# zalo/TetSim

Measured on AMD Instinct MI355X. Metric: tet_solves_per_sec, higher is better.
Workload: dtype f32; 1 GPU; Kuhn-6 cube lattice 55x55x55 cells (998250 tets, 175616 particles), polar-decomposition Jacobi, 20 substeps/frame, dt=1/1200 s; solver=polar_jacobi, arithmetic=fast, formulation=reference (rest shape carried from substep to substep, 148 B/tet), tets=998250, particles=175616, parallelism=single GPU

## Files before the change

include/tetsim.h:

```cpp
#ifndef TETSIM_H
#define TETSIM_H

#include <stdint.h>

#ifdef __cplusplus
extern "C" {
#endif

#define TETSIM_ABI_VERSION 5

typedef struct tetsim_body *tetsim_handle;

enum {
    TETSIM_OK = 0,
    TETSIM_EINVAL = 1,
    TETSIM_ENODEVICE = 2,
    TETSIM_EHIP = 3,
    TETSIM_ENOMEM = 4,
    TETSIM_ECOMM = 5,
    TETSIM_ESTATE = 6
};

enum {
    TETSIM_SOLVER_POLAR_JACOBI = 0,
// ... 102 lines not shown
int tetsim_write_state(tetsim_handle h, const float *pos, const float *vel);
int tetsim_state_size(tetsim_handle h, uint64_t *bytes_out);
int tetsim_save_state(tetsim_handle h, void *blob, uint64_t bytes);
int tetsim_load_state(tetsim_handle h, const void *blob, uint64_t bytes);

int tetsim_get_owned_ids(tetsim_handle h, int32_t *out);
int tetsim_get_local_tets(tetsim_handle h, int32_t *out);
int tetsim_get_tet_order(tetsim_handle h, int32_t *out);
int tetsim_get_level_offsets(tetsim_handle h, int32_t *out);
int tetsim_read_inv_mass(tetsim_handle h, float *out);


int tetsim_set_visual_mesh(tetsim_handle h, const float *vis_verts, uint32_t nvis, const float *rest_normals);
int tetsim_get_visual_ids(tetsim_handle h, int32_t *out);
int tetsim_read_visual_mesh(tetsim_handle h, float *positions_out, float *normals_out);
int tetsim_halo_refresh_final(tetsim_handle h);
int tetsim_group_refresh_final(tetsim_handle *handles, uint32_t count);
int tetsim_set_visual_triangles(tetsim_handle h, const int32_t *tri_ids, uint32_t ntri);
int tetsim_read_visual_vertex_normals(tetsim_handle h, float *normals_out);
int tetsim_visual_vertex_normals_from(tetsim_handle h, const float *all_positions, float *normals_out);
int tetsim_group_read_visual_vertex_normals(tetsim_handle *handles, uint32_t count, float *positions_out, float *normals_out);


int tetsim_set_grab(tetsim_handle h, int32_t id, const float xyz[3]);
int tetsim_start_grab(tetsim_handle h, const float xyz[3], int32_t *id_out);
int tetsim_nearest_particle(tetsim_handle h, const float xyz[3], int32_t *global_id, double *dist2);


typedef struct TetSimRay    { double origin[3], direction[3], near, far; } TetSimRay;
typedef struct TetSimRayHit { int32_t hit, body, triangle, reserved; double distance, point[3]; } TetSimRayHit;
int tetsim_raycast_visual(tetsim_handle h, const TetSimRay *rays, uint32_t count, TetSimRayHit *hits);
int tetsim_start_grab_ray(tetsim_handle h, const TetSimRay *ray, TetSimRayHit *hit_out, int32_t *id_out);
int tetsim_read_visual_bounding_sphere(tetsim_handle h, double centre[3], double *radius);


enum { TETSIM_COLLIDER_SPHERE = 0, TETSIM_COLLIDER_CAPSULE = 1, TETSIM_COLLIDER_BOX = 2, TETSIM_COLLIDER_PLANE = 3 };
#define TETSIM_MAX_COLLIDERS 8
typedef struct TetSimCollider {
    int32_t kind;
    int32_t reserved;
    double a[3];
    double b[3];
    double axes[9];
    double radius;
    double friction;
    double velocity[3];
} TetSimCollider;
int tetsim_set_colliders(tetsim_handle h, const TetSimCollider *colliders, uint32_t count);


enum { TETSIM_FIELD_POSITIONS = 0, TETSIM_FIELD_VELOCITIES = 1, TETSIM_FIELD_PREV_POSITIONS = 2,
       TETSIM_FIELD_QUATS = 3, TETSIM_FIELD_VISUAL_POSITIONS = 4, TETSIM_FIELD_VISUAL_NORMALS = 5,
       TETSIM_FIELD_VISUAL_VERTEX_NORMALS = 6 };
#define TETSIM_MAX_EXPORT_FIELDS 8
typedef struct TetSimDeviceField {
    int32_t field, reserved;
    void *dst;
    uint64_t row_stride;
} TetSimDeviceField;
int tetsim_export_device(tetsim_handle h, const TetSimDeviceField *fields, uint32_t count, void *consumer_stream);
int tetsim_import_device(tetsim_handle h, const void *pos, uint64_t pos_stride,
                         const void *vel, uint64_t vel_stride, void *producer_stream);


typedef struct tetsim_snapshot_s *tetsim_snapshot;
int tetsim_snapshot_create(tetsim_handle h, tetsim_snapshot *out);
int tetsim_snapshot_capture(tetsim_handle h, tetsim_snapshot s, const void *body_mask, void *caller_stream);
int tetsim_snapshot_restore(tetsim_handle h, tetsim_snapshot s, const void *body_mask, void *caller_stream);
void tetsim_snapshot_destroy(tetsim_snapshot s);


#define TETSIM_OBS_WIDTH 20
enum { TETSIM_OBS_MASS = 0, TETSIM_OBS_COM = 1 , TETSIM_OBS_VCOM = 4 , TETSIM_OBS_VOLUME = 7,
       TETSIM_OBS_REST_VOLUME = 8, TETSIM_OBS_MIN_VOLUME_RATIO = 9, TETSIM_OBS_INVERTED_TETS = 10,
       TETSIM_OBS_AABB_MIN = 11 , TETSIM_OBS_AABB_MAX = 14 , TETSIM_OBS_MAX_SPEED2 = 17,
       TETSIM_OBS_NONFINITE = 18, TETSIM_OBS_RESERVED = 19  };
int tetsim_observe_bodies_device(tetsim_handle h, void *dst, uint64_t row_stride, void *caller_stream);
int tetsim_read_body_observations(tetsim_handle h, double *out);


#define TETSIM_RAY_INVALID (-1)
int tetsim_raycast_visual_device(tetsim_handle h,
        const void *rays,     uint64_t ray_stride,
        const void *ray_body,
        uint32_t count,
        void *hits,           uint64_t hit_stride,
        void *caller_stream);
int tetsim_visual_bounding_spheres_device(tetsim_handle h, void *dst, uint64_t row_stride, void *caller_stream);


#define TETSIM_STRAIN_WIDTH 16
#define TETSIM_STRAIN_BODY_WIDTH 8
#define TETSIM_STRAIN_SWEEPS 4
enum { TETSIM_STRAIN_F = 0 , TETSIM_STRAIN_J = 9, TETSIM_STRAIN_DEV = 10,
       TETSIM_STRAIN_STRETCH = 11 , TETSIM_STRAIN_GREEN = 14, TETSIM_STRAIN_RESERVED = 15  };
int tetsim_tet_strain_device(tetsim_handle h, void *dst, uint64_t row_stride, void *caller_stream);
int tetsim_read_tet_strain(tetsim_handle h, float *out);
int tetsim_body_strain_device(tetsim_handle h, void *dst, uint64_t row_stride, void *caller_stream);
int tetsim_visual_strain_device(tetsim_handle h, int32_t channel, void *dst, uint64_t row_stride, void *caller_stream);
int tetsim_prep_strain_table(const float *verts, uint32_t nv, const int32_t *tets, uint32_t nt, double density, void *records_out);


int tetsim_profile(tetsim_handle h, uint32_t n, double dt, const TetSimParams *params, TetSimProfile *out);
int tetsim_time_kernels(tetsim_handle h, uint32_t reps, double dt, const TetSimParams *params, TetSimProfile *out);
int tetsim_time_step_n(tetsim_handle h, uint32_t n, double dt, const TetSimParams *params, double *ms_out);
int tetsim_measure_copy_bandwidth(int32_t device, uint64_t bytes, uint32_t reps, double *gbps_out);
int tetsim_measure_stream_bandwidth(int32_t device, uint64_t bytes, uint32_t reps, int32_t kind, double *gbps_out);


int tetsim_comm_unique_id(void *id128);
int tetsim_comm_init(tetsim_handle h, const void *id128, int32_t rank, int32_t nranks);
typedef struct TetSimCommInfo {
    int32_t rccl_ranks, rccl_rank;
    uint32_t neighbours;
    uint64_t send_bytes_per_substep, recv_bytes_per_substep, max_message_bytes;
    int32_t loopback;
    int32_t p2p;
} TetSimCommInfo;
int tetsim_comm_info(tetsim_handle h, TetSimCommInfo *out);
int tetsim_comm_selftest(tetsim_handle h);
int tetsim_comm_probe(tetsim_handle h, uint64_t bytes, uint32_t reps, int32_t use_graph, uint32_t per_graph,
                      double *host_us, double *total_us);
int tetsim_halo_probe(tetsim_handle h, uint32_t reps, double *min_us, double *median_us, double *max_us);
#define TETSIM_P2P_BLOB_BYTES 512
int tetsim_halo_p2p_export(tetsim_handle h, void *blob);
int tetsim_halo_p2p_connect(tetsim_handle h, const void *blobs, uint32_t count);
int tetsim_halo_p2p_probe(tetsim_handle h, uint32_t reps, double *min_us, double *median_us, double *max_us);
int tetsim_group_step_n(tetsim_handle *handles, uint32_t count, uint32_t n, double dt, const TetSimParams *params);
int tetsim_halo_exchange_local(tetsim_handle *handles, uint32_t count);
int tetsim_get_halo_plan(tetsim_handle h, int32_t *neigh ,
                         int32_t *send_counts, int32_t *recv_counts,
                         int32_t *send_ids, int32_t *recv_ids);
int tetsim_halo_export(tetsim_handle h, uint32_t n, float *out_xyzw);
int tetsim_halo_import(tetsim_handle h, uint32_t n, const float *in_xyzw);


int tetsim_prep_levels(const int32_t *tets, uint32_t nt, uint32_t nv, int32_t *level, uint32_t *num_levels);
int tetsim_prep_colours(const int32_t *tets, uint32_t nt, uint32_t nv, int32_t *colour, uint32_t *num_colours);
int tetsim_prep_clusters(const int32_t *tets, uint32_t nt, uint32_t nv, int32_t *order, int32_t *launch, int32_t *lane,
                         int32_t *step, uint32_t *num_launches, uint32_t *num_clusters);
int tetsim_prep_tiles(const float *verts, uint32_t nv, const int32_t *tets, uint32_t nt, const uint32_t *body_first_tet,
                      const uint32_t *body_first_vert, uint32_t bodies, int32_t *tile_tets, uint32_t *tile_off,
                      uint8_t *corner_slot, uint32_t *num_tiles);
int tetsim_prep_slot_table(const int32_t *tets, uint32_t nt, uint32_t nv, int32_t ref_quirk,
                           int32_t *slots , uint32_t *dropped);
int tetsim_prep_call_tiles(const float *verts, uint32_t nv, const int32_t *tets, uint32_t nt, uint32_t sizes[4],
                           uint32_t *blk_vert_off, int32_t *blk_verts, uint32_t *vp_ell);
int tetsim_prep_call_schedule(const int32_t *blk_verts, const uint32_t *blk_vert_off, uint32_t nb, const uint32_t *vp_ell,
                              uint32_t vp_cols, uint32_t nv_pad, uint32_t nv_owned, uint32_t lag, uint32_t *entry,
                              uint32_t capacity, uint32_t *period, uint32_t *tail, int32_t *fell_back);
int tetsim_prep_check_call_schedule(const int32_t *blk_verts, const uint32_t *blk_vert_off, uint32_t nb, const uint32_t *vp_ell,
                                    uint32_t vp_cols, uint32_t nv_pad, uint32_t nv_owned, const uint32_t *entry, uint32_t period,
                                    uint32_t tail);
int tetsim_prep_ref_grab_texels(int32_t grab_id, uint32_t num_elems, uint32_t num_particles, int32_t out[2]);
int tetsim_prep_boundary_surface(const float *verts ,
                                 const int32_t *tets, uint32_t nt, uint32_t nv,
                                 float *vis_verts , int32_t *tri_ids ,
                                 uint32_t *nrows, uint32_t *ntri);
int tetsim_prep_rest(const float *verts, uint32_t nv, const int32_t *tets, uint32_t nt, double density,
                     float *inv_mass, float *inv_rest_pose, float *inv_rest_volume);

int tetsim_prep_partition(const float *verts , uint32_t nv, const int32_t *tets, uint32_t nt,
                          int32_t part_count, int32_t *vert_owner_out);
typedef struct TetSimPartQuality {
    uint32_t owned_particles;
    uint32_t ghost_particles;
    uint32_t boundary_particles;
    uint32_t local_elems;
    uint32_t owned_elems;
    uint32_t num_neighbours;
} TetSimPartQuality;
int tetsim_prep_partition_quality(const int32_t *tets, uint32_t nt, uint32_t nv, int32_t part_count,
                                  const int32_t *vert_owner, TetSimPartQuality *out);

typedef struct tetsim_plan_s *tetsim_plan;
typedef struct TetSimPlanSizes {
    uint32_t owned_particles, boundary_particles, local_particles, local_elems, owned_elems, num_neighbours;
} TetSimPlanSizes;
int tetsim_plan_create(const int32_t *tets, uint32_t nt, uint32_t nv, int32_t part_count, int32_t part_index,
                       const int32_t *vert_owner, tetsim_plan *out);
int tetsim_plan_create_deep(const int32_t *tets, uint32_t nt, uint32_t nv, int32_t part_count, int32_t part_index,
                            const int32_t *vert_owner, int32_t depth, tetsim_plan *out);
int tetsim_plan_layers(tetsim_plan p, uint32_t *first_layer_ghosts, uint8_t *tet_layer);
int tetsim_plan_neighbour_layer2(tetsim_plan p, uint32_t i, uint32_t *send_count, uint32_t *recv_start, uint32_t *recv_count);
int tetsim_plan_neighbour_layer2_ids(tetsim_plan p, uint32_t i, int32_t *send_local, int32_t *send_global, int32_t *recv_global);
void tetsim_plan_destroy(tetsim_plan p);
int tetsim_plan_sizes(tetsim_plan p, TetSimPlanSizes *out);
int tetsim_plan_arrays(tetsim_plan p, int32_t *local_to_global_vert, int32_t *local_to_global_tet, int32_t *local_tets);
int tetsim_plan_neighbour(tetsim_plan p, uint32_t i, int32_t *rank, uint32_t *send_count, uint32_t *recv_start,
                          uint32_t *recv_count, int32_t *send_is_contiguous);
int tetsim_plan_neighbour_ids(tetsim_plan p, uint32_t i, int32_t *send_local, int32_t *send_global, int32_t *recv_global);

int tetsim_abi_version(void);
typedef struct TetSimLibraryInfo {
    int32_t abi;
    int32_t ablation;
    uint32_t debug_env;
    char source_sha[20];
    char kernel_sha[20];
} TetSimLibraryInfo;
int tetsim_library_info(TetSimLibraryInfo *out);

typedef struct TetSimMeshArrays {
    uint32_t num_particles;
    uint32_t num_elems;
    uint32_t num_edges;
    uint32_t num_vis_verts;
    uint32_t num_vis_tris;
    uint32_t part_count;
    const float *verts;
    const int32_t *tets;
    const int32_t *edge_ids;
    const float *vis_verts;
    const int32_t *vis_tri_ids;
    const int32_t *tet_colour;
    const int32_t *vert_owner;
} TetSimMeshArrays;
typedef struct tetsim_mesh_file *tetsim_mesh;

int tetsim_mesh_write(const char *path, const TetSimMeshArrays *a);
int tetsim_mesh_open(const char *path, tetsim_mesh *out);
int tetsim_mesh_arrays(tetsim_mesh m, TetSimMeshArrays *out);
int tetsim_mesh_close(tetsim_mesh m);
int tetsim_create_from_file(const char *path, const TetSimOptions *opts, tetsim_handle *out);

#ifdef __cplusplus
}
#endif
#endif
```

tetsim_amd/_capi.py:

```python
import ctypes as C
import os

_HERE = os.path.dirname(os.path.abspath(__file__))
LIB_PATH = os.environ.get("TETSIM_HIP_LIB") or os.path.join(_HERE, "libtetsim_hip.so")

OK, EINVAL, ENODEVICE, EHIP, ENOMEM, ECOMM, ESTATE = range(7)
RAY_INVALID = -1
SOLVER_POLAR_JACOBI, SOLVER_NEOHOOKEAN_GS = 0, 1
PRECISE, FAST = 0, 1
ORDER_ORIGINAL, ORDER_COLOURED, ORDER_CLUSTERED = 0, 1, 2
FLAG_REF_SLOT_TABLE, FLAG_REF_FIXED_BOUNDS, FLAG_GATHER_FORMULATION, FLAG_CONSTANT_REST_SHAPE, FLAG_REF_GRAB_TEXEL, FLAG_DEEP_GHOSTS = 1, 2, 4, 8, 16, 32
FLAG_REF_ROTATION_EXIT = 64
FLAG_LEAN_STATE = 128
K_TET, K_VERTEX, K_HALO, K_COUNT = 0, 1, 2, 3
COLLIDER_SPHERE, COLLIDER_CAPSULE, COLLIDER_BOX, COLLIDER_PLANE = 0, 1, 2, 3
MAX_COLLIDERS = 8
FIELD_POSITIONS, FIELD_VELOCITIES, FIELD_PREV_POSITIONS, FIELD_QUATS, FIELD_VISUAL_POSITIONS, FIELD_VISUAL_NORMALS, FIELD_VISUAL_VERTEX_NORMALS = range(7)
MAX_EXPORT_FIELDS = 8
OBS_WIDTH = 20
(OBS_MASS, OBS_COM, OBS_VCOM, OBS_VOLUME, OBS_REST_VOLUME, OBS_MIN_VOLUME_RATIO, OBS_INVERTED_TETS, OBS_AABB_MIN, OBS_AABB_MAX, OBS_MAX_SPEED2,
 OBS_NONFINITE, OBS_RESERVED) = 0, 1, 4, 7, 8, 9, 10, 11, 14, 17, 18, 19
STRAIN_WIDTH, STRAIN_BODY_WIDTH, STRAIN_SWEEPS = 16, 8, 4
STRAIN_F, STRAIN_J, STRAIN_DEV, STRAIN_STRETCH, STRAIN_GREEN, STRAIN_RESERVED = 0, 9, 10, 11, 14, 15


class TetSimParams(C.Structure):
    _fields_ = [("gravity", C.c_double), ("friction", C.c_double), ("devCompliance", C.c_double),
                ("volCompliance", C.c_double), ("worldBounds", C.c_double * 6)]


class TetSimOptions(C.Structure):
    _fields_ = [("solver", C.c_int32), ("precision", C.c_int32), ("order", C.c_int32), ("flags", C.c_uint32),
                ("device", C.c_int32), ("density", C.c_double), ("part_count", C.c_int32),
                ("part_index", C.c_int32), ("vert_owner", C.POINTER(C.c_int32)), ("tet_colour", C.POINTER(C.c_int32))]


class TetSimMeshArrays(C.Structure):
    _fields_ = [("num_particles", C.c_uint32), ("num_elems", C.c_uint32), ("num_edges", C.c_uint32),
                ("num_vis_verts", C.c_uint32), ("num_vis_tris", C.c_uint32), ("part_count", C.c_uint32),
                ("verts", C.POINTER(C.c_float)), ("tets", C.POINTER(C.c_int32)), ("edge_ids", C.POINTER(C.c_int32)),
                ("vis_verts", C.POINTER(C.c_float)), ("vis_tri_ids", C.POINTER(C.c_int32)),
                ("tet_colour", C.POINTER(C.c_int32)), ("vert_owner", C.POINTER(C.c_int32))]


class TetSimInfo(C.Structure):
    _fields_ = [("num_particles", C.c_uint32), ("num_elems", C.c_uint32), ("owned_particles", C.c_uint32),
                ("local_particles", C.c_uint32), ("local_elems", C.c_uint32), ("owned_elems", C.c_uint32),
                ("num_levels", C.c_uint32), ("max_valence", C.c_uint32), ("dropped_slots", C.c_uint32),
                ("num_neighbours", C.c_uint32), ("device_bytes", C.c_uint64), ("solver", C.c_int32),
                ("precision", C.c_int32), ("order", C.c_int32), ("device", C.c_int32), ("flags", C.c_uint32),
                ("num_vis_verts", C.c_uint32), ("num_bodies", C.c_uint32), ("fused_particle_pass", C.c_uint32), ("total_vis_verts", C.c_uint32)]


class TetSimProfile(C.Structure):
    _fields_ = [("total_ms", C.c_double), ("kernel_ms", C.c_double * K_COUNT), ("launches", C.c_uint32 * K_COUNT),
                ("substeps", C.c_uint32), ("tets_per_tet_launch", C.c_uint32)]


class TetSimLibraryInfo(C.Structure):
    _fields_ = [("abi", C.c_int32), ("ablation", C.c_int32), ("debug_env", C.c_uint32), ("source_sha", C.c_char * 20),
                ("kernel_sha", C.c_char * 20)]


DEBUG_ENV_NAMES = ["TETSIM_DEBUG_LOOPBACK_HALO", "TETSIM_DEBUG_LOOPBACK_COPY", "TETSIM_DEBUG_ONE_STREAM", "TETSIM_DEBUG_GROUP_SYNC",
                   "TETSIM_DEBUG_HOSTPROF", "TETSIM_DEBUG_TRACE", "TETSIM_HALO_SYNC", "TETSIM_HALO_GRAPH", "TETSIM_DEBUG_LOOPBACK_DELAY_US", "TETSIM_NH_QUADS", "TETSIM_FUSED_PARTICLE_PASS",
                   "TETSIM_FRAME_KERNEL", "TETSIM_FRAME_LOCAL", "TETSIM_NH_FOLD", "TETSIM_HALO_ALIGNED_TILES", "TETSIM_HALO_FOLD_WAIT", "TETSIM_QUAD", "TETSIM_QUAD_POLL_DELAY", "TETSIM_NH_FRAME",
                   "TETSIM_NH_ONE_LAUNCH", "TETSIM_PJ_ONE_LAUNCH", "TETSIM_PJ_CALL_LAG"]


LAB_ENV_NAMES = ["TETSIM_DEBUG_TRACE", "TETSIM_NH_QUADS", "TETSIM_FRAME_LOCAL", "TETSIM_NH_FOLD", "TETSIM_HALO_ALIGNED_TILES", "TETSIM_QUAD_POLL_DELAY", "TETSIM_NH_FRAME"]


class TetSimCommInfo(C.Structure):
    _fields_ = [("rccl_ranks", C.c_int32), ("rccl_rank", C.c_int32), ("neighbours", C.c_uint32), ("send_bytes_per_substep", C.c_uint64),
                ("recv_bytes_per_substep", C.c_uint64), ("max_message_bytes", C.c_uint64), ("loopback", C.c_int32), ("p2p", C.c_int32)]


class TetSimPlanSizes(C.Structure):
    _fields_ = [("owned_particles", C.c_uint32), ("boundary_particles", C.c_uint32), ("local_particles", C.c_uint32),
                ("local_elems", C.c_uint32), ("owned_elems", C.c_uint32), ("num_neighbours", C.c_uint32)]


class TetSimPartQuality(C.Structure):
    _fields_ = [("owned_particles", C.c_uint32), ("ghost_particles", C.c_uint32), ("boundary_particles", C.c_uint32),
                ("local_elems", C.c_uint32), ("owned_elems", C.c_uint32), ("num_neighbours", C.c_uint32)]


class TetSimError(RuntimeError):
    def __init__(self, code, msg):
        super().__init__("tetsim error %d: %s" % (code, msg))
        self.code = code


class TetSimCollider(C.Structure):
    _fields_ = [("kind", C.c_int32), ("reserved", C.c_int32), ("a", C.c_double * 3), ("b", C.c_double * 3), ("axes", C.c_double * 9),
                ("radius", C.c_double), ("friction", C.c_double), ("velocity", C.c_double * 3)]


class TetSimRay(C.Structure):
    _fields_ = [("origin", C.c_double * 3), ("direction", C.c_double * 3), ("near", C.c_double), ("far", C.c_double)]


class TetSimRayHit(C.Structure):
    _fields_ = [("hit", C.c_int32), ("body", C.c_int32), ("triangle", C.c_int32), ("reserved", C.c_int32), ("distance", C.c_double),
                ("point", C.c_double * 3)]


class TetSimDeviceField(C.Structure):
    _fields_ = [("field", C.c_int32), ("reserved", C.c_int32), ("dst", C.c_void_p), ("row_stride", C.c_uint64)]


SYMBOLS = [
    "tetsim_abi_version", "tetsim_default_options", "tetsim_default_params", "tetsim_create", "tetsim_create_batch", "tetsim_get_batch_layout", "tetsim_destroy",
    "tetsim_last_error", "tetsim_get_info", "tetsim_step", "tetsim_step_n", "tetsim_sync",
    "tetsim_library_info", "tetsim_read_quats_pinned", "tetsim_state_size", "tetsim_save_state", "tetsim_load_state",
    "tetsim_read_positions", "tetsim_read_positions_pinned", "tetsim_read_prev_positions", "tetsim_read_velocities", "tetsim_read_quats",
    "tetsim_read_vol_error", "tetsim_write_state", "tetsim_get_owned_ids", "tetsim_get_local_tets",
    "tetsim_get_tet_order", "tetsim_get_level_offsets", "tetsim_read_inv_mass", "tetsim_set_visual_mesh", "tetsim_get_visual_ids", "tetsim_halo_refresh_final", "tetsim_group_refresh_final", "tetsim_halo_probe", "tetsim_halo_p2p_probe",
    "tetsim_read_visual_mesh", "tetsim_set_visual_triangles", "tetsim_read_visual_vertex_normals", "tetsim_visual_vertex_normals_from", "tetsim_group_read_visual_vertex_normals", "tetsim_set_grab", "tetsim_set_colliders",
    "tetsim_start_grab", "tetsim_nearest_particle", "tetsim_profile", "tetsim_time_kernels", "tetsim_time_step_n", "tetsim_measure_copy_bandwidth", "tetsim_measure_stream_bandwidth",
    "tetsim_comm_unique_id", "tetsim_comm_init", "tetsim_comm_info", "tetsim_comm_selftest", "tetsim_comm_probe", "tetsim_group_step_n", "tetsim_halo_exchange_local", "tetsim_get_halo_plan",
    "tetsim_halo_p2p_export", "tetsim_halo_p2p_connect",
    "tetsim_halo_export", "tetsim_halo_import", "tetsim_prep_levels", "tetsim_prep_colours", "tetsim_prep_clusters",
    "tetsim_prep_tiles", "tetsim_prep_slot_table", "tetsim_prep_call_tiles", "tetsim_prep_call_schedule", "tetsim_prep_check_call_schedule", "tetsim_prep_ref_grab_texels", "tetsim_prep_rest", "tetsim_prep_partition", "tetsim_prep_partition_quality", "tetsim_plan_create", "tetsim_plan_destroy", "tetsim_plan_sizes",
    "tetsim_plan_arrays", "tetsim_plan_neighbour", "tetsim_plan_neighbour_ids",
    "tetsim_plan_create_deep", "tetsim_plan_layers", "tetsim_plan_neighbour_layer2", "tetsim_plan_neighbour_layer2_ids",
    "tetsim_raycast_visual", "tetsim_start_grab_ray", "tetsim_read_visual_bounding_sphere", "tetsim_prep_boundary_surface",
    "tetsim_export_device", "tetsim_import_device",
    "tetsim_snapshot_create", "tetsim_snapshot_capture", "tetsim_snapshot_restore", "tetsim_snapshot_destroy",
    "tetsim_observe_bodies_device", "tetsim_read_body_observations",
    "tetsim_raycast_visual_device", "tetsim_visual_bounding_spheres_device",
    "tetsim_tet_strain_device", "tetsim_read_tet_strain", "tetsim_body_strain_device", "tetsim_visual_strain_device", "tetsim_prep_strain_table",
    "tetsim_mesh_write", "tetsim_mesh_open", "tetsim_mesh_arrays", "tetsim_mesh_close", "tetsim_create_from_file",
]

OPTIONAL_SYMBOLS = ("tetsim_set_colliders", "tetsim_raycast_visual", "tetsim_start_grab_ray", "tetsim_read_visual_bounding_sphere", "tetsim_prep_boundary_surface",
                    "tetsim_export_device", "tetsim_import_device",
                    "tetsim_snapshot_create", "tetsim_snapshot_capture", "tetsim_snapshot_restore", "tetsim_snapshot_destroy",
                    "tetsim_observe_bodies_device", "tetsim_read_body_observations",
                    "tetsim_raycast_visual_device", "tetsim_visual_bounding_spheres_device",
                    "tetsim_tet_strain_device", "tetsim_read_tet_strain", "tetsim_body_strain_device", "tetsim_visual_strain_device", "tetsim_prep_strain_table")

_lib = None


def lib():
    global _lib
    if _lib is not None:
        return _lib
    if not os.path.exists(LIB_PATH):
        raise ImportError("libtetsim_hip.so is not built: run `python -m tetsim_amd.build` "
                          "(the HIP extension is mandatory; there is no CPU fallback)")
    L = C.CDLL(LIB_PATH)
    H, fp, ip, dp = C.c_void_p, C.POINTER(C.c_float), C.POINTER(C.c_int32), C.POINTER(C.c_double)
    u32, i32, dbl = C.c_uint32, C.c_int32, C.c_double
    PP = C.POINTER(TetSimParams)
    L.tetsim_abi_version.restype = C.c_int
    L.tetsim_default_options.argtypes = [C.POINTER(TetSimOptions)]
    L.tetsim_default_options.restype = None
    L.tetsim_default_params.argtypes = [PP]
    L.tetsim_default_params.restype = None
    L.tetsim_create.argtypes = [fp, u32, ip, u32, C.POINTER(TetSimOptions), C.POINTER(H)]
    L.tetsim_create_batch.argtypes = [C.POINTER(fp), C.POINTER(u32), C.POINTER(ip), C.POINTER(u32), u32, C.POINTER(TetSimOptions), C.POINTER(H)]
    L.tetsim_get_batch_layout.argtypes = [H, C.POINTER(u32), C.POINTER(u32)]
    L.tetsim_destroy.argtypes = [H]
    L.tetsim_destroy.restype = None
    L.tetsim_comm_probe.argtypes = [H, C.c_uint64, u32, i32, u32, dp, dp]
    L.tetsim_nearest_particle.argtypes = [H, fp, ip, dp]
    L.tetsim_mesh_write.argtypes = [C.c_char_p, C.POINTER(TetSimMeshArrays)]
    L.tetsim_mesh_open.argtypes = [C.c_char_p, C.POINTER(H)]
    L.tetsim_mesh_arrays.argtypes = [H, C.POINTER(TetSimMeshArrays)]
    L.tetsim_mesh_close.argtypes = [H]
    L.tetsim_create_from_file.argtypes = [C.c_char_p, C.POINTER(TetSimOptions), C.POINTER(H)]
    L.tetsim_last_error.argtypes = [H]
    L.tetsim_last_error.restype = C.c_char_p
    L.tetsim_get_info.argtypes = [H, C.POINTER(TetSimInfo)]
    L.tetsim_step.argtypes = [H, dbl, PP]
    L.tetsim_step_n.argtypes = [H, u32, dbl, PP]
    L.tetsim_sync.argtypes = [H]
    for n in ("positions", "prev_positions", "velocities", "quats", "inv_mass"):
        getattr(L, "tetsim_read_" + n).argtypes = [H, fp]
    L.tetsim_read_positions_pinned.argtypes = [H, C.POINTER(fp)]
    L.tetsim_read_quats_pinned.argtypes = [H, C.POINTER(fp)]
    L.tetsim_library_info.argtypes = [C.POINTER(TetSimLibraryInfo)]
    L.tetsim_state_size.argtypes = [H, C.POINTER(C.c_uint64)]
    L.tetsim_save_state.argtypes = [H, C.c_void_p, C.c_uint64]
    L.tetsim_load_state.argtypes = [H, C.c_void_p, C.c_uint64]
    L.tetsim_read_vol_error.argtypes = [H, dp]
    L.tetsim_write_state.argtypes = [H, fp, fp]
    for n in ("owned_ids", "local_tets", "tet_order", "level_offsets"):
        getattr(L, "tetsim_get_" + n).argtypes = [H, ip]
    L.tetsim_set_visual_mesh.argtypes = [H, fp, u32, fp]
    L.tetsim_read_visual_mesh.argtypes = [H, fp, fp]
    L.tetsim_get_visual_ids.argtypes = [H, C.POINTER(C.c_int32)]
    L.tetsim_halo_refresh_final.argtypes = [H]
    L.tetsim_halo_probe.argtypes = [H, u32, C.POINTER(C.c_double), C.POINTER(C.c_double), C.POINTER(C.c_double)]
    L.tetsim_halo_p2p_probe.argtypes = [H, u32, C.POINTER(C.c_double), C.POINTER(C.c_double), C.POINTER(C.c_double)]
    L.tetsim_group_refresh_final.argtypes = [C.POINTER(H), u32]
    L.tetsim_set_visual_triangles.argtypes = [H, ip, u32]
    L.tetsim_read_visual_vertex_normals.argtypes = [H, fp]
    L.tetsim_visual_vertex_normals_from.argtypes = [H, fp, fp]
    L.tetsim_group_read_visual_vertex_normals.argtypes = [C.POINTER(H), u32, fp, fp]
    L.tetsim_set_grab.argtypes = [H, i32, fp]
    if hasattr(L, "tetsim_set_colliders"):
        L.tetsim_set_colliders.argtypes = [H, C.POINTER(TetSimCollider), u32]
    L.tetsim_start_grab.argtypes = [H, fp, ip]
    if hasattr(L, "tetsim_raycast_visual"):
        L.tetsim_raycast_visual.argtypes = [H, C.c_void_p, u32, C.c_void_p]
        L.tetsim_start_grab_ray.argtypes = [H, C.POINTER(TetSimRay), C.POINTER(TetSimRayHit), ip]
        L.tetsim_read_visual_bounding_sphere.argtypes = [H, dp, dp]
        L.tetsim_prep_boundary_surface.argtypes = [fp, ip, u32, u32, fp, ip, C.POINTER(u32), C.POINTER(u32)]
    if hasattr(L, "tetsim_export_device"):
        L.tetsim_export_device.argtypes = [H, C.POINTER(TetSimDeviceField), u32, C.c_void_p]
        L.tetsim_import_device.argtypes = [H, C.c_void_p, C.c_uint64, C.c_void_p, C.c_uint64, C.c_void_p]
    if hasattr(L, "tetsim_snapshot_create"):
        L.tetsim_snapshot_create.argtypes = [H, C.POINTER(H)]
        L.tetsim_snapshot_capture.argtypes = [H, H, C.c_void_p, C.c_void_p]
        L.tetsim_snapshot_restore.argtypes = [H, H, C.c_void_p, C.c_void_p]
        L.tetsim_snapshot_destroy.argtypes = [H]
        L.tetsim_snapshot_destroy.restype = None
    if hasattr(L, "tetsim_observe_bodies_device"):
        L.tetsim_observe_bodies_device.argtypes = [H, C.c_void_p, C.c_uint64, C.c_void_p]
        L.tetsim_read_body_observations.argtypes = [H, dp]
    if hasattr(L, "tetsim_raycast_visual_device"):
        L.tetsim_raycast_visual_device.argtypes = [H, C.c_void_p, C.c_uint64, C.c_void_p, u32, C.c_void_p, C.c_uint64, C.c_void_p]
        L.tetsim_visual_bounding_spheres_device.argtypes = [H, C.c_void_p, C.c_uint64, C.c_void_p]
    if hasattr(L, "tetsim_tet_strain_device"):
        L.tetsim_tet_strain_device.argtypes = [H, C.c_void_p, C.c_uint64, C.c_void_p]
        L.tetsim_read_tet_strain.argtypes = [H, fp]
        L.tetsim_body_strain_device.argtypes = [H, C.c_void_p, C.c_uint64, C.c_void_p]
        L.tetsim_visual_strain_device.argtypes = [H, i32, C.c_void_p, C.c_uint64, C.c_void_p]
        L.tetsim_prep_strain_table.argtypes = [fp, u32, ip, u32, dbl, C.c_void_p]
    L.tetsim_profile.argtypes = [H, u32, dbl, PP, C.POINTER(TetSimProfile)]
    L.tetsim_time_kernels.argtypes = [H, u32, dbl, PP, C.POINTER(TetSimProfile)]
    L.tetsim_time_step_n.argtypes = [H, u32, dbl, PP, dp]
    L.tetsim_measure_copy_bandwidth.argtypes = [i32, C.c_uint64, u32, dp]
    L.tetsim_measure_stream_bandwidth.argtypes = [i32, C.c_uint64, u32, i32, dp]
    L.tetsim_comm_unique_id.argtypes = [C.c_void_p]
    L.tetsim_comm_init.argtypes = [H, C.c_void_p, i32, i32]
    L.tetsim_comm_selftest.argtypes = [H]
    L.tetsim_comm_info.argtypes = [H, C.POINTER(TetSimCommInfo)]
    L.tetsim_group_step_n.argtypes = [C.POINTER(H), u32, u32, dbl, PP]
    L.tetsim_halo_exchange_local.argtypes = [C.POINTER(H), u32]
    L.tetsim_halo_p2p_export.argtypes = [H, C.c_void_p]
    L.tetsim_halo_p2p_connect.argtypes = [H, C.c_void_p, u32]
    L.tetsim_get_halo_plan.argtypes = [H, ip, ip, ip, ip, ip]
    L.tetsim_halo_export.argtypes = [H, u32, fp]
    L.tetsim_halo_import.argtypes = [H, u32, fp]
    L.tetsim_prep_levels.argtypes = [ip, u32, u32, ip, C.POINTER(u32)]
    L.tetsim_prep_colours.argtypes = [ip, u32, u32, ip, C.POINTER(u32)]
    L.tetsim_prep_clusters.argtypes = [ip, u32, u32, ip, ip, ip, ip, C.POINTER(u32), C.POINTER(u32)]
    L.tetsim_prep_tiles.argtypes = [fp, u32, ip, u32, C.POINTER(u32), C.POINTER(u32), u32, ip, C.POINTER(u32), C.POINTER(C.c_uint8), C.POINTER(u32)]
    L.tetsim_prep_slot_table.argtypes = [ip, u32, u32, i32, ip, C.POINTER(u32)]
    up = C.POINTER(u32)
    L.tetsim_prep_call_tiles.argtypes = [fp, u32, ip, u32, up, up, ip, up]
    L.tetsim_prep_call_schedule.argtypes = [ip, up, u32, up, u32, u32, u32, u32, up, u32, up, up, ip]
    L.tetsim_prep_check_call_schedule.argtypes = [ip, up, u32, up, u32, u32, u32, up, u32, u32]
    L.tetsim_prep_ref_grab_texels.argtypes = [i32, u32, u32, ip]
    L.tetsim_prep_rest.argtypes = [fp, u32, ip, u32, dbl, fp, fp, fp]
    L.tetsim_prep_partition.argtypes = [fp, u32, ip, u32, i32, ip]
    L.tetsim_prep_partition_quality.argtypes = [ip, u32, u32, i32, ip, C.POINTER(TetSimPartQuality)]
    L.tetsim_plan_create.argtypes = [ip, u32, u32, i32, i32, ip, C.POINTER(H)]
    L.tetsim_plan_destroy.argtypes = [H]
    L.tetsim_plan_destroy.restype = None
    L.tetsim_plan_sizes.argtypes = [H, C.POINTER(TetSimPlanSizes)]
    L.tetsim_plan_arrays.argtypes = [H, ip, ip, ip]
    L.tetsim_plan_neighbour.argtypes = [H, u32, ip, C.POINTER(u32), C.POINTER(u32), C.POINTER(u32), ip]
    L.tetsim_plan_neighbour_ids.argtypes = [H, u32, ip, ip, ip]
    L.tetsim_plan_create_deep.argtypes = [ip, u32, u32, i32, i32, ip, i32, C.POINTER(H)]
    L.tetsim_plan_layers.argtypes = [H, C.POINTER(u32), C.POINTER(C.c_uint8)]
    L.tetsim_plan_neighbour_layer2.argtypes = [H, u32, C.POINTER(u32), C.POINTER(u32), C.POINTER(u32)]
    L.tetsim_plan_neighbour_layer2_ids.argtypes = [H, u32, ip, ip, ip]
    for s in SYMBOLS:
        if s in OPTIONAL_SYMBOLS and not hasattr(L, s):
            continue
        f = getattr(L, s)
        if s not in ("tetsim_default_options", "tetsim_default_params", "tetsim_destroy", "tetsim_last_error",
                     "tetsim_plan_destroy", "tetsim_snapshot_destroy"):
            f.restype = C.c_int
    _lib = L
    return L


def library_info():
    li = TetSimLibraryInfo()
    check(lib().tetsim_library_info(C.byref(li)))
    return {"abi": li.abi, "ablation": bool(li.ablation), "source_sha": li.source_sha.decode(), "kernel_sha": li.kernel_sha.decode(),
            "debug_env": [n for i, n in enumerate(DEBUG_ENV_NAMES) if li.debug_env >> i & 1], "path": LIB_PATH}


def check(rc, handle=None):
    if rc != OK:
        msg = lib().tetsim_last_error(handle)
        raise TetSimError(rc, msg.decode("utf-8", "replace") if msg else "")
```

tetsim_amd/csrc/body.h:

```cpp
#pragma once
#include <dlfcn.h>
#include <hip/hip_runtime.h>
#include <rccl/rccl.h>

#include <algorithm>
#include <atomic>
#include <chrono>
#include <cmath>
#include <cstdio>
#include <cstdlib>
#include <cstring>
#include <map>
#include <string>
#include <vector>

#include "../../include/tetsim.h"
#include "dev_common.h"
#include "dev_store.h"
#include "query_device.h"
#include "host_prep.h"
#include "mesh_file.h"

namespace tetsim {

// ... 4 lines not shown
    ncclResult_t (*GetUniqueId)(ncclUniqueId*) = nullptr;
    ncclResult_t (*CommInitRank)(ncclComm_t*, int, ncclUniqueId, int) = nullptr;
    ncclResult_t (*CommDestroy)(ncclComm_t) = nullptr;
    ncclResult_t (*CommCount)(const ncclComm_t, int*) = nullptr;
    ncclResult_t (*CommUserRank)(const ncclComm_t, int*) = nullptr;
    ncclResult_t (*Send)(const void*, size_t, ncclDataType_t, int, ncclComm_t, hipStream_t) = nullptr;
    ncclResult_t (*Recv)(void*, size_t, ncclDataType_t, int, ncclComm_t, hipStream_t) = nullptr;
    ncclResult_t (*GroupStart)() = nullptr;
    ncclResult_t (*GroupEnd)() = nullptr;
    const char* (*GetErrorString)(ncclResult_t) = nullptr;
    std::string err;
    bool loaded = false, process_wide = false;
    bool load() {
        if (loaded) return true;
        if (const char* over = getenv("TETSIM_RCCL_LIB")) {
            lib = dlopen(over, RTLD_NOW | RTLD_LOCAL);
            if (!lib) { err = std::string("cannot load TETSIM_RCCL_LIB=") + over + ": " + dlerror(); return false; }
        }
        for (const char* name : {"librccl.so.1", "librccl.so"}) {
            if (lib) break;
            lib = dlopen(name, RTLD_NOW | RTLD_NOLOAD);
        }
        if (!lib && dlsym(RTLD_DEFAULT, "ncclCommInitRank") && dlsym(RTLD_DEFAULT, "ncclSend")) process_wide = true;
        for (const char* name : {"librccl.so.1", "librccl.so", "/opt/rocm/lib/librccl.so.1"}) {
            if (lib || process_wide) break;
            lib = dlopen(name, RTLD_NOW | RTLD_LOCAL | RTLD_DEEPBIND);
        }
        if (!lib && !process_wide) { err = std::string("cannot load librccl: ") + dlerror(); return false; }
        auto sym = [&](const char* n) { void* p = dlsym(process_wide ? RTLD_DEFAULT : lib, n); if (!p) err = std::string("librccl lacks ") + n; return p; };
        GetUniqueId = reinterpret_cast<decltype(GetUniqueId)>(sym("ncclGetUniqueId"));
        CommInitRank = reinterpret_cast<decltype(CommInitRank)>(sym("ncclCommInitRank"));
        CommDestroy = reinterpret_cast<decltype(CommDestroy)>(sym("ncclCommDestroy"));
        CommCount = reinterpret_cast<decltype(CommCount)>(sym("ncclCommCount"));
        CommUserRank = reinterpret_cast<decltype(CommUserRank)>(sym("ncclCommUserRank"));
        Send = reinterpret_cast<decltype(Send)>(sym("ncclSend"));
        Recv = reinterpret_cast<decltype(Recv)>(sym("ncclRecv"));
        GroupStart = reinterpret_cast<decltype(GroupStart)>(sym("ncclGroupStart"));
        GroupEnd = reinterpret_cast<decltype(GroupEnd)>(sym("ncclGroupEnd"));
        GetErrorString = reinterpret_cast<decltype(GetErrorString)>(sym("ncclGetErrorString"));
        loaded = GetUniqueId && CommInitRank && CommDestroy && CommCount && CommUserRank && Send && Recv && GroupStart && GroupEnd && GetErrorString;
        return loaded;
    }
};
inline const char* lab_env(const char* name) {
#ifdef TETSIM_ABLATION
    return getenv(name);
#else
    (void)name;
    return nullptr;
#endif
}
extern Rccl g_rccl;
extern std::atomic<uint64_t> g_stream_generation;

struct PeerLink {
    float4* ghost[2] = {nullptr, nullptr};
    uint32_t* arrived[2] = {nullptr, nullptr};
    void* ipc[3] = {nullptr, nullptr, nullptr};
    float4* g1_even[2] = {nullptr, nullptr};
    float4* g1_final[2] = {nullptr, nullptr};
    float4* g2_even[2] = {nullptr, nullptr};
    float4* g2_odd[2] = {nullptr, nullptr};
    uint32_t* arrived2[2][2] = {{nullptr, nullptr}, {nullptr, nullptr}};
};
struct NeighDev {
    int rank = -1;
    uint32_t send_count = 0, recv_start = 0, recv_count = 0;
    bool contiguous = false;
    uint32_t send_first = 0;
    int32_t* send_idx = nullptr;
    float4* send_buf = nullptr;
    std::vector<int32_t> send_global, recv_global, send_local;
};

struct ObsDev {
    const void* tets = nullptr;
    const double* v0 = nullptr;
    const void *chunks = nullptr, *bodies = nullptr;
    double* partial = nullptr;
    double* rows = nullptr;
    uint32_t n_chunks = 0;
    bool ready = false;
};

struct StrainRec {
    int32_t id[4];
    float b[9];
    uint32_t degenerate;
    double v0_abs;
};
static_assert(sizeof(StrainRec) == 64 && alignof(StrainRec) == 8, "four dwordx4 loads per record");
struct StrainDev {
    const void* table = nullptr;
    const void *chunks = nullptr, *bodies = nullptr;
    const uint32_t* vis_tet = nullptr;
    double* partial = nullptr;
    float* rows = nullptr;
    uint32_t n_chunks = 0;
    bool ready = false;
};

}

using namespace tetsim;

struct tetsim_snapshot_s;

struct tetsim_body {
    std::string err;
    TetSimOptions opt{};
    TetSimInfo info{};
    hipStream_t stream = nullptr, comm_stream = nullptr;
    hipEvent_t ev_fork = nullptr, ev_bnd_tet = nullptr;
    uint32_t interior_tets = 0;
    bool queues_probed = false, queues_independent = false;
    uint64_t probe_generation = 0;
    std::map<uint32_t, std::pair<hipGraphExec_t, hipGraphExec_t>> flag_graphs;
    uint32_t* d_sync = nullptr;
    bool flag_sync = false;
    bool halo_graph_broken = false;
    bool halo_warm = false;
    bool loopback = false;
    bool vel_dead = false;
    bool needs_halo_refresh = false;
    bool fork_needed = true;
    hipEvent_t ev_a = nullptr, ev_b = nullptr, ev_halo = nullptr;
    hipEvent_t ev_boundary2[2] = {nullptr, nullptr}, ev_packed2[2] = {nullptr, nullptr}, ev_sent2[2] = {nullptr, nullptr};
    uint32_t halo_parity = 0;
    DevParams* d_params = nullptr;
    DevParams* d_params_halo = nullptr;
    std::vector<int32_t> tet_colour;
    int32_t grab_global = -1;
    int32_t grab_ref[2] = {-1, -1};
    float grab_pos[3] = {0, 0, 0};
    uint32_t n_colliders = 0;
    DevColliderF col[kMaxColliders] = {};
    DevColliderD d_col[kMaxColliders] = {};
    std::map<uint32_t, hipGraphExec_t> graphs;
    std::vector<void*> allocs;
    std::vector<float> h_verts;
    std::vector<int32_t> h_tets;
    std::vector<uint32_t> batch_first_vert, batch_first_tet;
    bool fast = false;

    PJDev pj;
    PJBlk blk;
    bool blocked = false;
    bool halo_use_flags = true;
    bool halo_use_graph = true;
    bool fused = false;
    bool pj_one_launch = false;
    uint32_t* d_substep_err = nullptr;
    PJCallSched call_sched;
    float4 *rest0_a = nullptr, *rest0_b = nullptr, *rest0_c = nullptr;
    bool quat_stale = false;
    bool frame = false;
    uint32_t frame_epoch = 1;
    uint32_t fold_wave_limit = 0, fold_tile_limit = 0;
    bool quad = false;
    uint32_t* d_frame_err = nullptr;
    int32_t* d_block_tile = nullptr;
    uint32_t frame_blocks = 0;
    DevParams params_on_device;
    bool params_known = false;
    bool frame_local = false;
    bool frame_turn_counted = false;
    bool epoch_block_fresh = false;
    bool frame_exclusive = false;
    float4* partial_b = nullptr;
    size_t partial_slots = 0;
    float4* pos_final_b = nullptr;
    bool fold_halo = false;
    bool fold_possible = false;
    bool fold_wait = false;
    bool v_pending = false;
    uint32_t fuse_step = 0;
    bool fin_in_b = false;
    std::vector<int32_t> tet_perm;
    std::vector<uint32_t> api2dev, dev2api;
    Partition part;
    bool partitioned = false;
    std::vector<int32_t> g2l_owned;
    std::vector<NeighDev> neigh;
    bool pred_any_dt = true;
    float dt_pred = 0.0f;
    ncclComm_t comm = nullptr;
    int comm_rank = -1, comm_size = 0;
    bool deep = false;
    uint32_t n_ghost1 = 0, nb_first = 0;
    std::vector<int32_t> g2l_ghost1;
    bool p2p = false;
    uint32_t timeout_ms = 0;
    float4* ghost_alt = nullptr;
    uint32_t* d_arrived = nullptr;
    uint32_t* d_peer_slots = nullptr;
    uint32_t p2p_cols = 0, p2p_stride = 0;
    uint32_t* d_peer_slots2 = nullptr;
    uint32_t p2p_cols2 = 0;
    float4* own_g1_even[2] = {nullptr, nullptr};
    float4* own_g1_final[2] = {nullptr, nullptr};
    float4* own_g2_even[2] = {nullptr, nullptr};
    float4* own_g2_odd[2] = {nullptr, nullptr};
    std::vector<PeerLink> links;
    uint32_t p2p_probe_base = 0;
    uint64_t p2p_round = 0;
    bool p2p_raise_pending = false;
    bool halo_pending = false;
    bool final_ghosts_fresh = false;
    std::vector<tetsim_body*> group;

    SkinDev skin;
    std::vector<uint32_t> vis_tet;
    std::vector<int32_t> vis_global;
    bool vis_attached = false;
    uint32_t vis_total = 0;
    float4* d_vis_full = nullptr;
    float* pinned_pos = nullptr;
    float* d_packed = nullptr;
    size_t packed_cap = 0;
    float* pinned_quat = nullptr;
    uint32_t* d_api2dev = nullptr;
    hipEvent_t ev_io[2][2] = {{nullptr, nullptr}, {nullptr, nullptr}};
    uint32_t io_parity = 0;
    std::vector<tetsim_snapshot_s*> snapshots;
    uint32_t *d_snap_first_vert = nullptr, *d_snap_first_elem = nullptr, *d_snap_tet_body = nullptr;
    ObsDev obs;
    StrainDev strain;
    double* d_best = nullptr; uint32_t* d_best_id = nullptr;
    uint32_t* d_sphere = nullptr;
    RayIn* d_rays = nullptr; RayPrep* d_ray_prep = nullptr; RayOut* d_ray_hits = nullptr; RayCand* d_ray_cand = nullptr;
    size_t ray_cap = 0, ray_prep_cap = 0, ray_hits_cap = 0, ray_cand_cap = 0;
    std::vector<int32_t> vis_row_body, tri_body;
    QueryBodiesDev qbodies;
    bool qrows_ready = false, qtris_ready = false;
    bool tri_spans_bodies = false;
    RayCand* d_cast_cand = nullptr;

    NHDev nh;
    std::vector<NHClusterLaunch> cluster_launch;
    int32_t* d_slot_vid = nullptr;
    bool nh_fold = false;
    uint8_t* d_first_mask = nullptr;
    uint32_t* d_nh_untouched = nullptr;
    uint32_t nh_untouched = 0;
    bool nh_one_launch = false;
    bool nh_call = false;
    NHSweep nh_sweep1;
    uint32_t nh_sub_index = 0;
    uint32_t nh_epoch_arg = 0;
    std::vector<uint32_t> level_off;
    bool nh_frame = false;
    NHFrameLaunch nh_frame_launch;
    std::vector<uint32_t> nh_seg;
    std::vector<int32_t> order;
    std::vector<float> h_inv_mass;
};

namespace tetsim {

inline bool is_batch(const tetsim_body* h) { return !h->batch_first_vert.empty(); }
inline void body_ranges(const tetsim_body* h, std::vector<uint32_t>* first_vert, std::vector<uint32_t>* first_tet) {
    *first_vert = h->batch_first_vert; *first_tet = h->batch_first_tet;
    if (!is_batch(h)) { *first_vert = {0u, h->info.num_particles}; *first_tet = {0u, h->info.num_elems}; }
}
inline uint32_t body_of_tet(const tetsim_body* h, uint32_t t) {
    const std::vector<uint32_t>& first = h->batch_first_tet;
    return first.empty() ? 0u : static_cast<uint32_t>(std::upper_bound(first.begin(), first.end(), t) - first.begin()) - 1u;
}

inline double rest_volume(const float* v, const int32_t* t) {
    const float *a = v + 3 * t[0], *b = v + 3 * t[1], *c = v + 3 * t[2], *d = v + 3 * t[3];
    const double e1x = static_cast<double>(b[0]) - a[0], e1y = static_cast<double>(b[1]) - a[1], e1z = static_cast<double>(b[2]) - a[2];
    const double e2x = static_cast<double>(c[0]) - a[0], e2y = static_cast<double>(c[1]) - a[1], e2z = static_cast<double>(c[2]) - a[2];
    const double e3x = static_cast<double>(d[0]) - a[0], e3y = static_cast<double>(d[1]) - a[1], e3z = static_cast<double>(d[2]) - a[2];
    const double cx = e2y * e3z - e2z * e3y, cy = e2z * e3x - e2x * e3z, cz = e2x * e3y - e2y * e3x;
    return ((e1x * cx + e1y * cy) + e1z * cz) / 6.0;
}

void build_strain_table(const float* verts, uint32_t nv, const int32_t* tets, uint32_t nt, double density, StrainRec* out);

#define HIPCHK(h, call)                                                                                 \
    do {                                                                                                \
        hipError_t e_ = (call);                                                                         \
        if (e_ != hipSuccess) {                                                                         \
            (h)->err = std::string(#call) + ": " + hipGetErrorString(e_);                               \
            return TETSIM_EHIP;                                                                         \
        }                                                                                               \
    } while (0)

int fail(tetsim_body* h, int code, const std::string& msg);
const char* create_error();
void group_begin(tetsim_body* const* hs, uint32_t count);
int group_result(tetsim_body* const* hs, uint32_t count, int rc);

template <class Tp>
inline int dev_alloc(tetsim_body* h, Tp** p, size_t count) {
    *p = nullptr;
    const size_t bytes = std::max<size_t>(count, 1) * sizeof(Tp);
    void* raw = nullptr;
    hipError_t e = hipMalloc(&raw, bytes);
    if (e != hipSuccess) { h->err = std::string("hipMalloc(") + std::to_string(bytes) + "): " + hipGetErrorString(e); return TETSIM_ENOMEM; }
    h->allocs.push_back(raw);
    h->info.device_bytes += bytes;
    *p = static_cast<Tp*>(raw);
    return 0;
}
// ... 112 lines not shown
```

tetsim_amd/csrc/build_info.cpp:

```cpp
#include <cstdlib>
#include <cstring>

#include "../../include/tetsim.h"

#ifndef TETSIM_SOURCE_SHA
#define TETSIM_SOURCE_SHA "unstamped"
#endif
#ifndef TETSIM_KERNEL_SHA
#define TETSIM_KERNEL_SHA "unstamped"
#endif

extern "C" int tetsim_library_info(TetSimLibraryInfo* out) {
    if (!out) return TETSIM_EINVAL;
    std::memset(out, 0, sizeof(*out));
    out->abi = TETSIM_ABI_VERSION;
#ifdef TETSIM_ABLATION
    out->ablation = 1;
#endif
    static const struct { const char* name; bool lab; } kEnv[] = {
        {"TETSIM_DEBUG_LOOPBACK_HALO", false}, {"TETSIM_DEBUG_LOOPBACK_COPY", false}, {"TETSIM_DEBUG_ONE_STREAM", false}, {"TETSIM_DEBUG_GROUP_SYNC", false},
        {"TETSIM_DEBUG_HOSTPROF", false}, {"TETSIM_DEBUG_TRACE", true}, {"TETSIM_HALO_SYNC", false}, {"TETSIM_HALO_GRAPH", false}, {"TETSIM_DEBUG_LOOPBACK_DELAY_US", false},
        {"TETSIM_NH_QUADS", true}, {"TETSIM_FUSED_PARTICLE_PASS", false}, {"TETSIM_FRAME_KERNEL", false}, {"TETSIM_FRAME_LOCAL", true}, {"TETSIM_NH_FOLD", true},
        {"TETSIM_HALO_ALIGNED_TILES", true}, {"TETSIM_HALO_FOLD_WAIT", false}, {"TETSIM_QUAD", false}, {"TETSIM_QUAD_POLL_DELAY", true}, {"TETSIM_NH_FRAME", true},
        {"TETSIM_NH_ONE_LAUNCH", false}, {"TETSIM_PJ_ONE_LAUNCH", false}, {"TETSIM_PJ_CALL_LAG", false}};
    for (unsigned i = 0; i < sizeof(kEnv) / sizeof(kEnv[0]); i++) {
#ifndef TETSIM_ABLATION
        if (kEnv[i].lab) continue;
#endif
        if (std::getenv(kEnv[i].name)) out->debug_env |= 1u << i;
    }
    std::strncpy(out->source_sha, TETSIM_SOURCE_SHA, sizeof(out->source_sha) - 1);
    std::strncpy(out->kernel_sha, TETSIM_KERNEL_SHA, sizeof(out->kernel_sha) - 1);
    return TETSIM_OK;
}
```

tetsim_amd/csrc/host_prep.cpp:

```cpp
#include "host_prep.h"

#include <algorithm>
#include <cmath>
#include <numeric>

namespace tetsim {

namespace {
inline float fround(double x) { return static_cast<float>(x); }

inline void edge_matrix(const float* verts, const int32_t* t, float m[9]) {
    for (int k = 0; k < 3; k++)
        for (int c = 0; c < 3; c++)
            m[3 * k + c] = fround(static_cast<double>(verts[3 * t[k + 1] + c]) - static_cast<double>(verts[3 * t[0] + c]));
}
inline double det3(const float* A) {
    double a11 = A[0], a12 = A[3], a13 = A[6];
    double a21 = A[1], a22 = A[4], a23 = A[7];
    double a31 = A[2], a32 = A[5], a33 = A[8];
    return a11 * a22 * a33 + a12 * a23 * a31 + a13 * a21 * a32 - a13 * a22 * a31 - a12 * a21 * a33 - a11 * a23 * a32;
}
}

void prep_rest(const float* verts, uint32_t nv, const int32_t* tets, uint32_t nt, double density,
// ... 341 lines not shown
    std::vector<uint8_t> live(4ull * nt, 0);
    for (int32_t enc : inc.slot) live[enc] = 1;

    std::vector<int32_t> slot_of(nv, -1);
    std::vector<int32_t> touched;
    struct Run { uint32_t begin, end; bool ghost; uint8_t cls; };
    auto cls_of = [&](uint32_t sorted_pos) -> uint8_t { return tet_class ? tet_class[B.tet_perm[sorted_pos]] : 0; };
    std::vector<Run> runs;
    {
        uint32_t i = 0;
        while (i < nt) {
            const uint32_t t0 = i;
            touched.clear();
            bool ghost = false;
            while (i < nt && i - t0 < kMaxTets && body_of_pos[i] == body_of_pos[t0] && cls_of(i) == cls_of(t0)) {
                const int32_t* t = &tets[4 * B.tet_perm[i]];
                uint32_t fresh = 0;
                for (int k = 0; k < 4; k++) {
                    bool seen = slot_of[t[k]] >= 0;
                    for (int j = 0; j < k && !seen; j++) seen = t[j] == t[k];
                    if (!seen) fresh++;
                }
                if (touched.size() + fresh > kMaxVerts) break;
                for (int k = 0; k < 4; k++)
                    if (slot_of[t[k]] < 0) {
                        slot_of[t[k]] = 0; touched.push_back(t[k]);
                        ghost |= static_cast<uint32_t>(t[k]) >= nv_owned || static_cast<uint32_t>(t[k]) < nv_boundary;
                    }
                i++;
            }
            for (int32_t v : touched) slot_of[v] = -1;
            runs.push_back({t0, i, ghost, cls_of(t0)});
        }
    }
    std::stable_sort(runs.begin(), runs.end(), [](const Run& a, const Run& b) { return a.cls != b.cls ? a.cls < b.cls : a.ghost < b.ghost; });
    {
        std::vector<int32_t> perm2(nt);
        uint32_t o = 0;
        for (Run& r : runs) {
            std::copy(B.tet_perm.begin() + r.begin, B.tet_perm.begin() + r.end, perm2.begin() + o);
            const uint32_t len = r.end - r.begin;
            r.begin = o; r.end = o + len;
            o += len;
        }
        B.tet_perm.swap(perm2);
    }

    B.tet_lidx.resize(4ull * nt);
    B.lc_ent.resize(4ull * nt);
    B.blk_tet_off.push_back(0);
    B.blk_vert_off.push_back(0);
    std::vector<std::vector<uint32_t>> vert_partials(nv_sum);
    std::vector<std::vector<uint32_t>> vert_staged(nv_sum);
    for (const Run& r : runs) {
        const uint32_t t0 = r.begin, i = r.end;
        if (!r.ghost && r.cls == 0) B.num_interior_blocks++;
        if (r.cls <= 1) B.num_first_blocks++;
        touched.clear();
        for (uint32_t j = t0; j < i; j++)
            for (int k = 0; k < 4; k++) {
                const int32_t v = tets[4 * B.tet_perm[j] + k];
                if (slot_of[v] < 0) { slot_of[v] = 0; touched.push_back(v); }
            }
        std::sort(touched.begin(), touched.end());
        for (size_t u = 0; u < touched.size(); u++) slot_of[touched[u]] = static_cast<int32_t>(u);
        for (uint32_t j = t0; j < i; j++)
            for (int k = 0; k < 4; k++) B.tet_lidx[4ull * j + k] = static_cast<uint8_t>(slot_of[tets[4 * B.tet_perm[j] + k]]);
        const uint32_t ntb = i - t0, nu = static_cast<uint32_t>(touched.size());
        const uint32_t v0 = B.blk_vert_off.back();
        std::vector<uint32_t> cnt(nu + 1, 0);
        for (uint32_t j = 0; j < ntb; j++)
            for (int k = 0; k < 4; k++)
                if (live[4ull * B.tet_perm[t0 + j] + k]) cnt[B.tet_lidx[4ull * (t0 + j) + k] + 1]++;
        for (uint32_t u = 0; u < nu; u++) cnt[u + 1] += cnt[u];
        for (uint32_t u = 0; u < nu; u++) B.lc_range.push_back(cnt[u] | (cnt[u + 1] << 16));
        std::vector<uint32_t> fillp(cnt.begin(), cnt.end() - 1);
        for (uint32_t j = 0; j < ntb; j++)
            for (int k = 0; k < 4; k++)
                if (live[4ull * B.tet_perm[t0 + j] + k]) {
                    const uint32_t u = B.tet_lidx[4ull * (t0 + j) + k];
                    B.lc_ent[4ull * t0 + fillp[u]++] = static_cast<uint16_t>(kMaxTets * k + j);
                }
        for (uint32_t u = 0; u < nu; u++) {
            const int32_t v = touched[u];
            B.blk_verts.push_back(v);
            if (static_cast<uint32_t>(v) < nv_sum && cnt[u + 1] > cnt[u]) vert_partials[v].push_back(v0 + u);
            else if (static_cast<uint32_t>(v) < nv_sum) vert_staged[v].push_back(v0 + u);
            slot_of[v] = -1;
        }
        B.blk_tet_off.push_back(i);
        B.blk_vert_off.push_back(v0 + nu);
        B.max_tile_verts = std::max(B.max_tile_verts, nu);
    }
    B.num_blocks = static_cast<uint32_t>(B.blk_tet_off.size() - 1);
    B.vp_off.assign(nv_sum + 1, 0);
    for (uint32_t v = 0; v < nv_sum; v++) {
        B.vp_off[v + 1] = B.vp_off[v] + static_cast<uint32_t>(vert_partials[v].size());
        B.max_partials = std::max<uint32_t>(B.max_partials, static_cast<uint32_t>(vert_partials[v].size()));
    }
    B.vp_idx.reserve(B.vp_off[nv_sum]);
    for (uint32_t v = 0; v < nv_sum; v++) B.vp_idx.insert(B.vp_idx.end(), vert_partials[v].begin(), vert_partials[v].end());
    B.nv_pad = (nv_sum + 63u) & ~63u;
    B.vp_cols = 0;
    for (uint32_t v = 0; v < nv_sum; v++) B.vp_cols = std::max<uint32_t>(B.vp_cols, static_cast<uint32_t>(vert_partials[v].size() + vert_staged[v].size()));
    B.vp_ell.assign(static_cast<size_t>(std::max(B.vp_cols, 1u)) * B.nv_pad, 0xffffffffu);
    for (uint32_t v = 0; v < nv_sum; v++) {
        const size_t live = vert_partials[v].size();
        for (size_t j = 0; j < live; j++) B.vp_ell[j * B.nv_pad + v] = vert_partials[v][j];
        for (size_t j = 0; j < vert_staged[v].size(); j++) B.vp_ell[(live + j) * B.nv_pad + v] = vert_staged[v][j];
    }
    const uint32_t ns = static_cast<uint32_t>(B.blk_verts.size());
    B.ns_pad = (ns + 63u) & ~63u;
    B.slot_src.assign(static_cast<size_t>(std::max(B.max_partials, 1u)) * B.ns_pad, 0xffffffffu);
    B.blk_maxsrc.assign(B.num_blocks, 0);
    for (uint32_t v = 0; v < nv_sum; v++)
        if (vert_partials[v].empty()) B.every_owned_particle_has_a_partial = false;
    for (uint32_t b = 0; b < B.num_blocks; b++)
        for (uint32_t g = B.blk_vert_off[b]; g < B.blk_vert_off[b + 1]; g++) {
            const uint32_t v = static_cast<uint32_t>(B.blk_verts[g]);
            if (v >= nv_sum) continue;
            const std::vector<uint32_t>& list = vert_partials[v];
            for (size_t j = 0; j < list.size(); j++) B.slot_src[j * B.ns_pad + g] = list[j];
            B.blk_maxsrc[b] = std::max<uint32_t>(B.blk_maxsrc[b], static_cast<uint32_t>(list.size()));
            if (!list.empty() && list[0] == g) B.lc_range[g] |= 1u << 15;
        }
}

namespace {
struct SchedDeps {
    uint32_t per_xcd = 0, tet_blocks = 0, npb = 0, plain_period = 0;
    std::vector<std::vector<uint32_t>> tiles_of_pb, pbs_of_tile;
};
SchedDeps sched_deps(const int32_t* blk_verts, const uint32_t* blk_vert_off, uint32_t nb, const uint32_t* vp_ell, uint32_t vp_cols, uint32_t nv_pad,
                     uint32_t nv_owned, uint32_t tile) {
    SchedDeps D;
    D.per_xcd = (nb + 7u) / 8u; D.tet_blocks = D.per_xcd * 8u; D.npb = (nv_owned + tile - 1u) / tile;
    D.plain_period = pjb_call_blocks_per_sub(nb, nv_owned, tile);
    D.tiles_of_pb.resize(D.npb); D.pbs_of_tile.resize(nb);
    for (uint32_t v = 0; v < nv_owned; v++)
        for (uint32_t j = 0; j < vp_cols; j++) {
            const uint32_t idx = vp_ell[static_cast<size_t>(j) * nv_pad + v];
            if (idx == 0xffffffffu) continue;
            const uint32_t b = static_cast<uint32_t>(std::upper_bound(blk_vert_off, blk_vert_off + nb + 1, idx) - blk_vert_off) - 1u;
            if (b < nb) D.tiles_of_pb[v / tile].push_back(b);
        }
    for (uint32_t b = 0; b < nb; b++)
        for (uint32_t g = blk_vert_off[b]; g < blk_vert_off[b + 1]; g++)
            if (static_cast<uint32_t>(blk_verts[g]) < nv_owned) D.pbs_of_tile[b].push_back(static_cast<uint32_t>(blk_verts[g]) / tile);
    auto uniq = [](std::vector<uint32_t>& v) { std::sort(v.begin(), v.end()); v.erase(std::unique(v.begin(), v.end()), v.end()); };
    for (auto& v : D.tiles_of_pb) uniq(v);
    for (auto& v : D.pbs_of_tile) uniq(v);
    return D;
}
inline uint32_t sched_tile_of(uint32_t r, uint32_t per_xcd) { return (r & 7u) * per_xcd + (r >> 3); }
void sched_plain(const SchedDeps& D, uint32_t nb, CallSchedule* out) {
    out->period = D.plain_period;
    out->tail = 0; out->lag = 0;
    out->entry.assign(out->period, sched_entry(kSchedEmpty, 0));
    for (uint32_t r = 0; r < D.tet_blocks; r++)
        if (sched_tile_of(r, D.per_xcd) < nb) out->entry[r] = sched_entry(kSchedTile, r);
    for (uint32_t k = 0; k < D.npb; k++) out->entry[D.tet_blocks + k] = sched_entry(kSchedParticles, k);
}
struct SchedPass { std::vector<uint32_t> entry, ready, left; uint32_t head_end = 0; bool stuck = false; };
SchedPass sched_pass(const SchedDeps& D, uint32_t nb, uint32_t lag, const std::vector<uint32_t>& head_at) {
    constexpr uint32_t none = 0xffffffffu;
    SchedPass R;
    R.ready.assign(D.npb, none);
    std::vector<uint32_t> need(D.npb), head, queue;
    std::vector<uint8_t> head_placed(D.npb, 0);
    for (uint32_t k = 0; k < D.npb; k++) {
        need[k] = static_cast<uint32_t>(D.tiles_of_pb[k].size());
        if (head_at[k] != none) head.push_back(k);
        if (need[k] == 0) { R.ready[k] = 0; if (head_at[k] == none) queue.push_back(k); }
    }
    std::stable_sort(head.begin(), head.end(), [&](uint32_t a, uint32_t b) { return head_at[a] < head_at[b]; });
    std::vector<std::vector<uint32_t>> pbs_by_tile(nb);
    for (uint32_t k = 0; k < D.npb; k++) for (uint32_t b : D.tiles_of_pb[k]) pbs_by_tile[b].push_back(k);
    size_t hi = 0, qi = 0;
    uint32_t col_next[8] = {}, tiles_left = D.tet_blocks;
    const uint64_t limit = 4ull * (D.tet_blocks + D.npb) + 64ull * (static_cast<uint64_t>(lag) + 1ull) + 64ull;
    for (uint32_t p = 0;; p++) {
        if (tiles_left == 0 && hi == head.size() && (p & 7u) == 0u) break;
        if (p >= limit) { R.stuck = true; break; }
        const uint32_t x = p & 7u;
        if (hi < head.size() && head_at[head[hi]] <= p) {
            const uint32_t k = head[hi++];
            R.entry.push_back(sched_entry(kSchedParticles, k, true));
            head_placed[k] = 1; R.head_end = p + 1u;
            continue;
        }
        if (qi < queue.size() && R.ready[queue[qi]] <= p) { R.entry.push_back(sched_entry(kSchedParticles, queue[qi++])); continue; }
        if (col_next[x] < D.per_xcd) {
            const uint32_t r = 8u * col_next[x] + x, b = sched_tile_of(r, D.per_xcd);
            bool held = false;
            if (b < nb) for (uint32_t k : D.pbs_of_tile[b]) held = held || (head_at[k] != none && !head_placed[k]);
            if (!held) {
                col_next[x]++; tiles_left--;
                R.entry.push_back(b < nb ? sched_entry(kSchedTile, r) : sched_entry(kSchedEmpty, 0));
                if (b < nb) for (uint32_t k : pbs_by_tile[b])
                    if (--need[k] == 0) { R.ready[k] = p + 8u * lag; if (head_at[k] == none) queue.push_back(k); }
                continue;
            }
        }
        R.entry.push_back(sched_entry(kSchedEmpty, 0));
    }
    R.left.assign(queue.begin() + static_cast<std::ptrdiff_t>(qi), queue.end());
    return R;
}
}

std::string check_call_schedule(const int32_t* blk_verts, const uint32_t* blk_vert_off, uint32_t nb, const uint32_t* vp_ell, uint32_t vp_cols,
                                uint32_t nv_pad, uint32_t nv_owned, const uint32_t* entry, uint32_t period, uint32_t tail, uint32_t tile) {
    constexpr uint32_t none = 0xffffffffu;
    const SchedDeps D = sched_deps(blk_verts, blk_vert_off, nb, vp_ell, vp_cols, nv_pad, nv_owned, tile);
    if (period == 0 || period % 8u != 0u) return "the period is not a positive multiple of 8";
    if (period < D.plain_period) return "the period is shorter than a substep's blocks";
    std::vector<uint64_t> at_tile(nb, none), at_pb(D.npb, none);
    uint32_t col_seen[8] = {}, wrapped_end = 0;
    for (uint32_t p = 0; p < period; p++) {
        const uint32_t kind = entry[p] >> 30, index = entry[p] & kSchedIndexMask;
        const bool wrapped = (entry[p] & kSchedWrapped) != 0u;
        if (kind == kSchedEmpty) continue;
        if (kind == kSchedTile) {
            const uint32_t b = sched_tile_of(index, D.per_xcd);
            if (index >= D.tet_blocks || b >= nb) return "entry " + std::to_string(p) + " names a tile that does not exist";
            if ((index & 7u) != (p & 7u)) return "tile block " + std::to_string(index) + " is not on its XCD";
            if (wrapped) return "tile block " + std::to_string(index) + " is wrapped";
            if ((index >> 3) < col_seen[p & 7u]) return "tile block " + std::to_string(index) + " is out of its XCD's order";
            col_seen[p & 7u] = (index >> 3) + 1u;
            if (at_tile[b] != none) return "tile " + std::to_string(b) + " appears twice";
            at_tile[b] = p;
        } else if (kind == kSchedParticles) {
            if (index >= D.npb) return "entry " + std::to_string(p) + " names a particle block that does not exist";
            if (at_pb[index] != none) return "particle block " + std::to_string(index) + " appears twice";
            at_pb[index] = static_cast<uint64_t>(p) + (wrapped ? period : 0u);
            if (wrapped) wrapped_end = p + 1u;
        } else return "entry " + std::to_string(p) + " has no kind";
    }
    for (uint32_t b = 0; b < nb; b++) if (at_tile[b] == none) return "tile " + std::to_string(b) + " is missing";
    for (uint32_t k = 0; k < D.npb; k++) if (at_pb[k] == none) return "particle block " + std::to_string(k) + " is missing";
    if (tail < wrapped_end || tail > period) return "the tail does not cover the wrapped entries";
    for (uint32_t k = 0; k < D.npb; k++)
        for (uint32_t b : D.tiles_of_pb[k])
            if (!(at_tile[b] < at_pb[k])) return "particle block " + std::to_string(k) + " does not follow tile " + std::to_string(b) + " of its lists";
    for (uint32_t b = 0; b < nb; b++)
        for (uint32_t k : D.pbs_of_tile[b])
            if (!(at_pb[k] < at_tile[b] + period)) return "tile " + std::to_string(b) + " of the next substep does not follow particle block " + std::to_string(k);
    return "";
}

void build_call_schedule(const int32_t* blk_verts, const uint32_t* blk_vert_off, uint32_t nb, const uint32_t* vp_ell, uint32_t vp_cols,
                         uint32_t nv_pad, uint32_t nv_owned, uint32_t lag, CallSchedule* out, uint32_t tile) {
    constexpr uint32_t none = 0xffffffffu;
    const SchedDeps D = sched_deps(blk_verts, blk_vert_off, nb, vp_ell, vp_cols, nv_pad, nv_owned, tile);
    *out = CallSchedule();
    auto plain = [&](const std::string& why) {
        sched_plain(D, nb, out);
        out->fell_back = !why.empty(); out->why = why;
    };
    if (lag == 0 || nb == 0) return plain("");
    if (static_cast<uint64_t>(lag) * 8u >= D.plain_period) return plain("lag " + std::to_string(lag) + ": a whole substep or more");
    std::vector<uint32_t> head_at(D.npb, none);
    SchedPass R;
    bool settled = false;
    for (int pass = 0; pass < 64 && !settled; pass++) {
        R = sched_pass(D, nb, lag, head_at);
        if (R.stuck) return plain("lag " + std::to_string(lag) + ": the layout does not close");
        const uint32_t period = static_cast<uint32_t>(R.entry.size());
        settled = R.left.empty();
        for (uint32_t k : R.left) head_at[k] = 0;
        for (uint32_t k = 0; k < D.npb; k++)
            if (head_at[k] != none && !settled) head_at[k] = R.ready[k] != none && R.ready[k] > period ? R.ready[k] - period : 0u;
    }
    if (!settled) return plain("lag " + std::to_string(lag) + ": the wrapped blocks do not settle");
    out->entry = R.entry;
    out->period = static_cast<uint32_t>(R.entry.size());
    out->tail = R.head_end;
    out->lag = lag;
    const std::string bad = check_call_schedule(blk_verts, blk_vert_off, nb, vp_ell, vp_cols, nv_pad, nv_owned, out->entry.data(), out->period, out->tail, tile);
    if (!bad.empty()) return plain("lag " + std::to_string(lag) + ": " + bad);
}

std::string validate_mesh(const float* verts, uint32_t nv, const int32_t* tets, uint32_t nt, bool forbid_repeats) {
    if ((nv && !verts) || (nt && !tets)) return "null mesh pointer";
    if (nv == 0) return "mesh has no vertices";
    if (nv > 0x3fffffffu || nt > 0x1fffffffu) return "mesh too large for 32-bit slot encoding";
    for (uint32_t e = 0; e < nt; e++) {
        const int32_t* t = &tets[4 * e];
        for (int k = 0; k < 4; k++)
            if (t[k] < 0 || static_cast<uint32_t>(t[k]) >= nv)
                return "tet " + std::to_string(e) + " references vertex " + std::to_string(t[k]) + " outside [0," + std::to_string(nv) + ")";
        if (forbid_repeats && (t[0] == t[1] || t[0] == t[2] || t[0] == t[3] || t[1] == t[2] || t[1] == t[3] || t[2] == t[3]))
            return "tet " + std::to_string(e) + " repeats a vertex (unsupported by the parallel Gauss-Seidel schedule)";
    }
    return "";
}

std::string build_partition(const int32_t* tets, uint32_t nt, uint32_t nv, int part_count, int part_index,
                            const int32_t* vert_owner, Partition* out, int depth) {
    Partition& P = *out;
    P = Partition();
    P.nv_global = nv;
    P.nt_global = nt;
    P.part_count = part_count;
    P.part_index = part_index;
    P.depth = depth;
    if (part_count < 1 || part_index < 0 || part_index >= part_count) return "bad part_index/part_count";
    if (depth != 1 && depth != 2) return "ghost depth must be 1 or 2";

    std::vector<int32_t> owner(nv);
    if (vert_owner) {
        for (uint32_t v = 0; v < nv; v++) {
            if (vert_owner[v] < 0 || vert_owner[v] >= part_count) return "vert_owner out of range";
            owner[v] = vert_owner[v];
        }
    } else {
        const std::string perr = prep_partition(nullptr, nv, tets, nt, part_count, owner.data());
        if (!perr.empty()) return perr;
    }
    const int me = part_index;

    std::vector<std::vector<int32_t>> near1(nv), near2(depth == 2 ? nv : 0);
    auto add = [](std::vector<int32_t>& s, int32_t r) { if (std::find(s.begin(), s.end(), r) == s.end()) s.push_back(r); };
    for (uint32_t e = 0; e < nt; e++) {
        const int32_t* t = &tets[4 * e];
        const int32_t o[4] = {owner[t[0]], owner[t[1]], owner[t[2]], owner[t[3]]};
        if (o[0] == o[1] && o[1] == o[2] && o[2] == o[3]) continue;
        for (int a = 0; a < 4; a++)
            for (int b = 0; b < 4; b++)
                if (o[b] != o[a]) add(near1[t[a]], o[b]);
    }
    if (depth == 2)
        for (uint32_t e = 0; e < nt; e++) {
            const int32_t* t = &tets[4 * e];
            for (int a = 0; a < 4; a++)
                for (int32_t r : near1[t[a]])
                    for (int b = 0; b < 4; b++) {
                        const int32_t v = t[b];
                        if (owner[v] != r && std::find(near1[v].begin(), near1[v].end(), r) == near1[v].end()) add(near2[v], r);
                    }
        }
    auto reads = [&](const std::vector<std::vector<int32_t>>& near, uint32_t v, int32_t r) {
        return !near.empty() && std::find(near[v].begin(), near[v].end(), r) != near[v].end();
    };

    for (uint32_t e = 0; e < nt; e++) {
        const int32_t* t = &tets[4 * e];
        bool mine = false, first_layer = false;
        int lowest = part_count;
        for (int k = 0; k < 4; k++) {
            if (owner[t[k]] == me) mine = true;
            else if (reads(near1, static_cast<uint32_t>(t[k]), me)) first_layer = true;
            lowest = std::min(lowest, owner[t[k]]);
        }
        if (!mine && !(depth == 2 && first_layer)) continue;
        P.local_to_global_tet.push_back(static_cast<int32_t>(e));
        P.tet_layer.push_back(mine ? 0 : 1);
        if (mine && lowest == me) P.owned_tets++;
    }

    std::vector<int32_t> g2l(nv, -1);
    auto is_boundary = [&](uint32_t v) { return !near1[v].empty() || (depth == 2 && !near2[v].empty()); };
    for (uint32_t v = 0; v < nv; v++)
        if (owner[v] == me && is_boundary(v)) { g2l[v] = static_cast<int32_t>(P.local_to_global_vert.size()); P.local_to_global_vert.push_back(v); }
    P.n_boundary = static_cast<uint32_t>(P.local_to_global_vert.size());
    for (uint32_t v = 0; v < nv; v++)
        if (owner[v] == me && !is_boundary(v)) { g2l[v] = static_cast<int32_t>(P.local_to_global_vert.size()); P.local_to_global_vert.push_back(v); }
    P.n_owned = static_cast<uint32_t>(P.local_to_global_vert.size());
    std::vector<int32_t> ghosts1, ghosts2;
    for (uint32_t v = 0; v < nv; v++) {
        if (owner[v] == me) continue;
        if (reads(near1, v, me)) ghosts1.push_back(static_cast<int32_t>(v));
        else if (reads(near2, v, me)) ghosts2.push_back(static_cast<int32_t>(v));
    }
    auto by_owner = [&](int32_t a, int32_t b) { return owner[a] < owner[b]; };
    std::stable_sort(ghosts1.begin(), ghosts1.end(), by_owner);
    std::stable_sort(ghosts2.begin(), ghosts2.end(), by_owner);
    for (int32_t v : ghosts1) { g2l[v] = static_cast<int32_t>(P.local_to_global_vert.size()); P.local_to_global_vert.push_back(v); }
    P.n_ghost1 = static_cast<uint32_t>(ghosts1.size());
    for (int32_t v : ghosts2) { g2l[v] = static_cast<int32_t>(P.local_to_global_vert.size()); P.local_to_global_vert.push_back(v); }

    P.local_tets.resize(4 * P.local_to_global_tet.size());
    for (size_t i = 0; i < P.local_to_global_tet.size(); i++)
        for (int k = 0; k < 4; k++) {
            const int32_t l = g2l[tets[4 * P.local_to_global_tet[i] + k]];
            if (l < 0) return "internal error in the partition plan: a local tet has a corner outside the ghost layers";
            P.local_tets[4 * i + k] = l;
        }

    size_t g1 = 0, g2 = 0;
    for (int r = 0; r < part_count; r++) {
        if (r == me) continue;
        Partition::Neighbour nb;
        nb.rank = r;
        nb.recv_start = P.n_owned + static_cast<uint32_t>(g1);
        while (g1 < ghosts1.size() && owner[ghosts1[g1]] == r) { nb.recv_global.push_back(ghosts1[g1]); g1++; }
        nb.recv_count = static_cast<uint32_t>(nb.recv_global.size());
        nb.recv2_start = P.n_owned + P.n_ghost1 + static_cast<uint32_t>(g2);
        while (g2 < ghosts2.size() && owner[ghosts2[g2]] == r) { nb.recv2_global.push_back(ghosts2[g2]); g2++; }
        nb.recv2_count = static_cast<uint32_t>(nb.recv2_global.size());
        for (uint32_t v = 0; v < nv; v++) {
            if (owner[v] != me) continue;
            if (reads(near1, v, r)) { nb.send_global.push_back(static_cast<int32_t>(v)); nb.send_local.push_back(g2l[v]); }
            else if (reads(near2, v, r)) { nb.send2_global.push_back(static_cast<int32_t>(v)); nb.send2_local.push_back(g2l[v]); }
        }
        nb.send_contiguous = !nb.send_local.empty();
        for (size_t i = 1; i < nb.send_local.size(); i++)
            if (nb.send_local[i] != nb.send_local[i - 1] + 1) { nb.send_contiguous = false; break; }
        if (nb.recv_count || nb.recv2_count || !nb.send_local.empty() || !nb.send2_local.empty()) P.neigh.push_back(std::move(nb));
    }
    return "";
}

}
```

tetsim_amd/csrc/host_prep.h:

```cpp
#pragma once
#include <cstdint>
#include <string>
#include <vector>

namespace tetsim {

constexpr int kRefSlots = 36;

void prep_rest(const float* verts, uint32_t nv, const int32_t* tets, uint32_t nt, double density,
               float* inv_mass, float* inv_rest_pose, float* inv_rest_volume);

float pj_inv_rest_volume(const float* verts, const int32_t* tet);

uint32_t prep_levels(const int32_t* tets, uint32_t nt, uint32_t nv, int32_t* level);
uint32_t prep_colours(const int32_t* tets, uint32_t nt, uint32_t nv, int32_t* colour);
constexpr uint32_t kClusterTets = 8, kClusterVerts = 8;
struct ClusterPlan {
    std::vector<int32_t> pre;
    std::vector<uint32_t> exec_pos;
    std::vector<uint32_t> corner_slots;
    std::vector<uint32_t> launch_off;
    std::vector<uint32_t> step_off;
    std::vector<uint32_t> step_first, step_count;
    std::vector<uint32_t> vid_off;
    std::vector<int32_t> slot_vid;
    uint32_t num_clusters = 0;
};
ClusterPlan prep_clusters(const int32_t* tets, uint32_t nt, uint32_t nv);
uint32_t prep_slot_table(const int32_t* tets, uint32_t nt, uint32_t nv, bool ref_quirk, int32_t* slots);

struct Incidence {
    std::vector<uint32_t> offset;
    std::vector<int32_t> slot;
    uint32_t max_valence = 0;
    uint32_t dropped = 0;
};
Incidence build_incidence(const int32_t* tets, uint32_t nt, uint32_t nv, bool ref_quirk, bool ref_cap);

struct Partition {
    uint32_t nv_global = 0, nt_global = 0;
    int part_count = 1, part_index = 0;
    std::vector<int32_t> local_to_global_vert;
    uint32_t n_owned = 0, n_boundary = 0;
    std::vector<int32_t> local_to_global_tet;
    std::vector<int32_t> local_tets;
    uint32_t owned_tets = 0;
    struct Neighbour {
        int rank;
        std::vector<int32_t> send_local;
        std::vector<int32_t> send_global;
        uint32_t recv_start = 0, recv_count = 0;
        std::vector<int32_t> recv_global;
        bool send_contiguous = false;
        std::vector<int32_t> send2_local, send2_global;
        uint32_t recv2_start = 0, recv2_count = 0;
        std::vector<int32_t> recv2_global;
    };
    std::vector<Neighbour> neigh;
    int depth = 1;
    uint32_t n_ghost1 = 0;
    std::vector<uint8_t> tet_layer;
};
std::string prep_partition(const float* verts, uint32_t nv, const int32_t* tets, uint32_t nt, int parts, int32_t* out_owner);
struct PartQuality {
    uint32_t owned_particles = 0, ghost_particles = 0, boundary_particles = 0;
    uint32_t local_elems = 0, owned_elems = 0;
    uint32_t num_neighbours = 0;
};
std::string partition_quality(const int32_t* tets, uint32_t nt, uint32_t nv, int parts, const int32_t* owner, PartQuality* out);
std::string build_partition(const int32_t* tets, uint32_t nt, uint32_t nv, int part_count, int part_index,
                            const int32_t* vert_owner, Partition* out, int depth = 1);

std::vector<uint32_t> morton_vertex_order(const float* xyz, uint32_t n, uint32_t first, uint32_t count);

#ifndef TETSIM_TILE
#define TETSIM_TILE 256
#endif
constexpr uint32_t kBlockTile = TETSIM_TILE;
constexpr uint32_t kQuadTile = 64;
constexpr int32_t kQuadPollDelay = 0;
constexpr uint32_t kQuadMaxPartials = 12;
struct BlockPlan {
    uint32_t num_blocks = 0;
    uint32_t tile = kBlockTile;
    std::vector<int32_t> tet_perm;
    std::vector<uint32_t> blk_tet_off;
    std::vector<uint32_t> blk_vert_off;
    std::vector<int32_t> blk_verts;
    std::vector<uint8_t> tet_lidx;
    std::vector<uint32_t> lc_range;
    std::vector<uint16_t> lc_ent;
    std::vector<uint32_t> vp_off;
    std::vector<uint32_t> vp_idx;
    std::vector<uint32_t> vp_ell;
    uint32_t vp_cols = 0;
    std::vector<uint32_t> slot_src;
    std::vector<uint32_t> blk_maxsrc;
    uint32_t ns_pad = 0;
    bool every_owned_particle_has_a_partial = true;
    uint32_t nv_pad = 0;
    uint32_t max_tile_verts = 0, max_partials = 0;
    uint32_t num_interior_blocks = 0;
    uint32_t num_first_blocks = 0;
};
void build_blocks(const float* verts, const int32_t* tets, uint32_t nt, uint32_t nv, uint32_t nv_sum,
                  const Incidence& inc, BlockPlan* out, const uint32_t* body_first_tet = nullptr,
                  const uint32_t* body_first_vert = nullptr, uint32_t bodies = 1, uint32_t nv_boundary = 0,
                  const uint8_t* tet_class = nullptr, uint32_t nv_owned = 0xffffffffu, uint32_t tile = kBlockTile);

constexpr uint32_t kSchedTile = 0u, kSchedParticles = 1u, kSchedEmpty = 2u, kSchedWrapped = 1u << 29, kSchedIndexMask = (1u << 29) - 1u;
constexpr uint32_t sched_entry(uint32_t kind, uint32_t index, bool wrapped = false) { return kind << 30 | (wrapped ? kSchedWrapped : 0u) | index; }
constexpr uint32_t pjb_call_blocks_per_sub(uint32_t nb, uint32_t nv_owned, uint32_t threads) {
    return (((nb + 7u) & ~7u) + (nv_owned + threads - 1u) / threads + 7u) & ~7u;
}
constexpr uint32_t kPJCallLagDefault = 0;
struct CallSchedule {
    std::vector<uint32_t> entry;
    uint32_t period = 0, tail = 0;
    uint32_t lag = 0;
    bool fell_back = false;
    std::string why;
};
void build_call_schedule(const int32_t* blk_verts, const uint32_t* blk_vert_off, uint32_t nb, const uint32_t* vp_ell, uint32_t vp_cols,
                         uint32_t nv_pad, uint32_t nv_owned, uint32_t lag, CallSchedule* out, uint32_t tile = kBlockTile);
std::string check_call_schedule(const int32_t* blk_verts, const uint32_t* blk_vert_off, uint32_t nb, const uint32_t* vp_ell, uint32_t vp_cols,
                                uint32_t nv_pad, uint32_t nv_owned, const uint32_t* entry, uint32_t period, uint32_t tail, uint32_t tile = kBlockTile);

std::string validate_mesh(const float* verts, uint32_t nv, const int32_t* tets, uint32_t nt, bool forbid_repeats);

}
```

tetsim_amd/csrc/pj_blocked.hip:

```cpp
#define TETSIM_FAST 1
#include <cstdio>
#include <algorithm>
#include <cstdlib>
#include <type_traits>
#include <vector>

#include "collide.h"
#include "dev_common.h"
#include "dev_store.h"
#include "host_prep.h"
#include "pj_lab.h"

namespace tetsim {
namespace {

#include "pj_math.inc"
#include "pj_blocked_lab.inc"


__device__ __forceinline__ uint32_t xcd_tile(uint32_t b, uint32_t tiles_per_xcd) { return (b & 7u) * tiles_per_xcd + (b >> 3); }

struct VertexOut { f3 p, vel, pred; };
__device__ __forceinline__ VertexOut pjb_vertex_update(f3 acc, float wsum, f3 prev, const DevParams& P, uint32_t v) {
    const float rw = __builtin_amdgcn_rcpf(wsum);
    f3 p = F3(acc.x * rw, acc.y * rw, acc.z * rw);
    const bool grabbed = static_cast<int32_t>(v) == P.grab_local || static_cast<int32_t>(v) == P.grab_local2;
    if (grabbed) p = F3(P.grab[0], P.grab[1], P.grab[2]);
    p.x = fminf(fmaxf(p.x, P.lo[0]), P.hi[0]);
    p.y = fminf(fmaxf(p.y, P.lo[1]), P.hi[1]);
    p.z = fminf(fmaxf(p.z, P.lo[2]), P.hi[2]);
    if (p.y < 0.0f) {
        p.y = 0.0f;
        const float Fx = prev.x - p.x, Fz = prev.z - p.z;
        const float fr = fminf(1.0f, P.dt * P.friction);
        p.x = fmaf(Fx, fr, p.x);
        p.z = fmaf(Fz, fr, p.z);
    }
    if (P.n_colliders != 0u && !grabbed) collide_f32<true>(p.x, p.y, p.z, prev.x, prev.y, prev.z, P);
    const float dt = P.dt;
    const float rdt = __builtin_amdgcn_rcpf(dt);
    VertexOut o;
    o.p = p;
    const float gx = dt * 0.0f, gy = dt * P.gravity, gz = dt * 0.0f;
    o.vel = F3(fmaf(rdt, p.x - prev.x, gx), fmaf(rdt, p.y - prev.y, gy), fmaf(rdt, p.z - prev.z, gz));
    o.pred = F3(fmaf(dt, o.vel.x, p.x), fmaf(dt, o.vel.y, p.y), fmaf(dt, o.vel.z, p.z));
    return o;
}

constexpr uint32_t kTile = kBlockTile;

__device__ __forceinline__ f3 lean_fourth_corner(const f3 r[4]) {
    return F3(-((r[0].x + r[1].x) + r[2].x), -((r[0].y + r[1].y) + r[2].y), -((r[0].z + r[1].z) + r[2].z));
}
struct PJHaloWait { const PJPeerSync* w; const uint32_t* vflag; uint32_t* error; uint32_t timeout_ms; const float4* ghosts; };
constexpr int kModeCarried = 0, kModeConstantRest = 1, kModeLeanState = 2;
inline int blk_mode(const PJBlk& d) { return pjb_mode(d); }
struct PJPoll { uint32_t block, want; uint32_t* error; uint32_t timeout_ms; };
template <int kMode, bool kFused, bool kAlt = false, bool kHaloWait = false, bool kPoll = false>
__device__ __forceinline__ void pjb_tet_body(const PJBlk& d, uint32_t tile_first, uint32_t tile_count, uint32_t tiles_per_xcd TETSIM_DBG_PARAM,
                                             [[maybe_unused]] const PJHaloWait* hw = nullptr, const uint32_t stamp = 0u, [[maybe_unused]] const PJPoll* poll = nullptr) {
    __shared__ float4 s_pos[kTile];
    __shared__ float s_gx[4 * kTile];
    __shared__ float s_gy[4 * kTile];
    __shared__ float s_gz[4 * kTile];
    __shared__ uint2 s_ent[kTile];

    constexpr bool kLean = kMode == kModeConstantRest;
    uint32_t block_index = blockIdx.x;
    if constexpr (kPoll) block_index = poll->block;
    const uint32_t rel = xcd_tile(block_index, tiles_per_xcd);
    if (rel >= tile_count) return;
    const uint32_t b = tile_first + rel;
    const uint32_t tid = threadIdx.x;
    TETSIM_LAB_TILE_BEGIN();
    TETSIM_POLL_TILE(0);
    const uint32_t t0 = d.blk_tet_off[b], ntb = d.blk_tet_off[b + 1] - t0;
    const uint32_t v0 = d.blk_vert_off[b], nu = d.blk_vert_off[b + 1] - v0;

    const bool has_slot = tid < nu, has_tet = tid < ntb;
    const uint32_t slot = v0 + (has_slot ? tid : 0u), e = t0 + (has_tet ? tid : 0u);
    const uint32_t vid = static_cast<uint32_t>(d.blk_verts[slot]);
    const uint32_t range = has_slot ? d.lc_range[slot] : 0u;
    uint32_t src[8];
    uint32_t src8 = 0xffffffffu;
    [[maybe_unused]] uint32_t maxsrc = 0;
    if constexpr (kFused) {
        maxsrc = d.blk_maxsrc[b];
        const uint32_t* col = d.slot_src + slot;
#pragma unroll
        for (uint32_t j = 0; j < 8u; j++) src[j] = (j < maxsrc) ? col[static_cast<size_t>(j) * d.ns_pad] : 0xffffffffu;
        if (maxsrc > 8u) src8 = col[8ull * d.ns_pad];
    }
    const uchar4 li = d.tet_lidx[e];
    auto rec4 = [](const float4* a, uint32_t i) { if constexpr (kPoll) return load_coherent(a, i); else return a[i]; };
    float4 ra = make_float4(0.0f, 0.0f, 0.0f, 0.0f), rb = ra, rc = ra, q_old = make_float4(0.0f, 0.0f, 0.0f, 1.0f);
    auto load_record = [&]() {
        ra = rec4(d.rest_a, e); rb = rec4(d.rest_b, e);
        if constexpr (kMode == kModeLeanState) { if constexpr (kPoll) rc.x = load_coherent1(d.rest_c1, e); else rc.x = d.rest_c1[e]; }
        else { rc = rec4(d.rest_c, e); q_old = rec4(d.quat, e); }
    };
    bool record_late = false;
    if constexpr (kPoll) record_late = poll->want != 0u;
    if (!record_late) load_record();
    const float V = d.vol[e];
    const uint2 ent_row = d.lc_ent[e];
    float4 pos_stage;
    if constexpr (kFused) {
        f3 g[8];
#pragma unroll
        for (uint32_t j = 0; j < 8u; j++) {
            const float4 t = d.partial_prev[src[j] == 0xffffffffu ? 0u : src[j]];
            g[j] = src[j] == 0xffffffffu ? F3(0.0f, 0.0f, 0.0f) : xyz(t);
        }
        const float4 t8 = d.partial_prev[src8 == 0xffffffffu ? 0u : src8];
        const float4 prev4 = d.fin_in[vid];
        const float wsum = d.wsum[vid];
        f3 acc = F3(0.0f, 0.0f, 0.0f);
#pragma unroll
        for (uint32_t j = 0; j < 8u; j++) { acc.x += g[j].x; acc.y += g[j].y; acc.z += g[j].z; }
        if (src8 != 0xffffffffu) { acc.x += t8.x; acc.y += t8.y; acc.z += t8.z; }
        if (maxsrc > 9u) {
            const uint32_t* col = d.slot_src + slot;
            for (uint32_t j = 9u; j < maxsrc; j++) {
                const uint32_t sj = col[static_cast<size_t>(j) * d.ns_pad];
                const float4 tj = d.partial_prev[sj == 0xffffffffu ? 0u : sj];
                if (sj != 0xffffffffu) { acc.x += tj.x; acc.y += tj.y; acc.z += tj.z; }
            }
        }
        const VertexOut o = pjb_vertex_update(acc, wsum, xyz(prev4), *d.params, vid);
        pos_stage = make_float4(o.pred.x, o.pred.y, o.pred.z, 0.0f);
        if (has_slot && ((range >> 15) & 1u)) {
            store_wt(d.fin_out, vid, make_float4(o.p.x, o.p.y, o.p.z, 0.0f));
            if (d.vel) store_wt(d.vel, vid, make_float4(o.vel.x, o.vel.y, o.vel.z, 0.0f));
        }
    } else if constexpr (kHaloWait) {
        if (tid < 64u) {
            const PJPeerSync& w = *hw->w;
            const uint32_t* word = tid == 0u ? hw->vflag : (tid <= w.n_wait ? w.wait[tid - 1u] : nullptr);
            bool pending = word != nullptr;
            const long long t0 = wall_clock64(), limit = 100000ll * hw->timeout_ms;
            while (true) {
                if (pending) pending = __hip_atomic_load(word, __ATOMIC_RELAXED, __HIP_MEMORY_SCOPE_SYSTEM) == 0u;
                if (__builtin_amdgcn_ballot_w64(pending) == 0ull) break;
                __builtin_amdgcn_s_sleep(16);
                if (limit && wall_clock64() - t0 > limit) { if (tid == 0) __hip_atomic_store(hw->error, 1u, __ATOMIC_RELAXED, __HIP_MEMORY_SCOPE_SYSTEM); break; }
            }
            if (w.delay_us && w.n_wait) { const long long d0 = wall_clock64(); while (wall_clock64() - d0 < 100ll * w.delay_us) __builtin_amdgcn_s_sleep(8); }
        }
        __syncthreads();
        const bool ghost = vid >= d.nv_owned;
        const float4 own = load_coherent(d.pos_pred, ghost ? 0u : vid), gh = load_coherent(hw->ghosts, ghost ? vid - d.nv_owned : 0u);
        pos_stage = ghost ? gh : own;
    } else if constexpr (kAlt) {
        const uint32_t g = vid - d.nv_owned;
        const float4* src = vid >= d.nv_owned ? (g < d.n_ghost1 ? d.ghost_alt + g : d.ghost2 + (g - d.n_ghost1)) : d.pos_pred + vid;
        pos_stage = *src;
    } else if constexpr (kPoll) {
        TETSIM_POLL_BEGIN();
        TETSIM_POLL_TILE(1);
        pos_stage = load_coherent(d.pos_pred, vid);
        if (poll->want != 0u) {
            bool pend = has_slot && __float_as_uint(pos_stage.w) != poll->want;
            if (__builtin_amdgcn_ballot_w64(pend) != 0ull) {
                const long long t0 = wall_clock64(), limit = 100000ll * poll->timeout_ms;
                do {
                    __builtin_amdgcn_s_sleep(TETSIM_POLL_SLEEP);
                    TETSIM_POLL_LOOK();
                    asm volatile("" ::: "memory");
                    if (pend) { pos_stage = load_coherent(d.pos_pred, vid); pend = __float_as_uint(pos_stage.w) != poll->want; }
                    if (limit && pend && wall_clock64() - t0 > limit) { __hip_atomic_store(poll->error, 1u, __ATOMIC_RELAXED, __HIP_MEMORY_SCOPE_SYSTEM); pend = false; }
                } while (__builtin_amdgcn_ballot_w64(pend) != 0ull);
            }
            TETSIM_POLL_TILE(2);
            __syncthreads();
            TETSIM_POLL_TILE(3);
            load_record();
        }
        TETSIM_POLL_TILE_SAVE();
    } else {
        pos_stage = d.pos_pred[vid];
    }
    if (has_slot) s_pos[tid] = pos_stage;
    if (has_tet) s_ent[tid] = ent_row;
    TETSIM_STAMP(1);
    __builtin_amdgcn_s_waitcnt(0x0F70);
    __syncthreads();
    TETSIM_STAMP(2);

    if (has_tet) {
        f3 cur[4], rest[4], goal[4];
        cur[0] = xyz(s_pos[li.x]); cur[1] = xyz(s_pos[li.y]); cur[2] = xyz(s_pos[li.z]); cur[3] = xyz(s_pos[li.w]);
        rest[0] = F3(ra.x, ra.y, ra.z); rest[1] = F3(ra.w, rb.x, rb.y);
        rest[2] = F3(rb.z, rb.w, rc.x); rest[3] = F3(rc.y, rc.z, rc.w);
        if constexpr (kMode == kModeLeanState) rest[3] = lean_fourth_corner(rest);
        float4 q_new;
        f3 cc;
        TETSIM_LAB_SOLVE_TET(cur, rest, q_old, q_new, goal, cc);
        TETSIM_STAMP(3);
        const f3 vcc = cc * V;
#pragma unroll
        for (int k = 0; k < 4; k++) {
            s_gx[k * kTile + tid] = fmaf(goal[k].x, V, vcc.x);
            s_gy[k * kTile + tid] = fmaf(goal[k].y, V, vcc.y);
            s_gz[k * kTile + tid] = fmaf(goal[k].z, V, vcc.z);
        }
        if constexpr (kMode != kModeLeanState) store_wt(d.quat, e, q_new);
        if (!kLean && TETSIM_DBG_STORE_REST) {
            store_wt(d.rest_a, e, make_float4(goal[0].x, goal[0].y, goal[0].z, goal[1].x));
            store_wt(d.rest_b, e, make_float4(goal[1].y, goal[1].z, goal[2].x, goal[2].y));
            if constexpr (kMode == kModeLeanState) store_wt1(d.rest_c1, e, goal[2].z);
            else store_wt(d.rest_c, e, make_float4(goal[2].z, goal[3].x, goal[3].y, goal[3].z));
        }
    }
    TETSIM_STAMP(4);
    if constexpr (kPoll) __builtin_amdgcn_s_waitcnt(0x0F70);
    __syncthreads();
    TETSIM_STAMP(5);

    if (tid < nu) {
        const uint32_t first = range & 0x7ffu, last = range >> 16;
        const uint16_t* ent = reinterpret_cast<const uint16_t*>(s_ent);
        auto plane = [](const float* base, uint32_t byte_off) { return *reinterpret_cast<const float*>(reinterpret_cast<const char*>(base) + byte_off); };
        float4 acc = make_float4(0.0f, 0.0f, 0.0f, 0.0f);
// ... 596 lines not shown
```

tetsim_amd/csrc/tetsim_api.hip:

```cpp
#include <mutex>

#include "body.h"

using namespace tetsim;

namespace tetsim {

namespace {
thread_local std::string g_create_error;
}
HostProf g_hostprof;

int fail(tetsim_body* h, int code, const std::string& msg) {
    if (h) h->err = msg; else g_create_error = msg;
    return code;
}
const char* create_error() { return g_create_error.c_str(); }
int group_result(tetsim_body* const* hs, uint32_t count, int rc) {
    if (rc == TETSIM_OK || !hs) return rc;
    for (uint32_t i = 0; i < count; i++)
        if (hs[i] && !hs[i]->err.empty()) { g_create_error = "partition " + std::to_string(i) + ": " + hs[i]->err; return rc; }
    if (g_create_error.empty()) g_create_error = "bad argument";
    return rc;
}
// ... 414 lines not shown
    if (o.part_count < 1) o.part_count = 1;
    std::string merr = validate_mesh(verts, nv, tets, nt, o.solver == TETSIM_SOLVER_NEOHOOKEAN_GS);
    if (!merr.empty()) return fail(nullptr, TETSIM_EINVAL, merr);

    int ndev = 0;
    hipError_t e = hipGetDeviceCount(&ndev);
    if (e != hipSuccess || ndev <= 0)
        return fail(nullptr, TETSIM_ENODEVICE, std::string("no HIP device available (") + (e != hipSuccess ? hipGetErrorString(e) : "device count 0") +
                                                   "); libtetsim_hip has no CPU fallback");
    if (o.device < 0 || o.device >= ndev) return fail(nullptr, TETSIM_ENODEVICE, "device ordinal out of range");
    if ((o.flags & TETSIM_FLAG_CONSTANT_REST_SHAPE) && o.solver != TETSIM_SOLVER_POLAR_JACOBI)
        return fail(nullptr, TETSIM_EINVAL, "TETSIM_FLAG_CONSTANT_REST_SHAPE applies to TETSIM_SOLVER_POLAR_JACOBI only");
    if ((o.flags & TETSIM_FLAG_LEAN_STATE) && o.solver != TETSIM_SOLVER_POLAR_JACOBI)
        return fail(nullptr, TETSIM_EINVAL, "TETSIM_FLAG_LEAN_STATE applies to TETSIM_SOLVER_POLAR_JACOBI only");
    if ((o.flags & TETSIM_FLAG_LEAN_STATE) && (o.flags & (TETSIM_FLAG_CONSTANT_REST_SHAPE | TETSIM_FLAG_DEEP_GHOSTS)))
        return fail(nullptr, TETSIM_EINVAL, "TETSIM_FLAG_LEAN_STATE excludes TETSIM_FLAG_CONSTANT_REST_SHAPE and TETSIM_FLAG_DEEP_GHOSTS");

    tetsim_body* h = new tetsim_body();
    h->opt = o;
    h->opt.vert_owner = nullptr;
    if (o.tet_colour && nt) h->tet_colour.assign(o.tet_colour, o.tet_colour + nt);
    h->opt.tet_colour = nullptr;
    h->fast = o.precision == TETSIM_FAST;
    h->timeout_ms = halo_timeout_ms(nullptr);
    h->info.num_particles = nv;
    h->info.num_elems = nt;
    h->info.solver = o.solver; h->info.precision = o.precision; h->info.order = o.order; h->info.device = o.device; h->info.flags = o.flags;
    h->h_verts.assign(verts, verts + 3ull * nv);
    h->h_tets.assign(tets, tets + 4ull * nt);
    h->batch_first_vert = batch_first_vert;
    h->batch_first_tet = batch_first_tet;
    h->info.num_bodies = batch_first_vert.empty() ? 1u : static_cast<uint32_t>(batch_first_vert.size() - 1);

    auto bail = [&](int rc) { g_create_error = h->err; tetsim_destroy(h); return rc; };
    auto hipok = [&](hipError_t er, const char* what) { if (er != hipSuccess) { h->err = std::string(what) + ": " + hipGetErrorString(er); return false; } return true; };
    if (!hipok(hipSetDevice(o.device), "hipSetDevice")) return bail(TETSIM_EHIP);
    if (!hipok(hipStreamCreateWithFlags(&h->stream, hipStreamNonBlocking), "hipStreamCreate")) return bail(TETSIM_EHIP);
    g_stream_generation++;
    if (!hipok(hipEventCreate(&h->ev_a), "hipEventCreate") || !hipok(hipEventCreate(&h->ev_b), "hipEventCreate")) return bail(TETSIM_EHIP);
    for (int i = 0; i < 2; i++)
        if (!hipok(hipEventCreateWithFlags(&h->ev_boundary2[i], hipEventDisableTiming), "hipEventCreate") ||
            !hipok(hipEventCreateWithFlags(&h->ev_packed2[i], hipEventDisableTiming), "hipEventCreate") ||
            !hipok(hipEventCreateWithFlags(&h->ev_sent2[i], hipEventDisableTiming), "hipEventCreate")) return bail(TETSIM_EHIP);
    if (!hipok(hipEventCreateWithFlags(&h->ev_halo, hipEventDisableTiming), "hipEventCreate")) return bail(TETSIM_EHIP);
    { int rc = dev_alloc(h, &h->d_params, 1); if (rc) return bail(rc); }

    TetSimOptions with_owner = o;
    h->opt.vert_owner = with_owner.vert_owner;
    int rc = o.solver == TETSIM_SOLVER_POLAR_JACOBI ? create_polar(h, verts, nv, tets, nt) : create_neohookean(h, verts, nv, tets, nt);
    h->opt.vert_owner = nullptr;
    if (rc) return bail(rc);
    if (!hipok(hipDeviceSynchronize(), "hipDeviceSynchronize")) return bail(TETSIM_EHIP);
    *out = h;
    return TETSIM_OK;
}
}

int tetsim_create(const float* verts, uint32_t nv, const int32_t* tets, uint32_t nt, const TetSimOptions* opts, tetsim_handle* out) {
    return create_common(verts, nv, tets, nt, opts, out, {}, {});
}

int tetsim_create_batch(const float* const* verts, const uint32_t* nv, const int32_t* const* tets, const uint32_t* nt, uint32_t count,
                        const TetSimOptions* opts, tetsim_handle* out) {
    if (!out) return fail(nullptr, TETSIM_EINVAL, "out handle pointer is null");
    *out = nullptr;
    if (!verts || !nv || !tets || !nt || count == 0) return fail(nullptr, TETSIM_EINVAL, "tetsim_create_batch: null argument or empty batch");
    if (opts && opts->part_count > 1) return fail(nullptr, TETSIM_EINVAL, "a batch cannot be partitioned (partition the bodies over handles instead)");
    if (opts && opts->tet_colour) return fail(nullptr, TETSIM_EINVAL, "tet_colour is not supported for batches");
    std::vector<uint32_t> fv(count + 1, 0), ft(count + 1, 0);
    for (uint32_t b = 0; b < count; b++) {
        const std::string merr = validate_mesh(verts[b], nv[b], tets[b], nt[b], opts && opts->solver == TETSIM_SOLVER_NEOHOOKEAN_GS);
        if (!merr.empty()) return fail(nullptr, TETSIM_EINVAL, "body " + std::to_string(b) + ": " + merr);
        const uint64_t v = static_cast<uint64_t>(fv[b]) + nv[b], t = static_cast<uint64_t>(ft[b]) + nt[b];
        if (v > 0x3fffffffull || t > 0x1fffffffull) return fail(nullptr, TETSIM_EINVAL, "batch too large for one handle");
        fv[b + 1] = static_cast<uint32_t>(v); ft[b + 1] = static_cast<uint32_t>(t);
    }
    std::vector<float> av(3ull * fv[count]);
    std::vector<int32_t> at(4ull * ft[count]);
    for (uint32_t b = 0; b < count; b++) {
        std::copy(verts[b], verts[b] + 3ull * nv[b], av.begin() + 3ull * fv[b]);
        for (uint64_t i = 0; i < 4ull * nt[b]; i++) at[4ull * ft[b] + i] = tets[b][i] + static_cast<int32_t>(fv[b]);
    }
    return create_common(av.data(), fv[count], at.data(), ft[count], opts, out, fv, ft);
}

int tetsim_get_batch_layout(tetsim_handle h, uint32_t* first_particle, uint32_t* first_elem) {
    if (!h || !first_particle || !first_elem) return fail(h, TETSIM_EINVAL, "null argument");
    std::vector<uint32_t> fv, ft;
    body_ranges(h, &fv, &ft);
    std::copy(fv.begin(), fv.end(), first_particle);
    std::copy(ft.begin(), ft.end(), first_elem);
    return 0;
}

void tetsim_destroy(tetsim_handle h) {
    if (!h) return;
    (void)hipSetDevice(h->opt.device);
    if (h->stream) (void)hipStreamSynchronize(h->stream);
    if (h->comm_stream) (void)hipStreamSynchronize(h->comm_stream);
    for (tetsim_body* g : h->group) {
        if (!g || g == h) continue;
        (void)hipSetDevice(g->opt.device);
        if (g->stream) (void)hipStreamSynchronize(g->stream);
        if (g->comm_stream) (void)hipStreamSynchronize(g->comm_stream);
        for (tetsim_body*& x : g->group) if (x == h) x = nullptr;
    }
    (void)hipSetDevice(h->opt.device);
    if (h->blk.trace && lab_env("TETSIM_DEBUG_TRACE")) {
        std::vector<unsigned long long> tr(8ull * h->blk.nb);
        if (hipMemcpy(tr.data(), h->blk.trace, tr.size() * sizeof(tr[0]), hipMemcpyDeviceToHost) == hipSuccess)
            if (FILE* f = fopen(lab_env("TETSIM_DEBUG_TRACE"), "wb")) { fwrite(tr.data(), sizeof(tr[0]), tr.size(), f); fclose(f); }
    }
    if (h->blk.trace && lab_env("TETSIM_DEBUG_POLL_TRACE")) {
        std::vector<unsigned long long> tr(8ull * (2ull * h->blk.nb + (h->blk.nv_owned + kBlockTile - 1u) / kBlockTile));
        if (hipMemcpy(tr.data(), h->blk.trace, tr.size() * sizeof(tr[0]), hipMemcpyDeviceToHost) == hipSuccess)
            if (FILE* f = fopen(lab_env("TETSIM_DEBUG_POLL_TRACE"), "wb")) { fwrite(tr.data(), sizeof(tr[0]), tr.size(), f); fclose(f); }
    }
#ifdef TETSIM_ABLATION
    if (h->blk.iter_hist && lab_env("TETSIM_DEBUG_ITER_HIST")) {
        std::vector<unsigned long long> hs(278);
        if (hipMemcpy(hs.data(), h->blk.iter_hist, hs.size() * sizeof(hs[0]), hipMemcpyDeviceToHost) == hipSuccess)
            if (FILE* f = fopen(lab_env("TETSIM_DEBUG_ITER_HIST"), "a")) {
                fprintf(f, "%u %u", h->info.num_elems, h->info.num_particles);
                for (unsigned long long x : hs) fprintf(f, " %llu", x);
                fprintf(f, "\n");
                fclose(f);
            }
    }
#endif
    frame_turn_leave(h);
    for (auto& kv : h->graphs) (void)hipGraphExecDestroy(kv.second);
    h->graphs.clear();
    drop_flag_graphs(h);
    for (PeerLink& l : h->links) for (void* m : l.ipc) if (m) (void)hipIpcCloseMemHandle(m);
    if (h->comm && g_rccl.CommDestroy) g_rccl.CommDestroy(h->comm);
    release_snapshots(h);
    for (void* p : h->allocs) (void)hipFree(p);
    if (h->pinned_pos) (void)hipHostFree(h->pinned_pos);
    if (h->pinned_quat) (void)hipHostFree(h->pinned_quat);
    for (hipEvent_t ev : {h->ev_a, h->ev_b, h->ev_halo, h->ev_boundary2[0], h->ev_boundary2[1], h->ev_packed2[0], h->ev_packed2[1],
                          h->ev_sent2[0], h->ev_sent2[1]}) if (ev) (void)hipEventDestroy(ev);
    for (hipEvent_t ev : {h->ev_fork, h->ev_bnd_tet, h->ev_io[0][0], h->ev_io[0][1], h->ev_io[1][0], h->ev_io[1][1]}) if (ev) (void)hipEventDestroy(ev);
    if (h->comm_stream) (void)hipStreamDestroy(h->comm_stream);
    if (h->stream) (void)hipStreamDestroy(h->stream);
    delete h;
}

int tetsim_get_info(tetsim_handle h, TetSimInfo* info) {
    if (!h || !info) return fail(h, TETSIM_EINVAL, "null argument");
    *info = h->info;
    return 0;
}

int tetsim_step(tetsim_handle h, double dt, const TetSimParams* params) {
    if (!h) return TETSIM_EINVAL;
    if (!h->group.empty()) return fail(h, TETSIM_ESTATE, "this body belongs to an in-process group: step it with tetsim_group_step_n");
    HIPCHK(h, hipSetDevice(h->opt.device));
    if (h->frame) {
        if (int rc = params_for_launch(h, dt, params)) return rc;
        return launch_in_turn(h, [&]() -> int { return launch_frame_kernel(h, 1u, 0u); });
    }
    if (h->nh_frame) {
        if (int rc = params_for_launch(h, dt, params)) return rc;
        return launch_nh_frame_kernel(h, 1u);
    }
    int rc = push_params(h, dt, params, true);
    if (rc) return rc;
    if ((rc = ensure_prediction(h, dt))) return rc;
    if (h->nh_one_launch) {
        if (!h->epoch_block_fresh && (rc = next_epoch_block(h))) return rc;
        h->epoch_block_fresh = false;
        h->nh_epoch_arg = h->frame_epoch;
    }
    if (h->nh_one_launch) rc = launch_in_turn(h, [&]() -> int { return enqueue_substep(h); });
    else rc = enqueue_substep(h);
    h->nh_epoch_arg = 0u;
    if (!rc) rc = flush_v(h);
    return rc;
}

int tetsim_step_n(tetsim_handle h, uint32_t n, double dt, const TetSimParams* params) {
    if (!h) return TETSIM_EINVAL;
    if (!h->group.empty()) return fail(h, TETSIM_ESTATE, "this body belongs to an in-process group: step it with tetsim_group_step_n");
    if (n == 0) return 0;
    while (h->frame && n > 32768u) {
        if (int rc = tetsim_step_n(h, 32768u, dt, params)) return rc;
        n -= 32768u;
    }
    if (h->pj_one_launch) {
        const uint32_t most = pjb_call_chunk(h->call_sched.period, h->call_sched.tail, kBlockTile, 8192u);
        while (n > most) {
            if (int rc = tetsim_step_n(h, most, dt, params)) return rc;
            n -= most;
        }
    }
    if (h->nh_one_launch) {
        const uint32_t stamps = 65000u / h->nh_sweep1.ncolours;
        const uint32_t most = h->nh_call ? call_chunk(nh_call_blocks_per_sub(h->nh_sweep1.blocks), 256u, stamps) : stamps;
        while (n > most) {
            if (int rc = tetsim_step_n(h, most, dt, params)) return rc;
            n -= most;
        }
    }
    HIPCHK(h, hipSetDevice(h->opt.device));
    if (h->nh_call && h->nh_one_launch && !has_transport(h)) {
        if (int rc = params_for_launch(h, dt, params)) return rc;
        return launch_in_turn(h, [&]() -> int {
            nh_launch_predict_value_fast(h->stream, h->nh, h->params_on_device, h->d_params);
            nh_launch_call_fast(h->stream, h->nh, h->nh_sweep1, n);
            nh_launch_post_fast(h->stream, h->nh);
            return launched_with_params(h);
        });
    }
    if (h->nh_frame) {
        if (int rc = params_for_launch(h, dt, params)) return rc;
        return launch_nh_frame_kernel(h, n);
    }
    if ((h->frame || h->pj_one_launch) && !has_transport(h)) {
        if (int rc = params_for_launch(h, dt, params)) return rc;
        return launch_in_turn(h, [&]() -> int {
            if (h->frame) return launch_frame_kernel(h, n, 0u);
            pjb_launch_call(h->stream, h->blk, h->call_sched, n, h->d_substep_err, halo_timeout_ms(h), h->params_on_device, h->d_params);
            return launched_with_params(h);
        });
    }
    int rc = push_params(h, dt, params);
    if (rc) return rc;
    if ((rc = ensure_prediction(h, dt))) return rc;
    if (has_transport(h)) {
        const bool use_graph = h->halo_use_graph;
        const bool own_rank = h->group.empty() && (h->comm || h->p2p);
        if (own_rank && use_graph && h->halo_warm && !h->halo_graph_broken && uses_flag_sync(h)) {
            if ((rc = probe_queue_independence(h))) return rc;
            if (h->queues_independent) {
                rc = step_n_flag_graphs(h, n);
                if (!rc) return 0;
                fprintf(stderr, "[tetsim] halo graph capture failed (%s); falling back to eager halo stepping\n", h->err.c_str());
                h->halo_graph_broken = true;
                (void)hipGetLastError();
                rc = 0;
            }
        }
        if (!own_rank || !h->comm || !use_graph || !h->halo_warm || h->halo_graph_broken || uses_flag_sync(h)) {
            for (uint32_t i = 0; i < n && !rc; i++) rc = enqueue_substep(h, i == 0, i + 1 == n);
            if (!rc) rc = flush_v(h);
            h->halo_warm = true;
            return rc;
        }
        if (h->halo_pending) {
            HIPCHK(h, hipStreamWaitEvent(h->stream, h->ev_sent2[h->halo_parity ^ 1u], 0));
            h->halo_pending = false;
        }
    }
    if (!has_transport(h) && !h->nh_one_launch && h->info.num_elems >= kDirectLaunchTets &&
        (h->opt.solver == TETSIM_SOLVER_POLAR_JACOBI || h->info.num_levels <= 32u)) {
        for (uint32_t i = 0; i < n && !rc; i++) rc = enqueue_substep(h, i == 0, i + 1 == n);
        return rc;
    }
    auto it = h->graphs.find(n);
    if (it == h->graphs.end()) {
        hipGraphExec_t exec = nullptr;
        if ((rc = build_graph(h, n, &exec))) {
            if (!has_transport(h)) return rc;
            fprintf(stderr, "[tetsim] halo graph capture failed (%s); falling back to eager halo stepping\n", h->err.c_str());
            h->halo_graph_broken = true;
            (void)hipGetLastError();
            rc = 0;
            for (uint32_t i = 0; i < n && !rc; i++) rc = enqueue_substep(h, i == 0, i + 1 == n);
            if (!rc) rc = flush_v(h);
            return rc;
        }
        it = h->graphs.emplace(n, exec).first;
    }
    if (h->nh_one_launch)
        return launch_in_turn(h, [&]() -> int { HIPCHK(h, hipGraphLaunch(it->second, h->stream)); return 0; });
    HIPCHK(h, hipGraphLaunch(it->second, h->stream));
    return 0;
}

int tetsim_sync(tetsim_handle h) {
    if (!h) return TETSIM_EINVAL;
    if (int rc = drain(h)) return rc;
    if (h->d_frame_err) {
        uint32_t err = 0;
        HIPCHK(h, hipMemcpy(&err, h->d_frame_err, sizeof err, hipMemcpyDeviceToHost));
        if (err) {
            HIPCHK(h, hipMemset(h->d_frame_err, 0, sizeof err));
            h->frame = false;
            frame_turn_leave(h);
            for (auto& kv : h->graphs) (void)hipGraphExecDestroy(kv.second);
            h->graphs.clear();
            return fail(h, TETSIM_EHIP, "persistent frame kernel: a tile waited in vain for a neighbour tile's partial sums (workgroups not co-resident?); "
                                        "the state since then is invalid; this body falls back to one kernel per substep");
        }
    }
    if (h->pj_one_launch) {
        uint32_t err = 0;
        HIPCHK(h, hipMemcpy(&err, h->d_substep_err, sizeof err, hipMemcpyDeviceToHost));
        if (err) {
            HIPCHK(h, hipMemset(h->d_substep_err, 0, sizeof err));
            h->pj_one_launch = false;
            for (auto& kv : h->graphs) (void)hipGraphExecDestroy(kv.second);
            h->graphs.clear();
            return fail(h, TETSIM_EHIP, "one-launch substep: a particle wave waited in vain for a tile's partial sums (workgroups not dispatched in grid order?); "
                                        "the state since then is invalid; this body falls back to two kernels per substep");
        }
// ... 32 lines not shown
```

tetsim_amd/csrc/tetsim_create.hip:

```cpp
#include "body.h"

namespace tetsim {

int create_polar(tetsim_body* h, const float* verts, uint32_t nv, const int32_t* tets, uint32_t nt) {
    const TetSimOptions& o = h->opt;
    const bool ref_table = (o.flags & TETSIM_FLAG_REF_SLOT_TABLE) != 0;
    std::vector<int32_t> ltets;
    std::vector<int32_t> l2g_v, l2g_t;
    uint32_t nvl = nv, nvo = nv, nvb = 0, ntl = nt;
    h->partitioned = o.part_count > 1;
    h->deep = h->partitioned && (o.flags & TETSIM_FLAG_DEEP_GHOSTS);
    {
        const char* sy = getenv("TETSIM_HALO_SYNC");
        const char* gr = getenv("TETSIM_HALO_GRAPH");
        h->halo_use_flags = !(sy && sy[0] == 'e');
        h->halo_use_graph = !(gr && gr[0] == '0');
    }
    if ((o.flags & TETSIM_FLAG_DEEP_GHOSTS) && !(h->partitioned && h->fast && !(o.flags & TETSIM_FLAG_GATHER_FORMULATION)))
        return fail(h, TETSIM_EINVAL, "TETSIM_FLAG_DEEP_GHOSTS needs a partitioned POLAR_JACOBI body in the blocked FAST formulation");
    uint32_t nvg1 = 0;
    if (h->partitioned) {
        std::string e = build_partition(tets, nt, nv, o.part_count, o.part_index, o.vert_owner, &h->part, h->deep ? 2 : 1);
        if (!e.empty()) return fail(h, TETSIM_EINVAL, e);
        if (h->deep) {
// ... 92 lines not shown
    HIPCHK(h, hipMemset(d.vel, 0, std::max<size_t>(nvl, 1) * sizeof(float4)));

    auto rest_weight = [&](uint32_t local_tet) {
        const uint32_t ge = h->partitioned ? static_cast<uint32_t>(l2g_t[local_tet]) : local_tet;
        return 1.0f / pj_inv_rest_volume(verts, &tets[4 * ge]);
    };

    h->blocked = h->fast && !(o.flags & TETSIM_FLAG_GATHER_FORMULATION);
    if ((o.flags & TETSIM_FLAG_CONSTANT_REST_SHAPE) && !h->blocked)
        return fail(h, TETSIM_EINVAL, "TETSIM_FLAG_CONSTANT_REST_SHAPE needs POLAR_JACOBI + TETSIM_FAST without TETSIM_FLAG_GATHER_FORMULATION");
    if ((o.flags & TETSIM_FLAG_LEAN_STATE) && !h->blocked)
        return fail(h, TETSIM_EINVAL, "TETSIM_FLAG_LEAN_STATE needs POLAR_JACOBI + TETSIM_FAST without TETSIM_FLAG_GATHER_FORMULATION");
    const bool lean_state = (o.flags & TETSIM_FLAG_LEAN_STATE) != 0;
    if (h->blocked) {
        BlockPlan B;
        std::vector<uint8_t> tet_class;
        if (h->partitioned) {
            const char* e = lab_env("TETSIM_HALO_ALIGNED_TILES");
            const bool aligned = !(e && e[0] == '0');
            tet_class.assign(ntl, 0);
            for (uint32_t i = 0; i < ntl; i++) {
                if (h->deep && h->part.tet_layer[i]) { tet_class[i] = 2; continue; }
                if (!aligned) continue;
                for (int c = 0; c < 4; c++) {
                    const uint32_t v = static_cast<uint32_t>(ltets[4ull * i + c]);
                    if (v < nvb || v >= nvo) tet_class[i] = 1;
                }
            }
        }
        static const bool allow_quad = [] { const char* e = getenv("TETSIM_QUAD"); return !(e && e[0] == '0'); }();
        uint32_t quad_cus = 0, quad_per_cu = 0;
        bool quad = allow_quad && !h->partitioned && !(o.flags & (TETSIM_FLAG_CONSTANT_REST_SHAPE | TETSIM_FLAG_LEAN_STATE)) && ntl > 0 && nvo == nvl;
        if (quad) {
            quad_per_cu = pjq_frame_capacity(&quad_cus);
            quad = quad_per_cu != 0u && (static_cast<uint64_t>(ntl) + kQuadTile - 1u) / kQuadTile <= static_cast<uint64_t>(quad_per_cu) * quad_cus / 2u;
        }
        for (;;) {
            build_blocks(lverts.data(), ltets.data(), ntl, nvl, nvo + nvg1, inc, &B, batch ? h->batch_first_tet.data() : nullptr,
                         batch ? h->batch_first_vert.data() : nullptr, bodies, nvb, h->partitioned ? tet_class.data() : nullptr, nvo, quad ? kQuadTile : kBlockTile);
            if (!quad || (B.every_owned_particle_has_a_partial && B.max_partials <= kQuadMaxPartials && B.num_blocks <= quad_per_cu * quad_cus / 2u)) break;
            quad = false;
        }
        h->quad = quad;
        h->tet_perm = B.tet_perm;
        h->nb_first = B.num_first_blocks;
        for (uint32_t b = 0; b < B.num_interior_blocks; b++)
            for (uint32_t e = B.blk_tet_off[b]; e < B.blk_tet_off[b + 1]; e++)
                for (int c = 0; c < 4; c++) {
                    const uint32_t v = static_cast<uint32_t>(ltets[4ull * static_cast<uint32_t>(B.tet_perm[e]) + c]);
                    if (v < nvb || v >= nvo) return fail(h, TETSIM_ESTATE, "internal error in the tile plan: an interior tile touches a boundary or a ghost particle");
                }
        PJBlk& k = h->blk;
        h->interior_tets = B.blk_tet_off[B.num_interior_blocks];
        k.nb = B.num_blocks; k.nb_interior = B.num_interior_blocks; k.nt = ntl; k.nv_local = nvl; k.nv_owned = nvo; k.nv_boundary = nvb;
        {
            const char* fw = getenv("TETSIM_HALO_FOLD_WAIT");
            h->fold_possible = !(fw && fw[0] == '0') && h->partitioned && B.num_interior_blocks > 0 && B.num_interior_blocks < B.num_blocks && nvo > nvb;
            if (h->fold_possible) pjb_wait_capacity((o.flags & TETSIM_FLAG_CONSTANT_REST_SHAPE) ? 1 : lean_state ? 2 : 0, &h->fold_wave_limit, &h->fold_tile_limit);
            h->fold_wait = h->fold_possible && fw && fw[0] == '1';
            h->fold_halo = h->fold_wait;
        }
        k.pos_pred = d.pos_pred; k.pos_final = d.pos_final; k.vel = d.vel; k.params = h->d_params;
        k.lean = (o.flags & TETSIM_FLAG_CONSTANT_REST_SHAPE) != 0;
        k.lean_state = lean_state;
        k.rot_exit_w2 = d.rot_exit_w2;
        uint32_t *bto, *bvo, *lcr, *vpe;
        int32_t* bv;
        uchar4* lidx;
        float* vol;
        uint2* lce;
        const size_t nslots = B.blk_verts.size();
        if ((rc = dev_alloc(h, &bto, B.blk_tet_off.size()))) return rc;
        if ((rc = dev_alloc(h, &bvo, B.blk_vert_off.size()))) return rc;
        if ((rc = dev_alloc(h, &bv, nslots))) return rc;
        if (ntl >= kStoreWtMaxIndex || nslots >= kStoreWtMaxIndex || nvl >= kStoreWtMaxIndex)
            return fail(h, TETSIM_EINVAL, "body too large for one handle (2^27 tets / particles / partial sums: 32-bit store offsets, dev_store.h); partition it");
        if ((rc = dev_alloc(h, &lidx, ntl))) return rc;
        if ((rc = dev_alloc(h, &k.rest_a, ntl))) return rc;
        if ((rc = dev_alloc(h, &k.rest_b, ntl))) return rc;
        if (lean_state) {
            if ((rc = dev_alloc(h, &k.rest_c1, ntl))) return rc;
            if ((rc = dev_alloc(h, &h->rest0_a, ntl))) return rc;
            if ((rc = dev_alloc(h, &h->rest0_b, ntl))) return rc;
            if ((rc = dev_alloc(h, &h->rest0_c, ntl))) return rc;
        } else if ((rc = dev_alloc(h, &k.rest_c, ntl))) return rc;
        if ((rc = dev_alloc(h, &vol, ntl))) return rc;
        if ((rc = dev_alloc(h, &k.quat, ntl))) return rc;
        if ((rc = dev_alloc(h, &lcr, nslots))) return rc;
        if ((rc = dev_alloc(h, &lce, ntl))) return rc;
        if ((rc = dev_alloc(h, &k.partial, nslots))) return rc;
        if ((rc = dev_alloc(h, &vpe, B.vp_ell.size()))) return rc;
        std::vector<float4> ra(ntl), rb(ntl), rcv(ntl), quat(ntl, make_float4(0, 0, 0, 1));
        std::vector<float> volh(ntl);
        std::vector<uchar4> lidxh(ntl);
        std::vector<uint2> lceh(ntl);
        for (uint32_t i = 0; i < ntl; i++) {
            const uint32_t lt = static_cast<uint32_t>(B.tet_perm[i]);
            const int32_t* c = &ltets[4 * lt];
            const float4 p0 = pos[c[0]], p1 = pos[c[1]], p2 = pos[c[2]], p3 = pos[c[3]];
            float4 r0 = p0, r1 = p1, r2 = p2, r3 = p3;
            {
                const float cx = (((p0.x + p1.x) + p2.x) + p3.x) * 0.25f, cy = (((p0.y + p1.y) + p2.y) + p3.y) * 0.25f,
                            cz = (((p0.z + p1.z) + p2.z) + p3.z) * 0.25f;
                r0 = make_float4(p0.x - cx, p0.y - cy, p0.z - cz, 0.0f); r1 = make_float4(p1.x - cx, p1.y - cy, p1.z - cz, 0.0f);
                r2 = make_float4(p2.x - cx, p2.y - cy, p2.z - cz, 0.0f); r3 = make_float4(p3.x - cx, p3.y - cy, p3.z - cz, 0.0f);
            }
            ra[i] = make_float4(r0.x, r0.y, r0.z, r1.x);
            rb[i] = make_float4(r1.y, r1.z, r2.x, r2.y);
            rcv[i] = make_float4(r2.z, r3.x, r3.y, r3.z);
            volh[i] = rest_weight(lt);
            lidxh[i] = make_uchar4(B.tet_lidx[4ull * i], B.tet_lidx[4ull * i + 1], B.tet_lidx[4ull * i + 2], B.tet_lidx[4ull * i + 3]);
            const uint16_t* en = &B.lc_ent[4ull * i];
            lceh[i] = make_uint2(en[0] | (static_cast<uint32_t>(en[1]) << 16), en[2] | (static_cast<uint32_t>(en[3]) << 16));
        }
        std::vector<float> wsum(std::max<size_t>(B.nv_pad, 1), 0.0f);
        {
            std::vector<float> slot_w(nslots, 0.0f);
            for (uint32_t b = 0; b < B.num_blocks; b++) {
                const uint32_t t0 = B.blk_tet_off[b], v0 = B.blk_vert_off[b], nu = B.blk_vert_off[b + 1] - v0;
                for (uint32_t u = 0; u < nu; u++) {
                    const uint32_t first = B.lc_range[v0 + u] & 0x7ffu, last = B.lc_range[v0 + u] >> 16;
                    float w = 0.0f;
                    for (uint32_t i = first; i < last; i++) w += volh[t0 + (B.lc_ent[4ull * t0 + i] % B.tile)];
                    slot_w[v0 + u] = w;
                }
            }
            for (uint32_t v = 0; v < nvo + nvg1; v++) {
                float w = 0.0f;
                for (uint32_t j = 0; j < B.max_partials; j++) {
                    const uint32_t idx = B.vp_ell[static_cast<size_t>(j) * B.nv_pad + v];
                    if (idx != 0xffffffffu) w += slot_w[idx];
                }
                wsum[v] = w;
            }
        }
        float* dws;
        if ((rc = dev_alloc(h, &dws, wsum.size()))) return rc;
        if ((rc = upload(h, dws, wsum))) return rc;
        k.wsum = dws;
        static const bool allow_fused = [] { const char* e = getenv("TETSIM_FUSED_PARTICLE_PASS"); return !(e && e[0] == '0'); }();
        static const bool force_fused = [] { const char* e = getenv("TETSIM_FUSED_PARTICLE_PASS"); return e && e[0] == '1'; }();
        h->fused = allow_fused && !h->quad && !h->partitioned && nvo == nvl && B.every_owned_particle_has_a_partial && ntl > 0 &&
                   (B.num_blocks < 2048u || force_fused);
        k.fin_in = d.pos_final; k.fin_out = d.pos_final;
        h->info.fused_particle_pass = h->fused ? 1u : 0u;
        {
            const char* e = getenv("TETSIM_PJ_ONE_LAUNCH");
            h->pj_one_launch = !(e && e[0] == '0') && !h->fused && !h->quad && !h->partitioned && nvo == nvl && ntl > 0 && B.num_blocks > 0;
            if (h->pj_one_launch) {
                h->info.fused_particle_pass = 5u;
                if ((rc = dev_alloc(h, &h->d_substep_err, 1))) return rc;
                HIPCHK(h, hipMemset(h->d_substep_err, 0, sizeof(uint32_t)));
                const char* lag_env = getenv("TETSIM_PJ_CALL_LAG");
                const uint32_t lag = lag_env ? static_cast<uint32_t>(std::min<unsigned long>(strtoul(lag_env, nullptr, 10), 1ul << 24)) : kPJCallLagDefault;
                CallSchedule S;
                build_call_schedule(B.blk_verts.data(), B.blk_vert_off.data(), B.num_blocks, B.vp_ell.data(), B.vp_cols, B.nv_pad, nvo, lag, &S);
                if (S.fell_back) fprintf(stderr, "[tetsim] TETSIM_PJ_CALL_LAG=%u ignored (%s): the call runs in the plain order\n", lag, S.why.c_str());
                uint32_t* dsched;
                if ((rc = dev_alloc(h, &dsched, S.entry.size()))) return rc;
                if ((rc = upload(h, dsched, S.entry))) return rc;
                h->call_sched.entry = dsched; h->call_sched.period = S.period; h->call_sched.tail = S.tail;
            }
        }
        if (h->fused || h->quad) {
            uint32_t *dsrc, *dmax;
            if ((rc = dev_alloc(h, &dsrc, B.slot_src.size()))) return rc;
            if ((rc = dev_alloc(h, &dmax, B.blk_maxsrc.size()))) return rc;
            if ((rc = dev_alloc(h, &h->partial_b, nslots))) return rc;
            if ((rc = upload(h, dsrc, B.slot_src))) return rc;
            if ((rc = upload(h, dmax, B.blk_maxsrc))) return rc;
            HIPCHK(h, hipMemset(h->partial_b, 0, std::max<size_t>(nslots, 1) * sizeof(float4)));
            h->partial_slots = nslots;
            if (h->fused) {
                if ((rc = dev_alloc(h, &h->pos_final_b, nvl))) return rc;
                if ((rc = upload(h, h->pos_final_b, pos))) return rc;
            }
            k.slot_src = dsrc; k.blk_maxsrc = dmax; k.ns_pad = B.ns_pad;
            static const bool allow_frame = [] { const char* e = getenv("TETSIM_FRAME_KERNEL"); return !(e && e[0] == '0'); }();
            uint32_t cus = 0;
            const uint32_t per_cu = !allow_frame ? 0u : h->quad ? pjq_frame_capacity(&cus) : pjb_frame_capacity(pjb_mode(k), &cus);
            const uint32_t nbk = B.num_blocks;
            std::vector<int32_t> block_tile;
            const uint32_t slots = per_cu * cus, exclusive_max = slots - slots / 10u;
            if (per_cu != 0u && nbk != 0u && nbk <= (h->partitioned ? slots / 2u : exclusive_max)) {
                h->frame_exclusive = nbk > slots / 2u;
                static const bool allow_local = [] { const char* e = lab_env("TETSIM_FRAME_LOCAL"); return !(e && e[0] == '0'); }();
                static int xcd_rule[64] = {};
                int& rule = xcd_rule[o.device & 63];
                if (allow_local && rule == 0) rule = pjb_probe_xcd(h->stream, 256) == 8u ? 1 : 2;
                std::vector<std::vector<uint32_t>> groups(bodies);
                for (uint32_t b = 0; b < nbk; b++) {
                    const uint32_t body = batch ? body_of_tet(h, static_cast<uint32_t>(B.tet_perm[B.blk_tet_off[b]])) : 0u;
                    groups[std::min(body, bodies - 1u)].push_back(b);
                }
                const uint32_t budget = per_cu * (cus / 8u) / 2u;
                std::vector<uint32_t> by_size(bodies);
                for (uint32_t g = 0; g < bodies; g++) by_size[g] = g;
                std::stable_sort(by_size.begin(), by_size.end(), [&](uint32_t a, uint32_t c) { return groups[a].size() > groups[c].size(); });
                std::vector<std::vector<uint32_t>> on_xcd(8);
                bool local = allow_local && rule == 1 && cus % 8u == 0u;
                for (uint32_t g : by_size) {
                    if (!local) break;
                    uint32_t best = 0;
                    for (uint32_t x = 1; x < 8u; x++) if (on_xcd[x].size() < on_xcd[best].size()) best = x;
                    if (on_xcd[best].size() + groups[g].size() > budget) { local = false; break; }
                    on_xcd[best].insert(on_xcd[best].end(), groups[g].begin(), groups[g].end());
                }
                if (!local) {
                    for (auto& v : on_xcd) v.clear();
                    for (uint32_t b = 0; b < nbk; b++) on_xcd[b & 7u].push_back(b);
                }
                uint32_t most = 0;
                for (auto& v : on_xcd) most = std::max<uint32_t>(most, static_cast<uint32_t>(v.size()));
                block_tile.assign(8ull * most, -1);
                for (uint32_t x = 0; x < 8u; x++)
                    for (uint32_t j = 0; j < on_xcd[x].size(); j++) block_tile[8ull * j + x] = static_cast<int32_t>(on_xcd[x][j]);
                h->frame = true;
                frame_turn_enter(h);
                h->frame_local = local;
                h->frame_blocks = static_cast<uint32_t>(block_tile.size());
            }
            if (h->frame) {
                if ((rc = dev_alloc(h, &h->d_block_tile, block_tile.size()))) return rc;
                if ((rc = upload(h, h->d_block_tile, block_tile))) return rc;
                if ((rc = dev_alloc(h, &h->d_frame_err, 1))) return rc;
                HIPCHK(h, hipMemset(h->d_frame_err, 0, sizeof(uint32_t)));
                h->info.fused_particle_pass = h->quad ? 3u : 2u;
            }
        }
        if ((rc = upload(h, bto, B.blk_tet_off))) return rc;
        if ((rc = upload(h, bvo, B.blk_vert_off))) return rc;
        if ((rc = upload(h, bv, B.blk_verts))) return rc;
        if ((rc = upload(h, lidx, lidxh))) return rc;
        if ((rc = upload(h, k.rest_a, ra))) return rc;
        if ((rc = upload(h, k.rest_b, rb))) return rc;
        if (lean_state) {
            std::vector<float> rc1(ntl);
            for (uint32_t i = 0; i < ntl; i++) rc1[i] = rcv[i].x;
            if ((rc = upload(h, k.rest_c1, rc1))) return rc;
            if ((rc = upload(h, h->rest0_a, ra))) return rc;
            if ((rc = upload(h, h->rest0_b, rb))) return rc;
            if ((rc = upload(h, h->rest0_c, rcv))) return rc;
        } else if ((rc = upload(h, k.rest_c, rcv))) return rc;
        if ((rc = upload(h, vol, volh))) return rc;
        if ((rc = upload(h, k.quat, quat))) return rc;
        if ((rc = upload(h, lcr, B.lc_range))) return rc;
        if ((rc = upload(h, lce, lceh))) return rc;
        if ((rc = upload(h, vpe, B.vp_ell))) return rc;
        HIPCHK(h, hipMemset(k.partial, 0, std::max<size_t>(nslots, 1) * sizeof(float4)));
        k.blk_tet_off = bto; k.blk_vert_off = bvo; k.blk_verts = bv; k.tet_lidx = lidx; k.vol = vol;
        k.lc_range = lcr; k.lc_ent = lce; k.vp_ell = vpe; k.vp_cols = B.vp_cols; k.nv_pad = B.nv_pad;
        d.quat = k.quat;
#ifdef TETSIM_ABLATION
        if (lab_env("TETSIM_DEBUG_ITER_HIST")) {
            if ((rc = dev_alloc(h, &k.iter_hist, 278))) return rc;
            HIPCHK(h, hipMemset(k.iter_hist, 0, 278 * sizeof(unsigned long long)));
        }
#endif
        if (lab_env("TETSIM_DEBUG_TRACE") || lab_env("TETSIM_DEBUG_POLL_TRACE")) {
            const size_t rows = lab_env("TETSIM_DEBUG_POLL_TRACE") ? 2ull * B.num_blocks + (nvo + kBlockTile - 1u) / kBlockTile : B.num_blocks;
            if ((rc = dev_alloc(h, &k.trace, 8ull * rows))) return rc;
            HIPCHK(h, hipMemset(k.trace, 0, 8ull * rows * sizeof(unsigned long long)));
        }
    } else {
        if ((rc = dev_alloc(h, &d.tet_idx, ntl))) return rc;
        if ((rc = dev_alloc(h, &d.elem, 4ull * d.nt_pad))) return rc;
        if ((rc = dev_alloc(h, &d.quat, ntl))) return rc;
        if ((rc = dev_alloc(h, &d.slot_tab, static_cast<size_t>(std::max(maxv, 1u)) * d.nv_pad))) return rc;
        if ((rc = dev_alloc(h, &d.slot_cnt, d.nv_pad))) return rc;
        std::vector<int4> idx(ntl);
        std::vector<float4> elem(4ull * d.nt_pad, make_float4(0, 0, 0, 0)), quat(ntl, make_float4(0, 0, 0, 1));
        for (uint32_t e = 0; e < ntl; e++) {
            const int32_t* lt = &ltets[4 * e];
            idx[e] = make_int4(lt[0], lt[1], lt[2], lt[3]);
            const float w = rest_weight(e);
            for (int k = 0; k < 4; k++) {
                const float4 p = pos[lt[k]];
                elem[static_cast<size_t>(k) * d.nt_pad + e] = make_float4(p.x, p.y, p.z, w);
            }
        }
        if ((rc = upload(h, d.tet_idx, idx))) return rc;
        if ((rc = upload(h, d.elem, elem))) return rc;
        if ((rc = upload(h, d.quat, quat))) return rc;

        std::vector<int32_t> tab(static_cast<size_t>(std::max(maxv, 1u)) * d.nv_pad, 0);
        std::vector<uint32_t> cnt(d.nv_pad, 0);
        for (uint32_t v = 0; v < nvo; v++) {
            const uint32_t c = inc.offset[v + 1] - inc.offset[v];
            cnt[v] = c;
            for (uint32_t sl = 0; sl < c; sl++) {
                const int32_t enc = inc.slot[inc.offset[v] + sl];
                tab[static_cast<size_t>(sl) * d.nv_pad + v] = static_cast<int32_t>((enc & 3) * d.nt_pad + (enc >> 2));
            }
        }
        if ((rc = upload(h, d.slot_tab, tab))) return rc;
        if ((rc = upload(h, d.slot_cnt, cnt))) return rc;
    }

    if (h->partitioned) {
        for (const auto& nb : h->part.neigh) {
            NeighDev nd;
            nd.rank = nb.rank;
            nd.send_count = static_cast<uint32_t>(nb.send_local.size());
            nd.recv_start = nb.recv_start;
            nd.recv_count = nb.recv_count;
            nd.contiguous = nb.send_contiguous;
            nd.send_first = nd.send_count ? static_cast<uint32_t>(nb.send_local[0]) : 0;
            nd.send_global = nb.send_global;
            nd.recv_global = nb.recv_global;
            nd.send_local = nb.send_local;
            if (nd.send_count) {
                if ((rc = dev_alloc(h, &nd.send_idx, nd.send_count))) return rc;
                if ((rc = dev_alloc(h, &nd.send_buf, nd.send_count))) return rc;
                if ((rc = upload(h, nd.send_idx, nb.send_local))) return rc;
// ... 256 lines not shown
```

tetsim_amd/csrc/tetsim_host.cpp:

```cpp
#include "body.h"

using namespace tetsim;

namespace tetsim {
void build_strain_table(const float* verts, uint32_t nv, const int32_t* tets, uint32_t nt, double density, StrainRec* out) {
    std::vector<float> inv_mass(nv), irp(9ull * nt), irv(nt);
    prep_rest(verts, nv, tets, nt, density, inv_mass.data(), irp.data(), irv.data());
    for (uint32_t e = 0; e < nt; e++) {
        StrainRec& r = out[e];
        const int32_t* t = &tets[4ull * e];
        const double v0 = rest_volume(verts, t);
        bool finite = true;
        for (uint32_t k = 0; k < 9u; k++) {
            r.b[k] = irp[9ull * e + k];
            finite = finite && std::isfinite(r.b[k]);
        }
        for (uint32_t k = 0; k < 4u; k++) r.id[k] = t[k];
        r.degenerate = (v0 == 0.0 || !finite) ? 1u : 0u;
        r.v0_abs = std::fabs(v0);
    }
}
}

extern "C" {

struct tetsim_mesh_file { tetsim::MeshFile* m; };

int tetsim_mesh_write(const char* path, const TetSimMeshArrays* a) {
    if (!a) return fail(nullptr, TETSIM_EINVAL, "arrays is null");
    const std::string e = mesh_write(path, *a);
    return e.empty() ? TETSIM_OK : fail(nullptr, TETSIM_EINVAL, e);
}
int tetsim_mesh_open(const char* path, tetsim_mesh* out) {
    if (!out) return fail(nullptr, TETSIM_EINVAL, "out is null");
    *out = nullptr;
    tetsim::MeshFile* m = nullptr;
    const std::string e = mesh_open(path, &m);
    if (!e.empty()) return fail(nullptr, TETSIM_EINVAL, e);
    *out = new tetsim_mesh_file{m};
    return TETSIM_OK;
}
int tetsim_mesh_arrays(tetsim_mesh m, TetSimMeshArrays* out) {
    if (!m || !out) return fail(nullptr, TETSIM_EINVAL, "null argument");
    *out = mesh_arrays(m->m);
    return TETSIM_OK;
}
int tetsim_mesh_close(tetsim_mesh m) {
    if (!m) return TETSIM_OK;
    mesh_close(m->m);
    delete m;
    return TETSIM_OK;
}

int tetsim_prep_levels(const int32_t* tets, uint32_t nt, uint32_t nv, int32_t* level, uint32_t* num_levels) {
    if ((nt && (!tets || !level)) || !num_levels) return TETSIM_EINVAL;
    std::string e = validate_mesh(reinterpret_cast<const float*>(tets), nv ? nv : 1, tets, nt, false);
    if (!e.empty()) return fail(nullptr, TETSIM_EINVAL, e);
    *num_levels = prep_levels(tets, nt, nv, level);
    return 0;
}
int tetsim_prep_colours(const int32_t* tets, uint32_t nt, uint32_t nv, int32_t* colour, uint32_t* num_colours) {
    if ((nt && (!tets || !colour)) || !num_colours) return TETSIM_EINVAL;
    std::string e = validate_mesh(reinterpret_cast<const float*>(tets), nv ? nv : 1, tets, nt, false);
    if (!e.empty()) return fail(nullptr, TETSIM_EINVAL, e);
    *num_colours = prep_colours(tets, nt, nv, colour);
    return 0;
}
int tetsim_prep_clusters(const int32_t* tets, uint32_t nt, uint32_t nv, int32_t* order, int32_t* launch, int32_t* lane, int32_t* step,
                         uint32_t* num_launches, uint32_t* num_clusters) {
    if ((nt && (!tets || !order || !launch || !lane || !step)) || !num_launches) return TETSIM_EINVAL;
    std::string e = validate_mesh(reinterpret_cast<const float*>(tets), nv ? nv : 1, tets, nt, false);
    if (!e.empty()) return fail(nullptr, TETSIM_EINVAL, e);
    const ClusterPlan P = prep_clusters(tets, nt, nv);
    for (uint32_t i = 0; i < nt; i++) order[i] = P.pre[i];
    const uint32_t nl = static_cast<uint32_t>(P.launch_off.size() - 1);
    for (uint32_t l = 0; l < nl; l++)
        for (uint32_t j = P.step_off[l]; j < P.step_off[l + 1]; j++)
            for (uint32_t i = 0; i < P.step_count[j]; i++) {
                const uint32_t pos = P.exec_pos[P.step_first[j] + i];
                launch[pos] = static_cast<int32_t>(l);
                lane[pos] = static_cast<int32_t>(i);
                step[pos] = static_cast<int32_t>(j - P.step_off[l]);
            }
    *num_launches = nl;
    if (num_clusters) *num_clusters = P.num_clusters;
    return 0;
}
int tetsim_prep_tiles(const float* verts, uint32_t nv, const int32_t* tets, uint32_t nt, const uint32_t* body_first_tet,
                      const uint32_t* body_first_vert, uint32_t bodies, int32_t* tile_tets, uint32_t* tile_off, uint8_t* corner_slot,
                      uint32_t* num_tiles) {
    if (!num_tiles) return TETSIM_EINVAL;
    std::string e = validate_mesh(verts, nv, tets, nt, false);
    if (!e.empty()) return fail(nullptr, TETSIM_EINVAL, e);
    if (body_first_tet && body_first_vert && bodies) {
        if (body_first_tet[0] != 0 || body_first_vert[0] != 0 || body_first_tet[bodies] != nt || body_first_vert[bodies] != nv)
            return fail(nullptr, TETSIM_EINVAL, "body ranges must cover the whole mesh");
        for (uint32_t b = 0; b < bodies; b++) {
            if (body_first_tet[b] > body_first_tet[b + 1] || body_first_vert[b] >= body_first_vert[b + 1]) return fail(nullptr, TETSIM_EINVAL, "body ranges must ascend");
            for (uint64_t i = 4ull * body_first_tet[b]; i < 4ull * body_first_tet[b + 1]; i++)
                if (static_cast<uint32_t>(tets[i]) < body_first_vert[b] || static_cast<uint32_t>(tets[i]) >= body_first_vert[b + 1])
                    return fail(nullptr, TETSIM_EINVAL, "a tet references a particle of another body");
        }
    }
    const Incidence inc = build_incidence(tets, nt, nv, false, false);
    BlockPlan B;
    build_blocks(verts, tets, nt, nv, nv, inc, &B, body_first_tet, body_first_vert, bodies);
    *num_tiles = B.num_blocks;
    if (tile_tets) std::copy(B.tet_perm.begin(), B.tet_perm.end(), tile_tets);
    if (tile_off) std::copy(B.blk_tet_off.begin(), B.blk_tet_off.end(), tile_off);
    if (corner_slot) std::copy(B.tet_lidx.begin(), B.tet_lidx.end(), corner_slot);
    return 0;
}
int tetsim_prep_slot_table(const int32_t* tets, uint32_t nt, uint32_t nv, int32_t ref_quirk, int32_t* slots, uint32_t* dropped) {
    if ((nt && !tets) || !slots) return TETSIM_EINVAL;
    std::string e = validate_mesh(reinterpret_cast<const float*>(tets), nv ? nv : 1, tets, nt, false);
    if (!e.empty()) return fail(nullptr, TETSIM_EINVAL, e);
    const uint32_t d = prep_slot_table(tets, nt, nv, ref_quirk != 0, slots);
    if (dropped) *dropped = d;
    return 0;
}
int tetsim_prep_call_tiles(const float* verts, uint32_t nv, const int32_t* tets, uint32_t nt, uint32_t sizes[4], uint32_t* blk_vert_off,
                           int32_t* blk_verts, uint32_t* vp_ell) {
    if (!sizes) return TETSIM_EINVAL;
    std::string e = validate_mesh(verts, nv, tets, nt, false);
    if (!e.empty()) return fail(nullptr, TETSIM_EINVAL, e);
    const std::vector<uint32_t> order = morton_vertex_order(verts, nv, 0, nv);
    std::vector<int32_t> to_dev(nv), ltets(4ull * nt);
    std::vector<float> lverts(3ull * nv);
    for (uint32_t i = 0; i < nv; i++) {
        to_dev[order[i]] = static_cast<int32_t>(i);
        for (int c = 0; c < 3; c++) lverts[3ull * i + c] = verts[3ull * order[i] + c];
    }
    for (uint64_t i = 0; i < 4ull * nt; i++) ltets[i] = to_dev[tets[i]];
    const Incidence inc = build_incidence(ltets.data(), nt, nv, false, false);
    BlockPlan B;
    build_blocks(lverts.data(), ltets.data(), nt, nv, nv, inc, &B);
    sizes[0] = B.num_blocks; sizes[1] = static_cast<uint32_t>(B.blk_verts.size()); sizes[2] = B.vp_cols; sizes[3] = B.nv_pad;
    if (blk_vert_off) std::copy(B.blk_vert_off.begin(), B.blk_vert_off.end(), blk_vert_off);
    if (blk_verts) std::copy(B.blk_verts.begin(), B.blk_verts.end(), blk_verts);
    if (vp_ell) std::copy(B.vp_ell.begin(), B.vp_ell.begin() + static_cast<std::ptrdiff_t>(static_cast<size_t>(B.vp_cols) * B.nv_pad), vp_ell);
    return 0;
}
int tetsim_prep_call_schedule(const int32_t* blk_verts, const uint32_t* blk_vert_off, uint32_t nb, const uint32_t* vp_ell, uint32_t vp_cols,
                              uint32_t nv_pad, uint32_t nv_owned, uint32_t lag, uint32_t* entry, uint32_t capacity, uint32_t* period,
                              uint32_t* tail, int32_t* fell_back) {
    if (!blk_vert_off || (nb && !blk_verts) || (vp_cols && !vp_ell) || !period || !tail) return TETSIM_EINVAL;
    if (nv_owned > nv_pad && vp_cols) return fail(nullptr, TETSIM_EINVAL, "tetsim_prep_call_schedule: nv_owned exceeds the column stride of vp_ell");
    CallSchedule S;
    build_call_schedule(blk_verts, blk_vert_off, nb, vp_ell, vp_cols, nv_pad, nv_owned, lag, &S);
    *period = S.period; *tail = S.tail;
    if (fell_back) *fell_back = S.fell_back ? 1 : 0;
    if (S.fell_back) fail(nullptr, TETSIM_OK, "tetsim_prep_call_schedule: " + S.why + " -- the plain order instead");
    if (entry) {
        if (capacity < S.period) return fail(nullptr, TETSIM_EINVAL, "tetsim_prep_call_schedule: the table needs " + std::to_string(S.period) + " entries");
        std::copy(S.entry.begin(), S.entry.end(), entry);
    }
    return 0;
}
int tetsim_prep_check_call_schedule(const int32_t* blk_verts, const uint32_t* blk_vert_off, uint32_t nb, const uint32_t* vp_ell, uint32_t vp_cols,
                                    uint32_t nv_pad, uint32_t nv_owned, const uint32_t* entry, uint32_t period, uint32_t tail) {
    if (!blk_vert_off || (nb && !blk_verts) || (vp_cols && !vp_ell) || !entry) return TETSIM_EINVAL;
    const std::string bad = check_call_schedule(blk_verts, blk_vert_off, nb, vp_ell, vp_cols, nv_pad, nv_owned, entry, period, tail);
    return bad.empty() ? 0 : fail(nullptr, TETSIM_EINVAL, "call schedule: " + bad);
}
int tetsim_prep_ref_grab_texels(int32_t grab_id, uint32_t num_elems, uint32_t num_particles, int32_t out[2]) {
    if (!out) return TETSIM_EINVAL;
    ref_grab_texels(grab_id, num_elems, num_particles, out);
    return 0;
}
int tetsim_prep_boundary_surface(const float* verts, const int32_t* tets, uint32_t nt, uint32_t nv, float* vis_verts, int32_t* tri_ids,
                                 uint32_t* nrows, uint32_t* ntri) {
    if ((nt && !tets) || !nrows || !ntri || (!vis_verts != !tri_ids)) return fail(nullptr, TETSIM_EINVAL, "tetsim_prep_boundary_surface: null argument");
    if (nt && nv == 0) return fail(nullptr, TETSIM_EINVAL, "tetsim_prep_boundary_surface: tets without particles (nv == 0)");
    std::string e = validate_mesh(reinterpret_cast<const float*>(tets), nv ? nv : 1, tets, nt, false);
    if (!e.empty()) return fail(nullptr, TETSIM_EINVAL, e);
    if (nt > (1u << 24)) return fail(nullptr, TETSIM_EINVAL, "tetsim_prep_boundary_surface: a tet id above 2^24 does not fit the f32 row format");
    static const int kFace[4][3] = {{1, 2, 3}, {0, 3, 2}, {0, 1, 3}, {0, 2, 1}};
    struct Face { int32_t key[3]; uint32_t tet, face; };
    std::vector<Face> faces(4ull * nt);
    for (uint32_t t = 0; t < nt; t++)
        for (uint32_t k = 0; k < 4; k++) {
            Face& f = faces[4ull * t + k];
            for (int j = 0; j < 3; j++) f.key[j] = tets[4 * t + kFace[k][j]];
            std::sort(f.key, f.key + 3);
            f.tet = t; f.face = k;
        }
    std::sort(faces.begin(), faces.end(), [](const Face& a, const Face& b) {
        return std::lexicographical_compare(a.key, a.key + 3, b.key, b.key + 3) || (std::equal(a.key, a.key + 3, b.key) && (a.tet < b.tet || (a.tet == b.tet && a.face < b.face)));
    });
    std::vector<uint64_t> boundary;
    for (size_t i = 0; i < faces.size();) {
        size_t j = i + 1;
        while (j < faces.size() && std::equal(faces[i].key, faces[i].key + 3, faces[j].key)) j++;
        if (j - i == 1) boundary.push_back(4ull * faces[i].tet + faces[i].face);
        i = j;
    }
    std::sort(boundary.begin(), boundary.end());
    std::vector<int32_t> row(nv, -1);
    for (uint64_t b : boundary)
        for (int j = 0; j < 3; j++) row[tets[4 * (b >> 2) + kFace[b & 3][j]]] = 0;
    uint32_t rows = 0;
    for (uint32_t v = 0; v < nv; v++)
        if (row[v] == 0) row[v] = static_cast<int32_t>(rows++);
    *nrows = rows;
    *ntri = static_cast<uint32_t>(boundary.size());
    if (!vis_verts) return 0;
    std::vector<uint8_t> done(rows, 0);
    for (uint32_t t = 0; t < nt; t++)
        for (int k = 0; k < 4; k++) {
            const int32_t r = row[tets[4 * t + k]];
            if (r < 0 || done[r]) continue;
            done[r] = 1;
            vis_verts[4 * r] = static_cast<float>(t);
            for (int j = 0; j < 3; j++) vis_verts[4 * r + 1 + j] = j == k ? 1.0f : 0.0f;
        }
    for (size_t i = 0; i < boundary.size(); i++) {
        const uint32_t t = static_cast<uint32_t>(boundary[i] >> 2), k = static_cast<uint32_t>(boundary[i] & 3);
        bool flip = false;
        if (verts) {
            const int32_t* c = tets + 4 * t;
            double m[3][3];
            for (int a = 0; a < 3; a++)
                for (int x = 0; x < 3; x++) m[a][x] = static_cast<double>(verts[3 * c[a + 1] + x]) - static_cast<double>(verts[3 * c[0] + x]);
            const double det = m[0][0] * (m[1][1] * m[2][2] - m[1][2] * m[2][1]) - m[0][1] * (m[1][0] * m[2][2] - m[1][2] * m[2][0]) +
                               m[0][2] * (m[1][0] * m[2][1] - m[1][1] * m[2][0]);
            flip = det < 0.0;
        }
        const int32_t a = row[tets[4 * t + kFace[k][0]]], b = row[tets[4 * t + kFace[k][1]]], c2 = row[tets[4 * t + kFace[k][2]]];
        tri_ids[3 * i] = a;
        tri_ids[3 * i + 1] = flip ? c2 : b;
        tri_ids[3 * i + 2] = flip ? b : c2;
    }
    return 0;
}
int tetsim_prep_rest(const float* verts, uint32_t nv, const int32_t* tets, uint32_t nt, double density, float* inv_mass, float* inv_rest_pose, float* inv_rest_volume) {
    if (!inv_mass || (nt && (!inv_rest_pose || !inv_rest_volume))) return TETSIM_EINVAL;
    std::string e = validate_mesh(verts, nv, tets, nt, false);
    if (!e.empty()) return fail(nullptr, TETSIM_EINVAL, e);
    prep_rest(verts, nv, tets, nt, density, inv_mass, inv_rest_pose, inv_rest_volume);
    return 0;
}

int tetsim_prep_strain_table(const float* verts, uint32_t nv, const int32_t* tets, uint32_t nt, double density, void* records_out) {
    if (nt && !records_out) return TETSIM_EINVAL;
    std::string e = validate_mesh(verts, nv, tets, nt, false);
    if (!e.empty()) return fail(nullptr, TETSIM_EINVAL, e);
    std::vector<StrainRec> recs(nt);
    build_strain_table(verts, nv, tets, nt, density, recs.data());
    if (nt) std::memcpy(records_out, recs.data(), recs.size() * sizeof(StrainRec));
    return 0;
}

int tetsim_prep_partition(const float* verts, uint32_t nv, const int32_t* tets, uint32_t nt, int32_t part_count, int32_t* vert_owner_out) {
    if ((nt && !tets) || (nv && !vert_owner_out) || part_count < 1) return fail(nullptr, TETSIM_EINVAL, "tetsim_prep_partition: null argument or part_count < 1");
    if (verts)
        for (uint64_t i = 0; i < 3ull * nv; i++)
            if (!std::isfinite(verts[i])) return fail(nullptr, TETSIM_EINVAL, "non-finite vertex coordinate");
    const std::string e = prep_partition(verts, nv, tets, nt, part_count, vert_owner_out);
    return e.empty() ? TETSIM_OK : fail(nullptr, TETSIM_EINVAL, e);
}
int tetsim_prep_partition_quality(const int32_t* tets, uint32_t nt, uint32_t nv, int32_t part_count, const int32_t* vert_owner, TetSimPartQuality* out) {
    if ((nt && !tets) || !out || part_count < 1) return fail(nullptr, TETSIM_EINVAL, "tetsim_prep_partition_quality: null argument or part_count < 1");
    std::vector<int32_t> own;
    if (!vert_owner) {
        own.resize(nv);
        const std::string e = prep_partition(nullptr, nv, tets, nt, part_count, own.data());
        if (!e.empty()) return fail(nullptr, TETSIM_EINVAL, e);
        vert_owner = own.data();
    }
    std::vector<PartQuality> q(part_count);
    const std::string e = partition_quality(tets, nt, nv, part_count, vert_owner, q.data());
    if (!e.empty()) return fail(nullptr, TETSIM_EINVAL, e);
    for (int32_t r = 0; r < part_count; r++) {
        out[r].owned_particles = q[r].owned_particles; out[r].ghost_particles = q[r].ghost_particles; out[r].boundary_particles = q[r].boundary_particles;
        out[r].local_elems = q[r].local_elems; out[r].owned_elems = q[r].owned_elems; out[r].num_neighbours = q[r].num_neighbours;
    }
    return TETSIM_OK;
}

struct tetsim_plan_s { Partition P; };

int tetsim_plan_create(const int32_t* tets, uint32_t nt, uint32_t nv, int32_t part_count, int32_t part_index,
                       const int32_t* vert_owner, tetsim_plan* out) {
    if (!out) return fail(nullptr, TETSIM_EINVAL, "null plan pointer");
    *out = nullptr;
    std::string e = validate_mesh(reinterpret_cast<const float*>(tets), nv, tets, nt, false);
    if (!e.empty()) return fail(nullptr, TETSIM_EINVAL, e);
    tetsim_plan_s* p = new tetsim_plan_s();
    e = build_partition(tets, nt, nv, part_count, part_index, vert_owner, &p->P);
    if (!e.empty()) { delete p; return fail(nullptr, TETSIM_EINVAL, e); }
    *out = p;
    return 0;
}
int tetsim_plan_create_deep(const int32_t* tets, uint32_t nt, uint32_t nv, int32_t part_count, int32_t part_index,
                            const int32_t* vert_owner, int32_t depth, tetsim_plan* out) {
    if (!out) return fail(nullptr, TETSIM_EINVAL, "null plan pointer");
    *out = nullptr;
    std::string e = validate_mesh(reinterpret_cast<const float*>(tets), nv, tets, nt, false);
    if (!e.empty()) return fail(nullptr, TETSIM_EINVAL, e);
    tetsim_plan_s* p = new tetsim_plan_s();
    e = build_partition(tets, nt, nv, part_count, part_index, vert_owner, &p->P, depth);
    if (!e.empty()) { delete p; return fail(nullptr, TETSIM_EINVAL, e); }
    *out = p;
    return 0;
}
int tetsim_plan_layers(tetsim_plan p, uint32_t* first_layer_ghosts, uint8_t* tet_layer) {
    if (!p) return TETSIM_EINVAL;
    if (first_layer_ghosts) *first_layer_ghosts = p->P.n_ghost1;
    if (tet_layer) std::copy(p->P.tet_layer.begin(), p->P.tet_layer.end(), tet_layer);
    return 0;
}
int tetsim_plan_neighbour_layer2(tetsim_plan p, uint32_t i, uint32_t* send_count, uint32_t* recv_start, uint32_t* recv_count) {
    if (!p || i >= p->P.neigh.size()) return TETSIM_EINVAL;
    const auto& nb = p->P.neigh[i];
    if (send_count) *send_count = static_cast<uint32_t>(nb.send2_local.size());
    if (recv_start) *recv_start = nb.recv2_start;
// ... 51 lines not shown
```

tetsim_amd/softbody.py:

```python
import ctypes as C

import numpy as np

from . import _capi as capi
from ._capi import TetSimError


def _f32(a):
    return np.ascontiguousarray(a, dtype=np.float32)


def _fp(a):
    return a.ctypes.data_as(C.POINTER(C.c_float))


def _ip(a):
    return a.ctypes.data_as(C.POINTER(C.c_int32))


_COLLIDER_KINDS = {"sphere": capi.COLLIDER_SPHERE, "capsule": capi.COLLIDER_CAPSULE, "box": capi.COLLIDER_BOX, "plane": capi.COLLIDER_PLANE}


def _vec(v, n=3):
    if isinstance(v, dict):
# ... 77 lines not shown
def _check_rows(torch, t, dev, n, width, name):
    if (not isinstance(t, torch.Tensor) or t.dtype != torch.float32 or t.device != dev or tuple(t.shape) != (n, width)
            or (n and t.stride(1) != 1) or (n > 1 and t.stride(0) < width)):
        raise ValueError("%s must be a float32 tensor on %s of shape (%d, %d) with contiguous, non-overlapping rows" % (name, dev, n, width))


class Snapshot:

    def __init__(self, body, handle):
        self._body, self._s = body, handle

    def close(self):
        if self._s is not None and getattr(self._body, "_h", None):
            self._body._L.tetsim_snapshot_destroy(self._s)
            self._body._snapshots.remove(self)
        self._s = None

    def __del__(self):
        try:
            self.close()
        except Exception:
            pass


class SoftBodyHIP:

    def __init__(self, vertices, tetIds, tetEdgeIds=None, physicsParams=None, visVerts=None, visTriIds=None,
                 visMaterial=None, world=None, *, solver="polar", precision="precise", order="original",
                 ref_slot_table=True, ref_fixed_bounds=True, gather=False, constant_rest_shape=False, ref_grab_texel=False, deep_ghosts=False, ref_rotation_exit=False,
                 lean_state=False,
                 device=0, part_count=1, part_index=0, vert_owner=None, tet_colour=None, mesh_file=None, batch=None):
        L = capi.lib()
        self.physicsParams = physicsParams if physicsParams is not None else {}
        self._batch = None
        if batch is not None:
            self._batch = [(_f32(v).reshape(-1), np.ascontiguousarray(np.asarray(t).reshape(-1), dtype=np.int32)) for v, t in batch]
            offs = np.concatenate([[0], np.cumsum([len(v) // 3 for v, _ in self._batch])])
            vertices = np.concatenate([v for v, _ in self._batch])
            tetIds = np.concatenate([t + int(offs[i]) for i, (_, t) in enumerate(self._batch)])
        if mesh_file is not None:
            from .meshfile import MeshFile
            with MeshFile(mesh_file) as mf:
                vertices, tetIds = mf.verts.copy(), mf.tets.copy()
                if visVerts is None and mf.vis_verts is not None:
                    visVerts = mf.vis_verts.copy()
                    if visTriIds is None and mf.vis_tri_ids is not None:
                        visTriIds = mf.vis_tri_ids.copy()
        self._verts = _f32(vertices).reshape(-1)
        self._tets = np.ascontiguousarray(np.asarray(tetIds).reshape(-1), dtype=np.int32)
        if self._verts.size % 3 or self._tets.size % 4:
            raise ValueError("vertices must hold 3 floats per particle and tetIds 4 ids per tet")
        self.numParticles = self._verts.size // 3
        self.numElems = self._tets.size // 4
        self.visVerts = visVerts
        self.grabId = -1
        self.grabPos = np.zeros(3, dtype=np.float32)
        o = capi.TetSimOptions()
        L.tetsim_default_options(C.byref(o))
        o.solver = {"polar": capi.SOLVER_POLAR_JACOBI, "neohookean": capi.SOLVER_NEOHOOKEAN_GS}[solver]
        o.precision = {"precise": capi.PRECISE, "fast": capi.FAST}[precision]
        o.order = {"original": capi.ORDER_ORIGINAL, "coloured": capi.ORDER_COLOURED, "clustered": capi.ORDER_CLUSTERED}[order]
        o.flags = ((capi.FLAG_REF_SLOT_TABLE if ref_slot_table else 0) | (capi.FLAG_REF_FIXED_BOUNDS if ref_fixed_bounds else 0)
                   | (capi.FLAG_GATHER_FORMULATION if gather else 0)
                   | (capi.FLAG_CONSTANT_REST_SHAPE if constant_rest_shape else 0)
                   | (capi.FLAG_REF_GRAB_TEXEL if ref_grab_texel else 0) | (capi.FLAG_DEEP_GHOSTS if deep_ghosts else 0)
                   | (capi.FLAG_REF_ROTATION_EXIT if ref_rotation_exit else 0) | (capi.FLAG_LEAN_STATE if lean_state else 0))
        o.device = device
        d = self.physicsParams.get("density", 1000.0) if isinstance(self.physicsParams, dict) else getattr(self.physicsParams, "density", 1000.0)
        o.density = float(d)
        o.part_count, o.part_index = part_count, part_index
        self._owner = None
        if vert_owner is not None:
            self._owner = np.ascontiguousarray(vert_owner, dtype=np.int32)
            o.vert_owner = _ip(self._owner)
        self._colour = None
        if tet_colour is not None:
            self._colour = np.ascontiguousarray(tet_colour, dtype=np.int32)
            if self._colour.size != self.numElems:
                raise ValueError("tet_colour needs one entry per tet")
            o.tet_colour = _ip(self._colour)
        self.solver = solver
        self._h = C.c_void_p()
        if mesh_file is not None:
            capi.check(L.tetsim_create_from_file(str(mesh_file).encode(), C.byref(o), C.byref(self._h)))
        elif self._batch is not None:
            n = len(self._batch)
            vp = (C.POINTER(C.c_float) * n)(*[_fp(v) for v, _ in self._batch])
            tp = (C.POINTER(C.c_int32) * n)(*[_ip(t) for _, t in self._batch])
            nvs = (C.c_uint32 * n)(*[len(v) // 3 for v, _ in self._batch])
            nts = (C.c_uint32 * n)(*[len(t) // 4 for _, t in self._batch])
            capi.check(L.tetsim_create_batch(vp, nvs, tp, nts, n, C.byref(o), C.byref(self._h)))
        else:
            capi.check(L.tetsim_create(_fp(self._verts), self.numParticles, _ip(self._tets), self.numElems,
                                       C.byref(o), C.byref(self._h)))
        self.info = capi.TetSimInfo()
        capi.check(L.tetsim_get_info(self._h, C.byref(self.info)), self._h)
        self._L = L
        self._export_cache = {}
        self._snapshots = []
        self.numVisVerts = 0
        if visVerts is not None and len(visVerts):
            if mesh_file is not None:
                self.numVisVerts, self._has_normals = self.info.num_vis_verts, False
            else:
                self.setVisualMesh(visVerts)
            if visTriIds is not None and len(visTriIds) and part_count <= 1:
                self.setVisualTriangles(visTriIds)

    @classmethod
    def batch(cls, bodies, physicsParams=None, **kw):
        return cls(None, None, None, physicsParams, batch=list(bodies), **kw)

    @property
    def bodyRanges(self):
        n = self.info.num_bodies
        fp_, fe = (C.c_uint32 * (n + 1))(), (C.c_uint32 * (n + 1))()
        capi.check(self._L.tetsim_get_batch_layout(self._h, fp_, fe), self._h)
        return [((fp_[b], fp_[b + 1]), (fe[b], fe[b + 1])) for b in range(n)]

    @classmethod
    def fromFile(cls, path, physicsParams=None, visMaterial=None, world=None, **kw):
        return cls(None, None, None, physicsParams, None, None, visMaterial, world, mesh_file=path, **kw)

    def close(self):
        if getattr(self, "_h", None):
            for snap in getattr(self, "_snapshots", ()):
                snap._s = None
            self._snapshots = []
            self._L.tetsim_destroy(self._h)
            self._h = None

    def __del__(self):
        try:
            self.close()
        except Exception:
            pass

    def simulate(self, dt, physicsParams=None):
        pp = self.physicsParams if physicsParams is None else physicsParams
        if isinstance(pp, dict) and self.solver == "polar":
            pp["dt"] = dt
        capi.check(self._L.tetsim_step(self._h, float(dt), C.byref(make_params(pp))), self._h)

    def simulateSubsteps(self, n, dt, physicsParams=None):
        pp = self.physicsParams if physicsParams is None else physicsParams
        capi.check(self._L.tetsim_step_n(self._h, int(n), float(dt), C.byref(make_params(pp))), self._h)

    def endFrame(self):
        capi.check(self._L.tetsim_sync(self._h), self._h)

    def sync(self):
        capi.check(self._L.tetsim_sync(self._h), self._h)

    def _read3(self, fn, n):
        out = np.empty(3 * n, dtype=np.float32)
        capi.check(fn(self._h, _fp(out)), self._h)
        return out.reshape(-1, 3)

    @property
    def pos(self):
        return self._read3(self._L.tetsim_read_positions, self.info.owned_particles)

    @property
    def posPinned(self):
        ptr = C.POINTER(C.c_float)()
        capi.check(self._L.tetsim_read_positions_pinned(self._h, C.byref(ptr)), self._h)
        return np.ctypeslib.as_array(ptr, shape=(self.info.owned_particles, 3))

    @property
    def prevPos(self):
        return self._read3(self._L.tetsim_read_prev_positions, self.info.owned_particles)

    @property
    def vel(self):
        return self._read3(self._L.tetsim_read_velocities, self.info.owned_particles)

    @property
    def quats(self):
        out = np.empty(4 * self.info.local_elems, dtype=np.float32)
        capi.check(self._L.tetsim_read_quats(self._h, _fp(out)), self._h)
        return out.reshape(-1, 4)

    @property
    def quatsPinned(self):
        ptr = C.POINTER(C.c_float)()
        capi.check(self._L.tetsim_read_quats_pinned(self._h, C.byref(ptr)), self._h)
        return np.ctypeslib.as_array(ptr, shape=(self.info.local_elems, 4))

    def saveState(self):
        n = C.c_uint64()
        capi.check(self._L.tetsim_state_size(self._h, C.byref(n)), self._h)
        buf = (C.c_char * n.value)()
        capi.check(self._L.tetsim_save_state(self._h, buf, n.value), self._h)
        return bytes(buf.raw)

    def loadState(self, blob):
        capi.check(self._L.tetsim_load_state(self._h, bytes(blob), len(blob)), self._h)

    @property
    def volError(self):
        v = C.c_double()
        capi.check(self._L.tetsim_read_vol_error(self._h, C.byref(v)), self._h)
        return v.value

    @property
    def invMass(self):
        out = np.empty(self.numParticles, dtype=np.float32)
        capi.check(self._L.tetsim_read_inv_mass(self._h, _fp(out)), self._h)
        return out

    @property
    def ownedIds(self):
        out = np.empty(self.info.owned_particles, dtype=np.int32)
        capi.check(self._L.tetsim_get_owned_ids(self._h, _ip(out)), self._h)
        return out

    @property
    def localTets(self):
        out = np.empty(self.info.local_elems, dtype=np.int32)
        capi.check(self._L.tetsim_get_local_tets(self._h, _ip(out)), self._h)
        return out

    @property
    def tetOrder(self):
        out = np.empty(self.numElems, dtype=np.int32)
        capi.check(self._L.tetsim_get_tet_order(self._h, _ip(out)), self._h)
        return out

    @property
    def levelOffsets(self):
        out = np.empty(self.info.num_levels + 1, dtype=np.int32)
        capi.check(self._L.tetsim_get_level_offsets(self._h, _ip(out)), self._h)
        return out

    def writeState(self, pos, vel):
        p, v = _f32(pos).reshape(-1), _f32(vel).reshape(-1)
        capi.check(self._L.tetsim_write_state(self._h, _fp(p), _fp(v)), self._h)

    def _torch_stream(self, torch, stream):
        dev = torch.device("cuda", self.info.device)
        if stream is None:
            return dev, torch.cuda.current_stream(dev).cuda_stream
        return dev, int(getattr(stream, "cuda_stream", stream))

    def exportTensors(self, fields=("pos",), out=None, stream=None):
        import torch
        dev, s = self._torch_stream(torch, stream)
        names = [fields] if isinstance(fields, str) else list(fields)
        cache = self._export_cache
        arr = (capi.TetSimDeviceField * max(1, len(names)))()
        res = {}
        for f, name in zip(arr, names):
            field, rows, width = _EXPORT_FIELDS[name]
            n = int(getattr(self.info, rows))
            t = out.get(name) if out is not None else None
            if t is None:
                t = cache.get(name)
                if t is None or t.shape[0] != n:
                    t = cache[name] = torch.empty((n, width), dtype=torch.float32, device=dev)
            else:
                _check_rows(torch, t, dev, n, width, "out[%r]" % name)
            f.field, f.reserved, f.dst = field, 0, t.data_ptr()
            f.row_stride = 4 * t.stride(0) if n > 1 else 0
            res[name] = t
        capi.check(self._L.tetsim_export_device(self._h, arr, len(names), s), self._h)
        return res

    def importTensors(self, pos, vel, stream=None):
        import torch
        dev, s = self._torch_stream(torch, stream)
        n = self.info.owned_particles
        _check_rows(torch, pos, dev, n, 3, "pos")
        _check_rows(torch, vel, dev, n, 3, "vel")
        capi.check(self._L.tetsim_import_device(self._h, pos.data_ptr(), 4 * pos.stride(0) if n > 1 else 0,
                                                vel.data_ptr(), 4 * vel.stride(0) if n > 1 else 0, s), self._h)

    def _body_mask(self, torch, dev, bodies):
        if bodies is None:
            return None, None
        n = self.info.num_bodies
        if isinstance(bodies, torch.Tensor):
            if bodies.dtype not in (torch.bool, torch.uint8) or bodies.device != dev or bodies.numel() != n or not bodies.is_contiguous():
                raise ValueError("bodies must be a contiguous torch.bool / torch.uint8 tensor of %d elements on %s" % (n, dev))
            return bodies.data_ptr(), bodies
        host = np.asarray([bool(b) for b in bodies], dtype=np.bool_)
        if host.size != n:
            raise ValueError("bodies must name every one of the %d bodies" % n)
        t = torch.from_numpy(host).to(dev)
        torch.cuda.current_stream(dev).synchronize()
        return t.data_ptr(), t

    def snapshot(self, stream=None):
        s = C.c_void_p()
        capi.check(self._L.tetsim_snapshot_create(self._h, C.byref(s)), self._h)
        snap = Snapshot(self, s)
        self._snapshots.append(snap)
        return snap

    def _snapshot_call(self, fn, snap, bodies, stream):
        import torch
        dev, s = self._torch_stream(torch, stream)
        if not isinstance(snap, Snapshot) or snap._s is None:
            raise ValueError("snap must be a live Snapshot")
        ptr, keep = self._body_mask(torch, dev, bodies)
        capi.check(fn(self._h, snap._s, ptr, s), self._h)
        self._mask_keep = keep
# ... 335 lines not shown
```

Baseline: 35170 M tet-solves/s.

## Add banded tile order for the persistent polar-Jacobi call schedule

Adds a second tile ordering for the one-launch polar-Jacobi call schedule. It builds a tile adjacency graph from shared particle blocks and orders tiles with a reverse Cuthill-McKee-like breadth-first sweep from a pseudo-peripheral root. Particle-block entries are then sorted by the latest tile they depend on, and placement can be balanced across XCD columns. The aim is to make particle blocks ready sooner and improve cache locality, at the cost of more complex host prep and a changed default order and lag when no env vars are set. It also adds schedule stats and query APIs.

```diff
diff --git a/include/tetsim.h b/include/tetsim.h
--- a/include/tetsim.h
+++ b/include/tetsim.h
@@ -278,6 +278,16 @@
 int tetsim_prep_check_call_schedule(const int32_t *blk_verts, const uint32_t *blk_vert_off, uint32_t nb, const uint32_t *vp_ell,
                                     uint32_t vp_cols, uint32_t nv_pad, uint32_t nv_owned, const uint32_t *entry, uint32_t period,
                                     uint32_t tail);
+int tetsim_prep_call_schedule_order(const int32_t *blk_verts, const uint32_t *blk_vert_off, uint32_t nb, const uint32_t *vp_ell,
+                                    uint32_t vp_cols, uint32_t nv_pad, uint32_t nv_owned, uint32_t lag, uint32_t order, uint32_t *entry,
+                                    uint32_t capacity, uint32_t *period, uint32_t *tail, int32_t *fell_back);
+int tetsim_prep_check_call_schedule_order(const int32_t *blk_verts, const uint32_t *blk_vert_off, uint32_t nb, const uint32_t *vp_ell,
+                                          uint32_t vp_cols, uint32_t nv_pad, uint32_t nv_owned, const uint32_t *entry, uint32_t period,
+                                          uint32_t tail, uint32_t order);
+int tetsim_prep_call_schedule_stats(const int32_t *blk_verts, const uint32_t *blk_vert_off, uint32_t nb, const uint32_t *vp_ell,
+                                    uint32_t vp_cols, uint32_t nv_pad, uint32_t nv_owned, const uint32_t *entry, uint32_t period,
+                                    int64_t out[11]);
+int tetsim_get_call_schedule(tetsim_handle h, uint32_t out[4]);
 int tetsim_prep_ref_grab_texels(int32_t grab_id, uint32_t num_elems, uint32_t num_particles, int32_t out[2]);
 int tetsim_prep_boundary_surface(const float *verts ,
                                  const int32_t *tets, uint32_t nt, uint32_t nv,
diff --git a/tetsim_amd/_capi.py b/tetsim_amd/_capi.py
--- a/tetsim_amd/_capi.py
+++ b/tetsim_amd/_capi.py
@@ -65,7 +65,7 @@
 DEBUG_ENV_NAMES = ["TETSIM_DEBUG_LOOPBACK_HALO", "TETSIM_DEBUG_LOOPBACK_COPY", "TETSIM_DEBUG_ONE_STREAM", "TETSIM_DEBUG_GROUP_SYNC",
                    "TETSIM_DEBUG_HOSTPROF", "TETSIM_DEBUG_TRACE", "TETSIM_HALO_SYNC", "TETSIM_HALO_GRAPH", "TETSIM_DEBUG_LOOPBACK_DELAY_US", "TETSIM_NH_QUADS", "TETSIM_FUSED_PARTICLE_PASS",
                    "TETSIM_FRAME_KERNEL", "TETSIM_FRAME_LOCAL", "TETSIM_NH_FOLD", "TETSIM_HALO_ALIGNED_TILES", "TETSIM_HALO_FOLD_WAIT", "TETSIM_QUAD", "TETSIM_QUAD_POLL_DELAY", "TETSIM_NH_FRAME",
-                   "TETSIM_NH_ONE_LAUNCH", "TETSIM_PJ_ONE_LAUNCH", "TETSIM_PJ_CALL_LAG"]
+                   "TETSIM_NH_ONE_LAUNCH", "TETSIM_PJ_ONE_LAUNCH", "TETSIM_PJ_CALL_LAG", "TETSIM_PJ_CALL_ORDER"]
 
 
 LAB_ENV_NAMES = ["TETSIM_DEBUG_TRACE", "TETSIM_NH_QUADS", "TETSIM_FRAME_LOCAL", "TETSIM_NH_FOLD", "TETSIM_HALO_ALIGNED_TILES", "TETSIM_QUAD_POLL_DELAY", "TETSIM_NH_FRAME"]
@@ -122,7 +122,7 @@
     "tetsim_comm_unique_id", "tetsim_comm_init", "tetsim_comm_info", "tetsim_comm_selftest", "tetsim_comm_probe", "tetsim_group_step_n", "tetsim_halo_exchange_local", "tetsim_get_halo_plan",
     "tetsim_halo_p2p_export", "tetsim_halo_p2p_connect",
     "tetsim_halo_export", "tetsim_halo_import", "tetsim_prep_levels", "tetsim_prep_colours", "tetsim_prep_clusters",
-    "tetsim_prep_tiles", "tetsim_prep_slot_table", "tetsim_prep_call_tiles", "tetsim_prep_call_schedule", "tetsim_prep_check_call_schedule", "tetsim_prep_ref_grab_texels", "tetsim_prep_rest", "tetsim_prep_partition", "tetsim_prep_partition_quality", "tetsim_plan_create", "tetsim_plan_destroy", "tetsim_plan_sizes",
+    "tetsim_prep_tiles", "tetsim_prep_slot_table", "tetsim_prep_call_tiles", "tetsim_prep_call_schedule", "tetsim_prep_check_call_schedule", "tetsim_prep_call_schedule_order", "tetsim_prep_check_call_schedule_order", "tetsim_prep_call_schedule_stats", "tetsim_get_call_schedule", "tetsim_prep_ref_grab_texels", "tetsim_prep_rest", "tetsim_prep_partition", "tetsim_prep_partition_quality", "tetsim_plan_create", "tetsim_plan_destroy", "tetsim_plan_sizes",
     "tetsim_plan_arrays", "tetsim_plan_neighbour", "tetsim_plan_neighbour_ids",
     "tetsim_plan_create_deep", "tetsim_plan_layers", "tetsim_plan_neighbour_layer2", "tetsim_plan_neighbour_layer2_ids",
     "tetsim_raycast_visual", "tetsim_start_grab_ray", "tetsim_read_visual_bounding_sphere", "tetsim_prep_boundary_surface",
@@ -256,6 +256,10 @@
     L.tetsim_prep_call_tiles.argtypes = [fp, u32, ip, u32, up, up, ip, up]
     L.tetsim_prep_call_schedule.argtypes = [ip, up, u32, up, u32, u32, u32, u32, up, u32, up, up, ip]
     L.tetsim_prep_check_call_schedule.argtypes = [ip, up, u32, up, u32, u32, u32, up, u32, u32]
+    L.tetsim_prep_call_schedule_order.argtypes = [ip, up, u32, up, u32, u32, u32, u32, u32, up, u32, up, up, ip]
+    L.tetsim_prep_check_call_schedule_order.argtypes = [ip, up, u32, up, u32, u32, u32, up, u32, u32, u32]
+    L.tetsim_prep_call_schedule_stats.argtypes = [ip, up, u32, up, u32, u32, u32, up, u32, C.POINTER(C.c_int64)]
+    L.tetsim_get_call_schedule.argtypes = [H, up]
     L.tetsim_prep_ref_grab_texels.argtypes = [i32, u32, u32, ip]
     L.tetsim_prep_rest.argtypes = [fp, u32, ip, u32, dbl, fp, fp, fp]
     L.tetsim_prep_partition.argtypes = [fp, u32, ip, u32, i32, ip]
diff --git a/tetsim_amd/csrc/body.h b/tetsim_amd/csrc/body.h
--- a/tetsim_amd/csrc/body.h
+++ b/tetsim_amd/csrc/body.h
@@ -180,6 +180,7 @@
     bool pj_one_launch = false;
     uint32_t* d_substep_err = nullptr;
     PJCallSched call_sched;
+    uint32_t call_order = 0, call_lag = 0;
     float4 *rest0_a = nullptr, *rest0_b = nullptr, *rest0_c = nullptr;
     bool quat_stale = false;
     bool frame = false;
diff --git a/tetsim_amd/csrc/build_info.cpp b/tetsim_amd/csrc/build_info.cpp
--- a/tetsim_amd/csrc/build_info.cpp
+++ b/tetsim_amd/csrc/build_info.cpp
@@ -17,18 +17,20 @@
 #ifdef TETSIM_ABLATION
     out->ablation = 1;
 #endif
-    static const struct { const char* name; bool lab; } kEnv[] = {
-        {"TETSIM_DEBUG_LOOPBACK_HALO", false}, {"TETSIM_DEBUG_LOOPBACK_COPY", false}, {"TETSIM_DEBUG_ONE_STREAM", false}, {"TETSIM_DEBUG_GROUP_SYNC", false},
-        {"TETSIM_DEBUG_HOSTPROF", false}, {"TETSIM_DEBUG_TRACE", true}, {"TETSIM_HALO_SYNC", false}, {"TETSIM_HALO_GRAPH", false}, {"TETSIM_DEBUG_LOOPBACK_DELAY_US", false},
-        {"TETSIM_NH_QUADS", true}, {"TETSIM_FUSED_PARTICLE_PASS", false}, {"TETSIM_FRAME_KERNEL", false}, {"TETSIM_FRAME_LOCAL", true}, {"TETSIM_NH_FOLD", true},
-        {"TETSIM_HALO_ALIGNED_TILES", true}, {"TETSIM_HALO_FOLD_WAIT", false}, {"TETSIM_QUAD", false}, {"TETSIM_QUAD_POLL_DELAY", true}, {"TETSIM_NH_FRAME", true},
-        {"TETSIM_NH_ONE_LAUNCH", false}, {"TETSIM_PJ_ONE_LAUNCH", false}, {"TETSIM_PJ_CALL_LAG", false}};
-    for (unsigned i = 0; i < sizeof(kEnv) / sizeof(kEnv[0]); i++) {
-#ifndef TETSIM_ABLATION
-        if (kEnv[i].lab) continue;
+#ifdef TETSIM_ABLATION
+#define LAB(name) name
+#else
+#define LAB(name) nullptr
 #endif
-        if (std::getenv(kEnv[i].name)) out->debug_env |= 1u << i;
-    }
+    static const char* const kEnv[] = {
+        "TETSIM_DEBUG_LOOPBACK_HALO", "TETSIM_DEBUG_LOOPBACK_COPY", "TETSIM_DEBUG_ONE_STREAM", "TETSIM_DEBUG_GROUP_SYNC", "TETSIM_DEBUG_HOSTPROF",
+        LAB("TETSIM_DEBUG_TRACE"), "TETSIM_HALO_SYNC", "TETSIM_HALO_GRAPH", "TETSIM_DEBUG_LOOPBACK_DELAY_US", LAB("TETSIM_NH_QUADS"),
+        "TETSIM_FUSED_PARTICLE_PASS", "TETSIM_FRAME_KERNEL", LAB("TETSIM_FRAME_LOCAL"), LAB("TETSIM_NH_FOLD"), LAB("TETSIM_HALO_ALIGNED_TILES"),
+        "TETSIM_HALO_FOLD_WAIT", "TETSIM_QUAD", LAB("TETSIM_QUAD_POLL_DELAY"), LAB("TETSIM_NH_FRAME"), "TETSIM_NH_ONE_LAUNCH",
+        "TETSIM_PJ_ONE_LAUNCH", "TETSIM_PJ_CALL_LAG", "TETSIM_PJ_CALL_ORDER"};
+#undef LAB
+    for (unsigned i = 0; i < sizeof(kEnv) / sizeof(kEnv[0]); i++)
+        if (kEnv[i] && std::getenv(kEnv[i])) out->debug_env |= 1u << i;
     std::strncpy(out->source_sha, TETSIM_SOURCE_SHA, sizeof(out->source_sha) - 1);
     std::strncpy(out->kernel_sha, TETSIM_KERNEL_SHA, sizeof(out->kernel_sha) - 1);
     return TETSIM_OK;
diff --git a/tetsim_amd/csrc/host_prep.cpp b/tetsim_amd/csrc/host_prep.cpp
--- a/tetsim_amd/csrc/host_prep.cpp
+++ b/tetsim_amd/csrc/host_prep.cpp
@@ -517,17 +517,66 @@
     for (auto& v : D.pbs_of_tile) uniq(v);
     return D;
 }
-inline uint32_t sched_tile_of(uint32_t r, uint32_t per_xcd) { return (r & 7u) * per_xcd + (r >> 3); }
-void sched_plain(const SchedDeps& D, uint32_t nb, CallSchedule* out) {
+constexpr uint32_t kNoTile = 0xffffffffu;
+std::vector<uint32_t> sched_sweep(const SchedDeps& D, uint32_t nb) {
+    std::vector<std::vector<uint32_t>> adj(nb);
+    for (const auto& clique : D.tiles_of_pb)
+        for (uint32_t a : clique) for (uint32_t b : clique) if (a != b) adj[a].push_back(b);
+    for (auto& v : adj) { std::sort(v.begin(), v.end()); v.erase(std::unique(v.begin(), v.end()), v.end()); }
+    auto by_degree = [&](uint32_t a, uint32_t b) { return adj[a].size() != adj[b].size() ? adj[a].size() < adj[b].size() : a < b; };
+    for (auto& v : adj) std::sort(v.begin(), v.end(), by_degree);
+    std::vector<uint32_t> rank_of(nb, kNoTile), level(nb), sweep, front;
+    sweep.reserve(nb);
+    auto levels = [&](uint32_t root) {
+        front.assign(1, root);
+        std::vector<uint8_t> seen(nb, 0);
+        seen[root] = 1; level[root] = 0;
+        for (size_t i = 0; i < front.size(); i++)
+            for (uint32_t b : adj[front[i]])
+                if (!seen[b] && rank_of[b] == kNoTile) { seen[b] = 1; level[b] = level[front[i]] + 1u; front.push_back(b); }
+        return level[front.back()];
+    };
+    for (uint32_t first = 0; first < nb; first++) {
+        if (rank_of[first] != kNoTile) continue;
+        uint32_t root = first, depth = levels(root);
+        for (int round = 0; round < 16; round++) {
+            uint32_t far = front.back();
+            for (uint32_t b : front) if (level[b] == depth && by_degree(b, far)) far = b;
+            const uint32_t d2 = levels(far);
+            if (d2 <= depth) { levels(root); break; }
+            root = far; depth = d2;
+        }
+        for (uint32_t b : front) { rank_of[b] = static_cast<uint32_t>(sweep.size()); sweep.push_back(b); }
+    }
+    std::reverse(sweep.begin(), sweep.end());
+    return sweep;
+}
+std::string sched_order(const SchedDeps& D, uint32_t nb, uint32_t order, std::vector<uint32_t>* seq, std::vector<uint32_t>* xcd_of) {
+    seq->assign(D.tet_blocks, kNoTile);
+    if (order == kCallOrderPlain) {
+        for (uint32_t r = 0; r < D.tet_blocks; r++) { const uint32_t b = (r & 7u) * D.per_xcd + (r >> 3); if (b < nb) (*seq)[r] = b; }
+    } else if (order == kCallOrderBanded) {
+        const std::vector<uint32_t> sweep = sched_sweep(D, nb);
+        std::copy(sweep.begin(), sweep.end(), seq->begin());
+    } else return "order " + std::to_string(order) + " is not known";
+    xcd_of->assign(nb, 0);
+    for (uint32_t r = 0; r < D.tet_blocks; r++) if ((*seq)[r] != kNoTile) (*xcd_of)[(*seq)[r]] = r & 7u;
+    return "";
+}
+void sched_lag0(const SchedDeps& D, const std::vector<uint32_t>& seq, uint32_t order, CallSchedule* out) {
     out->period = D.plain_period;
-    out->tail = 0; out->lag = 0;
+    out->tail = 0; out->lag = 0; out->order = order;
     out->entry.assign(out->period, sched_entry(kSchedEmpty, 0));
+    std::vector<uint32_t> at(D.pbs_of_tile.size(), 0);
     for (uint32_t r = 0; r < D.tet_blocks; r++)
-        if (sched_tile_of(r, D.per_xcd) < nb) out->entry[r] = sched_entry(kSchedTile, r);
-    for (uint32_t k = 0; k < D.npb; k++) out->entry[D.tet_blocks + k] = sched_entry(kSchedParticles, k);
+        if (seq[r] != kNoTile) { out->entry[r] = sched_entry(kSchedTile, seq[r]); at[seq[r]] = r; }
+    std::vector<uint32_t> pbs(D.npb), last(D.npb, 0);
+    for (uint32_t k = 0; k < D.npb; k++) { pbs[k] = k; for (uint32_t b : D.tiles_of_pb[k]) last[k] = std::max(last[k], at[b] >> 3); }
+    if (order != kCallOrderPlain) std::stable_sort(pbs.begin(), pbs.end(), [&](uint32_t a, uint32_t b) { return last[a] < last[b]; });
+    for (uint32_t k = 0; k < D.npb; k++) out->entry[D.tet_blocks + k] = sched_entry(kSchedParticles, pbs[k]);
 }
 struct SchedPass { std::vector<uint32_t> entry, ready, left; uint32_t head_end = 0; bool stuck = false; };
-SchedPass sched_pass(const SchedDeps& D, uint32_t nb, uint32_t lag, const std::vector<uint32_t>& head_at) {
+SchedPass sched_pass(const SchedDeps& D, uint32_t nb, const std::vector<uint32_t>& seq, uint32_t lag, const std::vector<uint32_t>& head_at, bool balanced) {
     constexpr uint32_t none = 0xffffffffu;
     SchedPass R;
     R.ready.assign(D.npb, none);
@@ -548,20 +597,22 @@
         if (tiles_left == 0 && hi == head.size() && (p & 7u) == 0u) break;
         if (p >= limit) { R.stuck = true; break; }
         const uint32_t x = p & 7u;
+        const bool may = !balanced || col_next[x] == *std::max_element(col_next, col_next + 8);
+        if (!may) {  } else
         if (hi < head.size() && head_at[head[hi]] <= p) {
             const uint32_t k = head[hi++];
             R.entry.push_back(sched_entry(kSchedParticles, k, true));
             head_placed[k] = 1; R.head_end = p + 1u;
             continue;
         }
-        if (qi < queue.size() && R.ready[queue[qi]] <= p) { R.entry.push_back(sched_entry(kSchedParticles, queue[qi++])); continue; }
+        if (may && qi < queue.size() && R.ready[queue[qi]] <= p) { R.entry.push_back(sched_entry(kSchedParticles, queue[qi++])); continue; }
         if (col_next[x] < D.per_xcd) {
-            const uint32_t r = 8u * col_next[x] + x, b = sched_tile_of(r, D.per_xcd);
+            const uint32_t b = seq[8u * col_next[x] + x];
             bool held = false;
             if (b < nb) for (uint32_t k : D.pbs_of_tile[b]) held = held || (head_at[k] != none && !head_placed[k]);
             if (!held) {
                 col_next[x]++; tiles_left--;
-                R.entry.push_back(b < nb ? sched_entry(kSchedTile, r) : sched_entry(kSchedEmpty, 0));
+                R.entry.push_back(b < nb ? sched_entry(kSchedTile, b) : sched_entry(kSchedEmpty, 0));
                 if (b < nb) for (uint32_t k : pbs_by_tile[b])
                     if (--need[k] == 0) { R.ready[k] = p + 8u * lag; if (head_at[k] == none) queue.push_back(k); }
                 continue;
@@ -575,9 +626,12 @@
 }
 
 std::string check_call_schedule(const int32_t* blk_verts, const uint32_t* blk_vert_off, uint32_t nb, const uint32_t* vp_ell, uint32_t vp_cols,
-                                uint32_t nv_pad, uint32_t nv_owned, const uint32_t* entry, uint32_t period, uint32_t tail, uint32_t tile) {
+                                uint32_t nv_pad, uint32_t nv_owned, const uint32_t* entry, uint32_t period, uint32_t tail, uint32_t tile, uint32_t order) {
     constexpr uint32_t none = 0xffffffffu;
     const SchedDeps D = sched_deps(blk_verts, blk_vert_off, nb, vp_ell, vp_cols, nv_pad, nv_owned, tile);
+    std::vector<uint32_t> seq, xcd_of;
+    const std::string unknown = sched_order(D, nb, order, &seq, &xcd_of);
+    if (!unknown.empty()) return unknown;
     if (period == 0 || period % 8u != 0u) return "the period is not a positive multiple of 8";
     if (period < D.plain_period) return "the period is shorter than a substep's blocks";
     std::vector<uint64_t> at_tile(nb, none), at_pb(D.npb, none);
@@ -587,12 +641,15 @@
         const bool wrapped = (entry[p] & kSchedWrapped) != 0u;
         if (kind == kSchedEmpty) continue;
         if (kind == kSchedTile) {
-            const uint32_t b = sched_tile_of(index, D.per_xcd);
-            if (index >= D.tet_blocks || b >= nb) return "entry " + std::to_string(p) + " names a tile that does not exist";
-            if ((index & 7u) != (p & 7u)) return "tile block " + std::to_string(index) + " is not on its XCD";
-            if (wrapped) return "tile block " + std::to_string(index) + " is wrapped";
-            if ((index >> 3) < col_seen[p & 7u]) return "tile block " + std::to_string(index) + " is out of its XCD's order";
-            col_seen[p & 7u] = (index >> 3) + 1u;
+            const uint32_t b = index;
+            if (b >= nb) return "entry " + std::to_string(p) + " names a tile that does not exist";
+            if (xcd_of[b] != (p & 7u)) return "tile " + std::to_string(b) + " is not on its XCD";
+            if (wrapped) return "tile " + std::to_string(b) + " is wrapped";
+            if (order == kCallOrderPlain) {
+                const uint32_t row = b - xcd_of[b] * D.per_xcd;
+                if (row < col_seen[p & 7u]) return "tile " + std::to_string(b) + " is out of its XCD's order";
+                col_seen[p & 7u] = row + 1u;
+            }
             if (at_tile[b] != none) return "tile " + std::to_string(b) + " appears twice";
             at_tile[b] = p;
         } else if (kind == kSchedParticles) {
@@ -615,21 +672,32 @@
 }
 
 void build_call_schedule(const int32_t* blk_verts, const uint32_t* blk_vert_off, uint32_t nb, const uint32_t* vp_ell, uint32_t vp_cols,
-                         uint32_t nv_pad, uint32_t nv_owned, uint32_t lag, CallSchedule* out, uint32_t tile) {
+                         uint32_t nv_pad, uint32_t nv_owned, uint32_t lag, CallSchedule* out, uint32_t tile, uint32_t order) {
     constexpr uint32_t none = 0xffffffffu;
     const SchedDeps D = sched_deps(blk_verts, blk_vert_off, nb, vp_ell, vp_cols, nv_pad, nv_owned, tile);
     *out = CallSchedule();
+    std::vector<uint32_t> seq, xcd_of;
     auto plain = [&](const std::string& why) {
-        sched_plain(D, nb, out);
+        sched_order(D, nb, kCallOrderPlain, &seq, &xcd_of);
+        sched_lag0(D, seq, kCallOrderPlain, out);
         out->fell_back = !why.empty(); out->why = why;
     };
-    if (lag == 0 || nb == 0) return plain("");
+    if (nb == 0) return plain("");
+    const std::string unknown = sched_order(D, nb, order, &seq, &xcd_of);
+    if (!unknown.empty()) return plain(unknown);
+    if (lag == 0) {
+        if (order == kCallOrderPlain) return plain("");
+        sched_lag0(D, seq, order, out);
+        const std::string bad = check_call_schedule(blk_verts, blk_vert_off, nb, vp_ell, vp_cols, nv_pad, nv_owned, out->entry.data(), out->period, out->tail, tile, order);
+        if (!bad.empty()) return plain("order " + std::to_string(order) + ": " + bad);
+        return;
+    }
     if (static_cast<uint64_t>(lag) * 8u >= D.plain_period) return plain("lag " + std::to_string(lag) + ": a whole substep or more");
     std::vector<uint32_t> head_at(D.npb, none);
     SchedPass R;
     bool settled = false;
     for (int pass = 0; pass < 64 && !settled; pass++) {
-        R = sched_pass(D, nb, lag, head_at);
+        R = sched_pass(D, nb, seq, lag, head_at, order != kCallOrderPlain);
         if (R.stuck) return plain("lag " + std::to_string(lag) + ": the layout does not close");
         const uint32_t period = static_cast<uint32_t>(R.entry.size());
         settled = R.left.empty();
@@ -641,9 +709,59 @@
     out->entry = R.entry;
     out->period = static_cast<uint32_t>(R.entry.size());
     out->tail = R.head_end;
-    out->lag = lag;
-    const std::string bad = check_call_schedule(blk_verts, blk_vert_off, nb, vp_ell, vp_cols, nv_pad, nv_owned, out->entry.data(), out->period, out->tail, tile);
+    out->lag = lag; out->order = order;
+    const std::string bad = check_call_schedule(blk_verts, blk_vert_off, nb, vp_ell, vp_cols, nv_pad, nv_owned, out->entry.data(), out->period, out->tail, tile, order);
     if (!bad.empty()) return plain("lag " + std::to_string(lag) + ": " + bad);
+}
+
+std::string call_schedule_stats(const int32_t* blk_verts, const uint32_t* blk_vert_off, uint32_t nb, const uint32_t* vp_ell, uint32_t vp_cols,
+                                uint32_t nv_pad, uint32_t nv_owned, const uint32_t* entry, uint32_t period, CallScheduleStats* out, uint32_t tile) {
+    constexpr uint64_t none = ~0ull;
+    const SchedDeps D = sched_deps(blk_verts, blk_vert_off, nb, vp_ell, vp_cols, nv_pad, nv_owned, tile);
+    *out = CallScheduleStats();
+    if (period == 0 || period % 8u != 0u) return "the period is not a positive multiple of 8";
+    std::vector<uint64_t> at_tile(nb, none), at_pb(D.npb, none);
+    for (uint32_t p = 0; p < period; p++) {
+        const uint32_t kind = entry[p] >> 30, index = entry[p] & kSchedIndexMask;
+        const bool wrapped = (entry[p] & kSchedWrapped) != 0u;
+        if (kind == kSchedEmpty) { out->empty++; continue; }
+        if (kind == kSchedTile && index < nb && at_tile[index] == none) at_tile[index] = p;
+        else if (kind == kSchedParticles && index < D.npb && at_pb[index] == none) { at_pb[index] = static_cast<uint64_t>(p) + (wrapped ? period : 0u); out->wrapped += wrapped ? 1u : 0u; }
+        else return "entry " + std::to_string(p) + " names nothing, or something a second time";
+    }
+    for (uint64_t a : at_tile) if (a == none) return "a tile is missing";
+    for (uint64_t a : at_pb) if (a == none) return "a particle block is missing";
+    auto row = [](uint64_t a) { return static_cast<int64_t>(a >> 3); };
+    auto pick = [](std::vector<int64_t>& v, size_t num, size_t den) {
+        if (v.empty()) return static_cast<int64_t>(0);
+        std::sort(v.begin(), v.end());
+        return v[std::min(v.size() - 1u, (v.size() - 1u) * num / den)];
+    };
+    std::vector<int64_t> ahead, to_pb, to_tile;
+    int64_t band = 0;
+    for (uint32_t b = 0; b < nb; b++) {
+        int64_t reach = row(at_tile[b]);
+        for (uint32_t k : D.pbs_of_tile[b]) {
+            for (uint32_t b2 : D.tiles_of_pb[k]) reach = std::max(reach, row(at_tile[b2]));
+            to_tile.push_back(row(at_tile[b] + period) - row(at_pb[k]));
+        }
+        ahead.push_back(reach - row(at_tile[b]));
+    }
+    for (uint32_t k = 0; k < D.npb; k++) {
+        int64_t lo = INT64_MAX, hi = INT64_MIN;
+        for (uint32_t b : D.tiles_of_pb[k]) {
+            to_pb.push_back(row(at_pb[k]) - row(at_tile[b]));
+            lo = std::min(lo, row(at_tile[b])); hi = std::max(hi, row(at_tile[b]));
+        }
+        if (!D.tiles_of_pb[k].empty()) band = std::max(band, hi - lo);
+    }
+    out->ahead_median = pick(ahead, 1, 2); out->ahead_p90 = pick(ahead, 9, 10); out->ahead_max = pick(ahead, 1, 1);
+    out->tile_to_pb_min = pick(to_pb, 0, 1); out->tile_to_pb_median = pick(to_pb, 1, 2);
+    out->pb_to_tile_min = pick(to_tile, 0, 1); out->pb_to_tile_median = pick(to_tile, 1, 2);
+    out->band = band;
+    const int64_t fit = static_cast<int64_t>(D.per_xcd) - band - static_cast<int64_t>((D.npb + 7u) / 8u) - 1;
+    out->fit_lag = std::max<int64_t>(fit, 0);
+    return "";
 }
 
 std::string validate_mesh(const float* verts, uint32_t nv, const int32_t* tets, uint32_t nt, bool forbid_repeats) {
diff --git a/tetsim_amd/csrc/host_prep.h b/tetsim_amd/csrc/host_prep.h
--- a/tetsim_amd/csrc/host_prep.h
+++ b/tetsim_amd/csrc/host_prep.h
@@ -113,18 +113,30 @@
 constexpr uint32_t pjb_call_blocks_per_sub(uint32_t nb, uint32_t nv_owned, uint32_t threads) {
     return (((nb + 7u) & ~7u) + (nv_owned + threads - 1u) / threads + 7u) & ~7u;
 }
-constexpr uint32_t kPJCallLagDefault = 0;
+constexpr uint32_t sched_tile_of_block(uint32_t r, uint32_t per_xcd) { return (r & 7u) * per_xcd + (r >> 3); }
+constexpr uint32_t sched_block_of_tile(uint32_t b, uint32_t per_xcd) { return (b % per_xcd) * 8u + b / per_xcd; }
+constexpr uint32_t kCallOrderPlain = 0, kCallOrderBanded = 1;
+constexpr uint32_t kPJCallOrderDefault = kCallOrderBanded;
+constexpr uint32_t kPJCallLagDefault = 256;
 struct CallSchedule {
     std::vector<uint32_t> entry;
     uint32_t period = 0, tail = 0;
     uint32_t lag = 0;
+    uint32_t order = 0;
     bool fell_back = false;
     std::string why;
 };
 void build_call_schedule(const int32_t* blk_verts, const uint32_t* blk_vert_off, uint32_t nb, const uint32_t* vp_ell, uint32_t vp_cols,
-                         uint32_t nv_pad, uint32_t nv_owned, uint32_t lag, CallSchedule* out, uint32_t tile = kBlockTile);
+                         uint32_t nv_pad, uint32_t nv_owned, uint32_t lag, CallSchedule* out, uint32_t tile = kBlockTile, uint32_t order = kCallOrderPlain);
 std::string check_call_schedule(const int32_t* blk_verts, const uint32_t* blk_vert_off, uint32_t nb, const uint32_t* vp_ell, uint32_t vp_cols,
-                                uint32_t nv_pad, uint32_t nv_owned, const uint32_t* entry, uint32_t period, uint32_t tail, uint32_t tile = kBlockTile);
+                                uint32_t nv_pad, uint32_t nv_owned, const uint32_t* entry, uint32_t period, uint32_t tail, uint32_t tile = kBlockTile,
+                                uint32_t order = kCallOrderPlain);
+struct CallScheduleStats {
+    int64_t ahead_median = 0, ahead_p90 = 0, ahead_max = 0, tile_to_pb_min = 0, tile_to_pb_median = 0, pb_to_tile_min = 0, pb_to_tile_median = 0,
+            band = 0, fit_lag = 0, empty = 0, wrapped = 0;
+};
+std::string call_schedule_stats(const int32_t* blk_verts, const uint32_t* blk_vert_off, uint32_t nb, const uint32_t* vp_ell, uint32_t vp_cols,
+                                uint32_t nv_pad, uint32_t nv_owned, const uint32_t* entry, uint32_t period, CallScheduleStats* out, uint32_t tile = kBlockTile);
 
 std::string validate_mesh(const float* verts, uint32_t nv, const int32_t* tets, uint32_t nt, bool forbid_repeats);
 
diff --git a/tetsim_amd/csrc/pj_blocked.hip b/tetsim_amd/csrc/pj_blocked.hip
--- a/tetsim_amd/csrc/pj_blocked.hip
+++ b/tetsim_amd/csrc/pj_blocked.hip
@@ -55,7 +55,7 @@
 struct PJHaloWait { const PJPeerSync* w; const uint32_t* vflag; uint32_t* error; uint32_t timeout_ms; const float4* ghosts; };
 constexpr int kModeCarried = 0, kModeConstantRest = 1, kModeLeanState = 2;
 inline int blk_mode(const PJBlk& d) { return pjb_mode(d); }
-struct PJPoll { uint32_t block, want; uint32_t* error; uint32_t timeout_ms; };
+struct PJPoll { uint32_t tile, want; uint32_t* error; uint32_t timeout_ms; };
 template <int kMode, bool kFused, bool kAlt = false, bool kHaloWait = false, bool kPoll = false>
 __device__ __forceinline__ void pjb_tet_body(const PJBlk& d, uint32_t tile_first, uint32_t tile_count, uint32_t tiles_per_xcd TETSIM_DBG_PARAM,
                                              [[maybe_unused]] const PJHaloWait* hw = nullptr, const uint32_t stamp = 0u, [[maybe_unused]] const PJPoll* poll = nullptr) {
@@ -66,9 +66,8 @@
     __shared__ uint2 s_ent[kTile];
 
     constexpr bool kLean = kMode == kModeConstantRest;
-    uint32_t block_index = blockIdx.x;
-    if constexpr (kPoll) block_index = poll->block;
-    const uint32_t rel = xcd_tile(block_index, tiles_per_xcd);
+    uint32_t rel = 0;
+    if constexpr (kPoll) rel = poll->tile; else rel = xcd_tile(blockIdx.x, tiles_per_xcd);
     if (rel >= tile_count) return;
     const uint32_t b = tile_first + rel;
     const uint32_t tid = threadIdx.x;
diff --git a/tetsim_amd/csrc/tetsim_api.hip b/tetsim_amd/csrc/tetsim_api.hip
--- a/tetsim_amd/csrc/tetsim_api.hip
+++ b/tetsim_amd/csrc/tetsim_api.hip
@@ -590,6 +590,14 @@
     return 0;
 }
 
+int tetsim_get_call_schedule(tetsim_handle h, uint32_t out[4]) {
+    if (!h || !out) return fail(h, TETSIM_EINVAL, "null argument");
+    const bool has = h->pj_one_launch || h->call_sched.entry;
+    out[0] = has ? h->call_order : 0u; out[1] = has ? h->call_lag : 0u;
+    out[2] = has ? h->call_sched.period : 0u; out[3] = has ? h->call_sched.tail : 0u;
+    return 0;
+}
+
 int tetsim_step(tetsim_handle h, double dt, const TetSimParams* params) {
     if (!h) return TETSIM_EINVAL;
     if (!h->group.empty()) return fail(h, TETSIM_ESTATE, "this body belongs to an in-process group: step it with tetsim_group_step_n");
diff --git a/tetsim_amd/csrc/tetsim_create.hip b/tetsim_amd/csrc/tetsim_create.hip
--- a/tetsim_amd/csrc/tetsim_create.hip
+++ b/tetsim_amd/csrc/tetsim_create.hip
@@ -268,14 +268,18 @@
                 if ((rc = dev_alloc(h, &h->d_substep_err, 1))) return rc;
                 HIPCHK(h, hipMemset(h->d_substep_err, 0, sizeof(uint32_t)));
                 const char* lag_env = getenv("TETSIM_PJ_CALL_LAG");
-                const uint32_t lag = lag_env ? static_cast<uint32_t>(std::min<unsigned long>(strtoul(lag_env, nullptr, 10), 1ul << 24)) : kPJCallLagDefault;
+                uint32_t lag = lag_env ? static_cast<uint32_t>(std::min<unsigned long>(strtoul(lag_env, nullptr, 10), 1ul << 24)) : 0u;
+                const char* order_env = getenv("TETSIM_PJ_CALL_ORDER");
+                if (!lag_env && !order_env) lag = kPJCallLagDefault;
+                const uint32_t order = order_env ? static_cast<uint32_t>(std::min<unsigned long>(strtoul(order_env, nullptr, 10), 1ul << 24)) : (lag_env ? kCallOrderPlain : kPJCallOrderDefault);
                 CallSchedule S;
-                build_call_schedule(B.blk_verts.data(), B.blk_vert_off.data(), B.num_blocks, B.vp_ell.data(), B.vp_cols, B.nv_pad, nvo, lag, &S);
-                if (S.fell_back) fprintf(stderr, "[tetsim] TETSIM_PJ_CALL_LAG=%u ignored (%s): the call runs in the plain order\n", lag, S.why.c_str());
+                build_call_schedule(B.blk_verts.data(), B.blk_vert_off.data(), B.num_blocks, B.vp_ell.data(), B.vp_cols, B.nv_pad, nvo, lag, &S, kBlockTile, order);
+                if (S.fell_back && (lag_env || order_env)) fprintf(stderr, "[tetsim] TETSIM_PJ_CALL_ORDER=%u TETSIM_PJ_CALL_LAG=%u ignored (%s): the call runs in the plain order\n", order, lag, S.why.c_str());
                 uint32_t* dsched;
                 if ((rc = dev_alloc(h, &dsched, S.entry.size()))) return rc;
                 if ((rc = upload(h, dsched, S.entry))) return rc;
                 h->call_sched.entry = dsched; h->call_sched.period = S.period; h->call_sched.tail = S.tail;
+                h->call_order = S.order; h->call_lag = S.lag;
             }
         }
         if (h->fused || h->quad) {
diff --git a/tetsim_amd/csrc/tetsim_host.cpp b/tetsim_amd/csrc/tetsim_host.cpp
--- a/tetsim_amd/csrc/tetsim_host.cpp
+++ b/tetsim_amd/csrc/tetsim_host.cpp
@@ -141,27 +141,69 @@
     if (vp_ell) std::copy(B.vp_ell.begin(), B.vp_ell.begin() + static_cast<std::ptrdiff_t>(static_cast<size_t>(B.vp_cols) * B.nv_pad), vp_ell);
     return 0;
 }
+namespace {
+int prep_call_schedule(const char* who, bool block_form, const int32_t* blk_verts, const uint32_t* blk_vert_off, uint32_t nb, const uint32_t* vp_ell, uint32_t vp_cols,
+                       uint32_t nv_pad, uint32_t nv_owned, uint32_t lag, uint32_t order, uint32_t* entry, uint32_t capacity, uint32_t* period,
+                       uint32_t* tail, int32_t* fell_back) {
+    const std::string me = who;
+    if (!blk_vert_off || (nb && !blk_verts) || (vp_cols && !vp_ell) || !period || !tail) return TETSIM_EINVAL;
+    if (nv_owned > nv_pad && vp_cols) return fail(nullptr, TETSIM_EINVAL, me + ": nv_owned exceeds the column stride of vp_ell");
+    CallSchedule S;
+    build_call_schedule(blk_verts, blk_vert_off, nb, vp_ell, vp_cols, nv_pad, nv_owned, lag, &S, kBlockTile, order);
+    *period = S.period; *tail = S.tail;
+    if (fell_back) *fell_back = S.fell_back ? 1 : 0;
+    if (S.fell_back) fail(nullptr, TETSIM_OK, me + ": " + S.why + " -- the plain order instead");
+    if (entry) {
+        if (capacity < S.period) return fail(nullptr, TETSIM_EINVAL, me + ": the table needs " + std::to_string(S.period) + " entries");
+        std::copy(S.entry.begin(), S.entry.end(), entry);
+        if (block_form)
+            for (uint32_t p = 0; p < S.period; p++)
+                if ((entry[p] >> 30) == kSchedTile) entry[p] = sched_entry(kSchedTile, sched_block_of_tile(entry[p] & kSchedIndexMask, (nb + 7u) / 8u));
+    }
+    return 0;
+}
+}
 int tetsim_prep_call_schedule(const int32_t* blk_verts, const uint32_t* blk_vert_off, uint32_t nb, const uint32_t* vp_ell, uint32_t vp_cols,
                               uint32_t nv_pad, uint32_t nv_owned, uint32_t lag, uint32_t* entry, uint32_t capacity, uint32_t* period,
                               uint32_t* tail, int32_t* fell_back) {
-    if (!blk_vert_off || (nb && !blk_verts) || (vp_cols && !vp_ell) || !period || !tail) return TETSIM_EINVAL;
-    if (nv_owned > nv_pad && vp_cols) return fail(nullptr, TETSIM_EINVAL, "tetsim_prep_call_schedule: nv_owned exceeds the column stride of vp_ell");
-    CallSchedule S;
-    build_call_schedule(blk_verts, blk_vert_off, nb, vp_ell, vp_cols, nv_pad, nv_owned, lag, &S);
-    *period = S.period; *tail = S.tail;
-    if (fell_back) *fell_back = S.fell_back ? 1 : 0;
-    if (S.fell_back) fail(nullptr, TETSIM_OK, "tetsim_prep_call_schedule: " + S.why + " -- the plain order instead");
-    if (entry) {
-        if (capacity < S.period) return fail(nullptr, TETSIM_EINVAL, "tetsim_prep_call_schedule: the table needs " + std::to_string(S.period) + " entries");
-        std::copy(S.entry.begin(), S.entry.end(), entry);
-    }
-    return 0;
+    return prep_call_schedule("tetsim_prep_call_schedule", true, blk_verts, blk_vert_off, nb, vp_ell, vp_cols, nv_pad, nv_owned, lag, kCallOrderPlain, entry, capacity,
+                              period, tail, fell_back);
+}
+int tetsim_prep_call_schedule_order(const int32_t* blk_verts, const uint32_t* blk_vert_off, uint32_t nb, const uint32_t* vp_ell, uint32_t vp_cols,
+                                    uint32_t nv_pad, uint32_t nv_owned, uint32_t lag, uint32_t order, uint32_t* entry, uint32_t capacity, uint32_t* period,
+                                    uint32_t* tail, int32_t* fell_back) {
+    return prep_call_schedule("tetsim_prep_call_schedule_order", false, blk_verts, blk_vert_off, nb, vp_ell, vp_cols, nv_pad, nv_owned, lag, order, entry, capacity,
+                              period, tail, fell_back);
 }
 int tetsim_prep_check_call_schedule(const int32_t* blk_verts, const uint32_t* blk_vert_off, uint32_t nb, const uint32_t* vp_ell, uint32_t vp_cols,
                                     uint32_t nv_pad, uint32_t nv_owned, const uint32_t* entry, uint32_t period, uint32_t tail) {
     if (!blk_vert_off || (nb && !blk_verts) || (vp_cols && !vp_ell) || !entry) return TETSIM_EINVAL;
-    const std::string bad = check_call_schedule(blk_verts, blk_vert_off, nb, vp_ell, vp_cols, nv_pad, nv_owned, entry, period, tail);
+    const uint32_t per_xcd = (nb + 7u) / 8u;
+    std::vector<uint32_t> tiled(entry, entry + period);
+    for (uint32_t& e : tiled)
+        if ((e >> 30) == kSchedTile) {
+            const uint32_t r = e & kSchedIndexMask;
+            e = (e & ~kSchedIndexMask) | (r < 8u * per_xcd ? sched_tile_of_block(r, per_xcd) : kSchedIndexMask);
+        }
+    const std::string bad = check_call_schedule(blk_verts, blk_vert_off, nb, vp_ell, vp_cols, nv_pad, nv_owned, tiled.data(), period, tail);
     return bad.empty() ? 0 : fail(nullptr, TETSIM_EINVAL, "call schedule: " + bad);
+}
+int tetsim_prep_check_call_schedule_order(const int32_t* blk_verts, const uint32_t* blk_vert_off, uint32_t nb, const uint32_t* vp_ell, uint32_t vp_cols,
+                                          uint32_t nv_pad, uint32_t nv_owned, const uint32_t* entry, uint32_t period, uint32_t tail, uint32_t order) {
+    if (!blk_vert_off || (nb && !blk_verts) || (vp_cols && !vp_ell) || !entry) return TETSIM_EINVAL;
+    const std::string bad = check_call_schedule(blk_verts, blk_vert_off, nb, vp_ell, vp_cols, nv_pad, nv_owned, entry, period, tail, kBlockTile, order);
+    return bad.empty() ? 0 : fail(nullptr, TETSIM_EINVAL, "call schedule: " + bad);
+}
+int tetsim_prep_call_schedule_stats(const int32_t* blk_verts, const uint32_t* blk_vert_off, uint32_t nb, const uint32_t* vp_ell, uint32_t vp_cols,
+                                    uint32_t nv_pad, uint32_t nv_owned, const uint32_t* entry, uint32_t period, int64_t out[11]) {
+    if (!blk_vert_off || (nb && !blk_verts) || (vp_cols && !vp_ell) || !entry || !out) return TETSIM_EINVAL;
+    CallScheduleStats S;
+    const std::string bad = call_schedule_stats(blk_verts, blk_vert_off, nb, vp_ell, vp_cols, nv_pad, nv_owned, entry, period, &S);
+    if (!bad.empty()) return fail(nullptr, TETSIM_EINVAL, "call schedule: " + bad);
+    const int64_t rows[11] = {S.ahead_median, S.ahead_p90, S.ahead_max, S.tile_to_pb_min, S.tile_to_pb_median, S.pb_to_tile_min, S.pb_to_tile_median,
+                              S.band, S.fit_lag, S.empty, S.wrapped};
+    std::copy(rows, rows + 11, out);
+    return 0;
 }
 int tetsim_prep_ref_grab_texels(int32_t grab_id, uint32_t num_elems, uint32_t num_particles, int32_t out[2]) {
     if (!out) return TETSIM_EINVAL;
diff --git a/tetsim_amd/softbody.py b/tetsim_amd/softbody.py
--- a/tetsim_amd/softbody.py
+++ b/tetsim_amd/softbody.py
@@ -253,6 +253,11 @@
     def sync(self):
         capi.check(self._L.tetsim_sync(self._h), self._h)
 
+    def callSchedule(self):
+        out = (C.c_uint32 * 4)()
+        capi.check(self._L.tetsim_get_call_schedule(self._h, out), self._h)
+        return dict(zip(("order", "lag", "period", "tail"), (int(x) for x in out)))
+
     def _read3(self, fn, n):
         out = np.empty(3 * n, dtype=np.float32)
         capi.check(fn(self._h, _fp(out)), self._h)
```

After: 34780 M tet-solves/s. -1.1%, worse.
